# half-potato/nmf

Hardware: AMD Instinct MI355X
Metric: train rays/sec (microfacet_tensorf2, 4096-ray chunks, steady state) (higher is better)
Workload: dtype f32; 1 GPU; BASELINE configs[1] on scene S1 (solid cube, SURVEY 8d), TensoRF 128^3 (16+24 comps, f32 tables), env 512x1024, 800x800 camera, 4096 rays/GPU/step in 1 chunk(s) of 4096, fwd+bwd+all-reduce+Adam, steady state (all secondary rays re-traced); rays_per_gpu=4096, chunks_in_flight=1, grid=128, parallelism=dp1, ranks_seen=1, startup_steps=55, operator_graph_fallbacks=0

## Files before the change

### include/nmf_hip.h

```cpp
#ifndef NMF_HIP_H
#define NMF_HIP_H

#include <stdint.h>

#ifdef __cplusplus
extern "C" {
#endif

#define NMF_OK 0
#define NMF_EINVAL (-1)
#define NMF_ERANGE (-2)

#define NMF_DENSITY_C 16
#define NMF_APP_C 24
#define NMF_APP_DIM 24
#define NMF_MLP_IN 66
#define NMF_MLP_HID 64

#define NMF_ABI_VERSION 125
int nmf_version(void);
const char* nmf_last_error_string(void);

int nmf_event_create(void** event);
int nmf_event_create_timed(void** event);
// ... 199 lines not shown
                        const float* feat_noise, float anoise, float min_rough, int32_t row_inputs, float* V, float* N,
                        float* r1, float* f0, float* diffuse, float* feat, float* xyz, void* stream);
int nmf_bounce_prep_fwd_heads(const int32_t* bidx, int64_t Mb, const float* normals, const float* app, const float* head_W,
                              const float* head_b, float diffuse_mul, float diffuse_bias, float tint_bias, float f0_bias,
                              float rough_bias, const float* xyzt, const int32_t* ray_id, const float* rays, const float* conv,
                              const float* feat_noise, float anoise, float min_rough, int32_t row_inputs, float* heads_out,
                              float* V, float* N, float* r1, float* f0, float* diffuse, float* feat, float* xyz, void* stream);
int nmf_bounce_prep_bwd(const int32_t* inv, int64_t M, const int32_t* bidx, int64_t Mb, const float* normals,
                        const float* heads, const int32_t* ray_id, const float* rays, const float* conv,
                        float min_rough, int32_t detach_normals, int32_t row_inputs, const float* dN,
                        const float* dr1, const float* df0,
                        const float* ddiffuse, const int32_t row_strides[4], const float* dfeat, float* d_normals,
                        float* d_heads, float* d_app, void* stream);
int nmf_bounce_prep_heads_bwd(const int32_t* bidx, int64_t Mb, const float* normals, const float* heads, const int32_t* ray_id,
                              const float* rays, const float* conv, float min_rough, int32_t detach_normals, const float* dN,
                              const float* dr1, const float* df0, const float* ddiffuse, const int32_t row_strides[4],
                              const float* dfeat, const float* app, const float* head_W, const float* head_b, float diffuse_mul,
                              float diffuse_bias, float tint_bias, float f0_bias, float rough_bias, float* d_normals, float* d_app,
                              float* g_head_W, float* g_head_b, void* stream);
int nmf_ray_compose_fwd(const float* weight, const float* refl_rows, const int32_t* inv, const float* normals,
                        const float* rays, const int64_t* offsets, int64_t B, const float* bg, int32_t bg_per_ray,
                        int32_t tonemap, int32_t noclip, float* rgb_map, float* acc, float* rgb_lin, float* ori,
                        void* stream);
int nmf_ray_compose_bwd(const float* weight, const float* refl_rows, const int32_t* inv, const float* normals,
                        const float* rays, const int32_t* ray_id, int64_t M, const float* bg, int32_t bg_per_ray,
                        int32_t tonemap, int32_t noclip, const float* rgb_lin, const float* d_rgb_map,
                        const float* d_acc, const float* d_ori, float* d_weight, float* d_refl, float* d_normals,
                        void* stream);
int nmf_bg_adjoint(const float* acc, const float* d_rgb_map, int64_t B, float* d_bg, void* stream);

int nmf_retrace_scores(const float* brdf , const float* V_rows, const float* N_rows ,
                       const float* lpdf , const float* w_rows , const int32_t* cnt_rows,
                       const int32_t* row_of_ray, int64_t R, float* score, void* stream);
int nmf_argsort_f32(const float* keys, int64_t n, int32_t* order, void* workspace, int64_t workspace_bytes,
                    void* stream);
int64_t nmf_topk_select_workspace_bytes(int64_t n);
int nmf_topk_select(const float* keys, int64_t n, int64_t k, int32_t* idx_top, int32_t* idx_rest, void* workspace,
                    int64_t workspace_bytes, void* stream);
int64_t nmf_argsort_workspace_bytes(int64_t n);

int nmf_l1_mean_fwd(const float* const x[], const int64_t numel[], int32_t count, float* out, void* stream);
int nmf_l1_mean_bwd(const float* const x[], const int64_t numel[], int32_t count, const float* d_out,
                    float* const g[], int32_t accumulate, void* stream);
int nmf_sqerr_fwd(const float* pred, const float* gt, int64_t n, float* out, void* stream);
int nmf_sqerr_bwd(const float* pred, const float* gt, int64_t n, const float* d_out, float* d_pred, void* stream);
int nmf_loss_mix_fwd(const float* const x[], const int64_t numel[], const float w[], int32_t count, float scale,
                     float* out, void* stream);
int nmf_loss_mix_bwd(const int64_t numel[], const float w[], int32_t count, float scale, const float* d_out,
                     float* const g[], void* stream);
int64_t nmf_loss_head_workspace_bytes(int64_t n_rays);
int nmf_loss_head(const float* pred, const float* gt, int64_t n_rays, const float* d_out, float scale, float w_pred,
                  float w_a, float w_b, float* loss, float* d_pred, float* g_a, float* g_b, void* workspace,
                  int64_t workspace_bytes, void* stream);

typedef struct {
    void* param;
    const void* grad;
    void* exp_avg;
    void* exp_avg_sq;
    int64_t numel;
    double beta1, beta2, eps, weight_decay, step_size, bc2_sqrt;
    int32_t is_f64;
    int32_t reserved;
} nmf_adam_slot;
int nmf_adam_step(const nmf_adam_slot* slots, int32_t n_slots, const float* guard, void* stream);

typedef struct {
    const void* src;
    void* dst;
    int64_t numel;
    int32_t src_is_f64;
    int32_t dst_is_f64;
} nmf_copy_slot;
int nmf_multi_copy(const nmf_copy_slot* slots, int32_t n_slots, void* stream);

int nmf_ssim(const float* a, const float* b, int64_t n_img, int32_t H, int32_t W, int32_t C,
             const double* taps11, double c1, double c2,
             double* mean_out, float* map_out, void* workspace, int64_t workspace_bytes, void* stream);
int64_t nmf_ssim_workspace_bytes(int64_t n_img, int32_t H, int32_t W, int32_t C);
int nmf_normal_err(const float* pred, const float* gt, const float* acc, int64_t n_img, int64_t n_px,
                   double* mean_out, float* err_map, void* workspace, int64_t workspace_bytes, void* stream);
int64_t nmf_normal_err_workspace_bytes(int64_t n_img, int64_t n_px);

int nmf_material_maps(const float* app, const float* normals, const float* weight, const int64_t* offsets, int64_t B, int64_t M,
                      const float* rays, const float* head_W, const float* head_b, float diffuse_mul, float diffuse_bias,
                      float tint_bias, float f0_bias, float rough_bias, const float* conv, const int32_t* inv,
                      const int64_t* row_off, const int32_t* cnt, int64_t Mb, const float* incoming, const float* brdf_weight,
                      int64_t R, const float* acc, const float* bg, float* out, void* stream);

#define NMF_EDIT_ROW 32
#define NMF_EDIT_MAX 16
int nmf_heads_edit(float* heads, const float* xyz, int32_t xyz_stride, int64_t n, const float* edits, int32_t n_edits, void* stream);
int nmf_material_maps_edit(const float* app, const float* normals, const float* weight, const int64_t* offsets, int64_t B, int64_t M,
                           const float* rays, const float* head_W, const float* head_b, float diffuse_mul, float diffuse_bias,
                           float tint_bias, float f0_bias, float rough_bias, const float* conv, const int32_t* inv,
                           const int64_t* row_off, const int32_t* cnt, int64_t Mb, const float* incoming, const float* brdf_weight,
                           int64_t R, const float* acc, const float* bg, float* out, const float* xyz, int32_t xyz_stride,
                           const float* edits, int32_t n_edits, void* stream);

int nmf_mc_count(const float* vol, int32_t gx, int32_t gy, int32_t gz, float level, uint8_t* cases, int32_t* vcount,
                 int32_t* tcount, void* stream);
int nmf_mc_emit(const float* vol, int32_t gx, int32_t gy, int32_t gz, float level, const uint8_t* cases, const int32_t* vscan,
                const int32_t* tscan, int64_t n_verts, int64_t n_faces, float* verts, int32_t* faces, void* stream);
int64_t nmf_mc_workspace_bytes(int32_t gx, int32_t gy, int32_t gz);
int nmf_mc_case_triangles(int case_index, int8_t out[16]);

#define NMF_TV_PLANE 0
#define NMF_TV_LINE 1
#define NMF_TV_ENVMAP 2
int64_t nmf_tv_workspace_bytes(const int32_t* shape, const int32_t* kind, int32_t count);
int nmf_tv_fwd_bwd(const float* const x[], float* const g[], const int32_t* shape, const int64_t* x_stride, const int64_t* g_stride,
                   const int32_t* kind, const float w[], int32_t count, const float* scale_dev, float* value_out, void* workspace,
                   int64_t workspace_bytes, void* stream);

int nmf_env_resample(const float* src, int32_t kind, int32_t Hs, int32_t Ws, float r00, float r01, float r02, float r10, float r11,
                     float r12, float r20, float r21, float r22, float gain, int32_t supersample, float* dst, int32_t H, int32_t W,
                     void* stream);

int nmf_relight_frame(const float* rgb_lin, const float* acc, int64_t n_img, int64_t H, int64_t W, float* out, void* stream);
int64_t nmf_relight_ratio_workspace_bytes(int64_t n_img, int64_t H, int64_t W);
int nmf_relight_ratio(const float* pred, const float* gt, int64_t n_img, int64_t H, int64_t W, double* sum, int64_t* count,
                      void* workspace, int64_t workspace_bytes, void* stream);
int64_t nmf_relight_adjust_workspace_bytes(int64_t n_img, int64_t H, int64_t W);
int nmf_relight_adjust(const float* pred, const float* gt, float multi_r, float multi_g, float multi_b, int64_t n_img, int64_t H,
                       int64_t W, float* tp, float* tg, double* sqerr, void* workspace, int64_t workspace_bytes, void* stream);

int nmf_camera_rays(float r00, float r01, float r02, float r10, float r11, float r12, float r20, float r21, float r22, float tx,
                    float ty, float tz, float fx, float fy, float cx, float cy, int32_t H, int32_t W, float* rays, void* stream);
int nmf_frame_finish(const float* rgb, const float* depth, const float* normal, const float* acc, float near, float far,
                     const uint8_t* lut, int32_t H, int32_t W, uint8_t* out, void* stream);

int nmf_atlas_texels(const float* verts, const int32_t* faces, int64_t V, int64_t F, int32_t W, int32_t T, int64_t t0, int64_t n,
                     float* pos, int32_t* face_of, void* stream);
int nmf_atlas_store(const int32_t* face_of, const float* albedo, const float* f0, const float* roughness, const float* normal,
                    int64_t t0, int64_t n, int32_t W, uint8_t* albedo_tex, uint8_t* f0_tex, uint8_t* rough_tex, uint8_t* normal_tex,
                    void* stream);

#define NMF_MERGE_MAX_LISTS 8
typedef struct {
    const int64_t* offsets[NMF_MERGE_MAX_LISTS];
    const float* z[NMF_MERGE_MAX_LISTS];
    int64_t* dst[NMF_MERGE_MAX_LISTS];
    float scale[NMF_MERGE_MAX_LISTS];
    int64_t M[NMF_MERGE_MAX_LISTS];
} nmf_merge_lists;
int nmf_rays_place(const float* rays_in, const float* R, const float* c, float s, int32_t inverse, int64_t B, float* rays_out,
                   void* stream);
int nmf_merge_rank(int32_t K, const nmf_merge_lists* lists, int64_t B, int64_t* offsets_m, void* stream);
int nmf_merge_scatter(int64_t M_k, int64_t M_total, const int64_t* dst, const float* sigma, const float* dist, const float* z,
                      const float* normal, const int32_t* ray_id, const int32_t* inv, float sigma_ratio, float scale, const float* R,
                      int32_t part, int64_t row_base, float* sigma_m, float* dist_m, float* z_m, float* normal_m, int32_t* ray_id_m,
                      int32_t* part_m, int32_t* src_m, int32_t* inv_m, void* stream);

#ifdef __cplusplus
}
#endif
#endif
```

### nmf_amd/csrc/brdf.hip

```cpp
#include "common.hpp"

namespace {



template <int G>
__global__ void __launch_bounds__(256) k_segment_sum_wide(const float* __restrict__ vals, int64_t stride, int D,
                                                          const int64_t* __restrict__ offsets, int64_t n_seg,
                                                          float* __restrict__ out) {
    const int64_t s = (int64_t)blockIdx.x * 4 + (threadIdx.x >> 6);
    if (s >= n_seg) return;
    const int lane = lane_id();
    const int ch = lane & (G - 1), slot = lane / G;
    constexpr int SLOTS = 64 / G;
    const int64_t b = offsets[s], e = offsets[s + 1];
    float a = 0.f;
    if (ch < D) {
        float a1 = 0.f, a2 = 0.f, a3 = 0.f;
        int64_t r = b + slot;
        for (; r + 3 * SLOTS < e; r += 4 * SLOTS) {
            const float v0 = vals[r * stride + ch], v1 = vals[(r + SLOTS) * stride + ch];
            const float v2 = vals[(r + 2 * SLOTS) * stride + ch], v3 = vals[(r + 3 * SLOTS) * stride + ch];
            a += v0; a1 += v1; a2 += v2; a3 += v3;
        }
        for (; r < e; r += SLOTS) a += vals[r * stride + ch];
        a = (a + a1) + (a2 + a3);
    }
#pragma unroll
    for (int sh = 32; sh >= G; sh >>= 1) a += __shfl_down(a, sh, 64);
    if (lane < D) out[s * D + lane] = a;
}

}


extern "C" int nmf_segment_sum_wide(const float* vals, int64_t row_stride, int32_t D, const int64_t* offsets,
                                    int64_t n_seg, float* out, void* stream) {
    NMF_REQUIRE(n_seg >= 0, NMF_EINVAL, "nmf_segment_sum_wide: n_seg < 0");
    if (n_seg == 0) return NMF_OK;
    NMF_REQUIRE(vals && offsets && out && D > 0 && D <= 64 && row_stride >= D, NMF_EINVAL, "nmf_segment_sum_wide: args");
    const dim3 grid((unsigned)cdiv(n_seg, 4)), block(256);
    hipStream_t st = (hipStream_t)stream;
    if (D <= 8) NMF_LAUNCH(k_segment_sum_wide<8>, grid, block, 0, st, vals, row_stride, D, offsets, n_seg, out);
    else if (D <= 16) NMF_LAUNCH(k_segment_sum_wide<16>, grid, block, 0, st, vals, row_stride, D, offsets, n_seg, out);
    else if (D <= 32) NMF_LAUNCH(k_segment_sum_wide<32>, grid, block, 0, st, vals, row_stride, D, offsets, n_seg, out);
    else NMF_LAUNCH(k_segment_sum_wide<64>, grid, block, 0, st, vals, row_stride, D, offsets, n_seg, out);
    NMF_CHECK_LAUNCH("nmf_segment_sum_wide");
    return NMF_OK;
}
```

### nmf_amd/csrc/composite.hip

```cpp
#include "common.hpp"

namespace {

constexpr int WPR_MAX_RAYS = 16384;

template <int W, int D>
__device__ __forceinline__ double lane_below(double v) {
    if constexpr (W <= 16) {
        return dpp_f64<0x110 + D, 0xf, 0xf>(v);
    } else {
        return __shfl_up(v, D, W);
    }
}
template <int W>
__device__ __forceinline__ double group_incl_prod(double v, int lane) {
    { const double t = lane_below<W, 1>(v); if (lane >= 1) v *= t; }
    if constexpr (W > 2) { const double t = lane_below<W, 2>(v); if (lane >= 2) v *= t; }
    if constexpr (W > 4) { const double t = lane_below<W, 4>(v); if (lane >= 4) v *= t; }
    if constexpr (W > 8) { const double t = lane_below<W, 8>(v); if (lane >= 8) v *= t; }
    if constexpr (W > 16) { const double t = __shfl_up(v, 16, W); if (lane >= 16) v *= t; }
    if constexpr (W > 32) { const double t = __shfl_up(v, 32, W); if (lane >= 32) v *= t; }
    return v;
}
template <int W>
__device__ __forceinline__ double group_incl_sum(double v, int lane) {
    { const double t = lane_below<W, 1>(v); if (lane >= 1) v += t; }
    if constexpr (W > 2) { const double t = lane_below<W, 2>(v); if (lane >= 2) v += t; }
    if constexpr (W > 4) { const double t = lane_below<W, 4>(v); if (lane >= 4) v += t; }
    if constexpr (W > 8) { const double t = lane_below<W, 8>(v); if (lane >= 8) v += t; }
    if constexpr (W > 16) { const double t = __shfl_up(v, 16, W); if (lane >= 16) v += t; }
    if constexpr (W > 32) { const double t = __shfl_up(v, 32, W); if (lane >= 32) v += t; }
    return v;
}

template <int W>
__global__ void __launch_bounds__(256) k_composite_fwd_wave(const float* __restrict__ sigma,
                                                            const float* __restrict__ dist,
                                                            const int64_t* __restrict__ offsets, int64_t b, float scale,
                                                            float* __restrict__ weight, float* __restrict__ acc) {
    const int64_t r = ((int64_t)blockIdx.x * 256 + threadIdx.x) / W;
    const int lane = threadIdx.x & (W - 1);
    const bool ray_ok = r < b;
    const int64_t s = ray_ok ? offsets[r] : 0, e = ray_ok ? offsets[r + 1] : 0;
    double carry = 1.0;
    float a_sum = 0.f;
    float sg_n = 0.f, ds_n = 0.f;
    if (s + lane < e) { sg_n = sigma[s + lane]; ds_n = dist[s + lane]; }
    for (int64_t k0 = s; k0 < e; k0 += W) {
        const int64_t k = k0 + lane;
        const bool in = k < e;
        const float sg = sg_n, ds = ds_n;
        if (k + W < e) { sg_n = sigma[k + W]; ds_n = dist[k + W]; }
        float alpha = 0.f;
        if (in) alpha = 1.0f - expf(-fmul(sg, fmul(ds, scale)));
        const float f = in ? fadd(fsub(1.0f, alpha), 1e-10f) : 1.0f;
        const double incl = group_incl_prod<W>((double)f, lane);
        const double below = lane_below<W, 1>(incl);
        const double T = carry * (lane >= 1 ? below : 1.0);
        const float w = fmul(alpha, (float)T);
        if (in) weight[k] = w;
        a_sum += in ? w : 0.f;
        carry *= __shfl(incl, W - 1, W);
    }
    if (acc) {
#pragma unroll
        for (int d = W / 2; d > 0; d >>= 1) a_sum += __shfl_down(a_sum, d, W);
        if (lane == 0 && ray_ok) acc[r] = a_sum;
    }
}

template <int W>
__global__ void __launch_bounds__(256) k_composite_bwd_wave(const float* __restrict__ sigma,
                                                            const float* __restrict__ dist,
                                                            const float* __restrict__ weight,
                                                            const int64_t* __restrict__ offsets, int64_t b, float scale,
                                                            const float* __restrict__ d_weight,
                                                            float* __restrict__ d_sigma, int one_chunk_path) {
    const int64_t r = ((int64_t)blockIdx.x * 256 + threadIdx.x) / W;
    const int lane = threadIdx.x & (W - 1);
    const bool ray_ok = r < b;
    const int64_t s = ray_ok ? offsets[r] : 0, e = ray_ok ? offsets[r + 1] : 0;
    if (one_chunk_path && e - s <= W) {
        const int n = (int)(e - s);
        const bool in = lane < n;
        const int64_t k = e - 1 - lane;
        float dw = 0.f, d = 0.f, ex = 1.f, f = 1.0f;
        double v = 0.0;
        if (in) {
            dw = d_weight[k];
            v = (double)dw * (double)weight[k];
            d = fmul(dist[k], scale);
            ex = expf(-fmul(sigma[k], d));
            f = fadd(fsub(1.0f, 1.0f - ex), 1e-10f);
        }
        const double incl = group_incl_sum<W>(v, lane);
        const float A = in ? (-(float)(0.0 + incl - v) / f) * (d * ex) : 0.f;
        const int src = in ? n - 1 - lane : lane;
        const float d2 = __shfl(d, src, W), ex2 = __shfl(ex, src, W), dw2 = __shfl(dw, src, W), A2 = __shfl(A, src, W);
        const float f2 = in ? __shfl(f, src, W) : 1.0f;
        const double incl2 = group_incl_prod<W>((double)f2, lane);
        const double below = lane_below<W, 1>(incl2);
        const double T = 1.0 * (lane >= 1 ? below : 1.0);
        if (in) d_sigma[s + lane] = A2 + dw2 * (float)T * (d2 * ex2);
        return;
    }
    double carry = 0.0;
    float p_dw = 0.f, p_w = 0.f, p_di = 0.f, p_sg = 0.f;
    if (e - 1 - lane >= s) { const int64_t q = e - 1 - lane; p_dw = d_weight[q]; p_w = weight[q]; p_di = dist[q]; p_sg = sigma[q]; }
    for (int64_t k1 = e; k1 > s; k1 -= W) {
        const int64_t k = k1 - 1 - lane;
        const bool in = k >= s;
        const float c_dw = p_dw, c_w = p_w, c_di = p_di, c_sg = p_sg;
        if (k - W >= s) { const int64_t q = k - W; p_dw = d_weight[q]; p_w = weight[q]; p_di = dist[q]; p_sg = sigma[q]; }
        const double v = in ? (double)c_dw * (double)c_w : 0.0;
        const double incl = group_incl_sum<W>(v, lane);
        if (in) {
            const float d = fmul(c_di, scale);
            const float ex = expf(-fmul(c_sg, d));
            const float f = fadd(fsub(1.0f, 1.0f - ex), 1e-10f);
            d_sigma[k] = (-(float)(carry + incl - v) / f) * (d * ex);
        }
        carry += __shfl(incl, W - 1, W);
    }
    double cp = 1.0;
    float q_di = 0.f, q_sg = 0.f, q_dw = 0.f, q_ds = 0.f;
    if (s + lane < e) { const int64_t q = s + lane; q_di = dist[q]; q_sg = sigma[q]; q_dw = d_weight[q]; q_ds = d_sigma[q]; }
    for (int64_t k0 = s; k0 < e; k0 += W) {
        const int64_t k = k0 + lane;
        const bool in = k < e;
        const float c_di = q_di, c_sg = q_sg, c_dw = q_dw, c_ds = q_ds;
        if (k + W < e) { const int64_t q = k + W; q_di = dist[q]; q_sg = sigma[q]; q_dw = d_weight[q]; q_ds = d_sigma[q]; }
        float d = 0.f, ex = 1.f;
        if (in) { d = fmul(c_di, scale); ex = expf(-fmul(c_sg, d)); }
        const float f = in ? fadd(fsub(1.0f, 1.0f - ex), 1e-10f) : 1.0f;
        const double incl = group_incl_prod<W>((double)f, lane);
        const double below = lane_below<W, 1>(incl);
        const double T = cp * (lane >= 1 ? below : 1.0);
        if (in) d_sigma[k] = c_ds + c_dw * (float)T * (d * ex);
        cp *= __shfl(incl, W - 1, W);
    }
}

template <int D>
__global__ void __launch_bounds__(256) k_segment_sum(const float* __restrict__ vals, const float* __restrict__ scale,
                                                     const int64_t* __restrict__ offsets, int64_t n_seg,
                                                     float* __restrict__ out) {
    const int64_t r = (int64_t)blockIdx.x * blockDim.x + threadIdx.x;
    if (r >= n_seg) return;
    const int64_t s = offsets[r], e = offsets[r + 1];
    float a[D];
#pragma unroll
    for (int d = 0; d < D; ++d) a[d] = 0.f;
    for (int64_t k = s; k < e; ++k) {
        const float sc = scale ? scale[k] : 1.f;
#pragma unroll
        for (int d = 0; d < D; ++d) a[d] = fadd(a[d], fmul(sc, vals[k * D + d]));
    }
#pragma unroll
    for (int d = 0; d < D; ++d) out[r * D + d] = a[d];
}

template <int D, int W>
__global__ void __launch_bounds__(256) k_segment_sum_group(const float* __restrict__ vals, const float* __restrict__ scale,
                                                           const int64_t* __restrict__ offsets, int64_t n_seg,
                                                           float* __restrict__ out) {
    const int64_t r = ((int64_t)blockIdx.x * 256 + threadIdx.x) / W;
    const int lane = threadIdx.x & (W - 1);
    const bool ok = r < n_seg;
    const int64_t s = ok ? offsets[r] : 0, e = ok ? offsets[r + 1] : 0;
    float a[D];
#pragma unroll
    for (int d = 0; d < D; ++d) a[d] = 0.f;
    int64_t k = s + lane;
    for (; k + 3 * W < e; k += 4 * W) {
        float sc[4], v[4][D];
#pragma unroll
        for (int q = 0; q < 4; ++q) {
            sc[q] = scale ? scale[k + q * W] : 1.f;
#pragma unroll
            for (int d = 0; d < D; ++d) v[q][d] = vals[(k + q * W) * D + d];
        }
#pragma unroll
        for (int q = 0; q < 4; ++q)
#pragma unroll
            for (int d = 0; d < D; ++d) a[d] += sc[q] * v[q][d];
    }
    for (; k < e; k += W) {
        const float sc = scale ? scale[k] : 1.f;
#pragma unroll
        for (int d = 0; d < D; ++d) a[d] += sc * vals[k * D + d];
    }
#pragma unroll
    for (int sh = W / 2; sh > 0; sh >>= 1) {
#pragma unroll
        for (int d = 0; d < D; ++d) a[d] += __shfl_down(a[d], sh, W);
    }
    if (ok && lane == 0) {
#pragma unroll
        for (int d = 0; d < D; ++d) out[r * D + d] = a[d];
    }
}

}

static int group_width(int dflt) { return dflt; }

extern "C" int nmf_composite_fwd(const float* sigma, const float* dist, const int64_t* offsets, int64_t b,
                                 float distance_scale, float* weight, float* acc, void* stream) {
    NMF_REQUIRE(b >= 0, NMF_EINVAL, "nmf_composite_fwd: b < 0");
    if (b == 0) return NMF_OK;
    NMF_REQUIRE(sigma && dist && offsets && weight, NMF_EINVAL, "nmf_composite_fwd: null");
    if (b <= WPR_MAX_RAYS)
        NMF_LAUNCH(k_composite_fwd_wave<64>, dim3((unsigned)cdiv(b, 4)), dim3(256), 0, (hipStream_t)stream, sigma,
                           dist, offsets, b, distance_scale, weight, acc);
    else if (group_width(8) == 16)
        NMF_LAUNCH(k_composite_fwd_wave<16>, dim3((unsigned)cdiv(b, 16)), dim3(256), 0, (hipStream_t)stream, sigma,
                           dist, offsets, b, distance_scale, weight, acc);
    else
        NMF_LAUNCH(k_composite_fwd_wave<8>, dim3((unsigned)cdiv(b, 32)), dim3(256), 0, (hipStream_t)stream, sigma,
                           dist, offsets, b, distance_scale, weight, acc);
    NMF_CHECK_LAUNCH("nmf_composite_fwd");
    return NMF_OK;
}

extern "C" int nmf_composite_bwd(const float* sigma, const float* dist, const float* weight, const int64_t* offsets,
                                 int64_t b, float distance_scale, const float* d_weight, float* d_sigma,
                                 void* stream) {
    NMF_REQUIRE(b >= 0, NMF_EINVAL, "nmf_composite_bwd: b < 0");
    if (b == 0) return NMF_OK;
    NMF_REQUIRE(sigma && dist && weight && offsets && d_weight && d_sigma, NMF_EINVAL, "nmf_composite_bwd: null");
    static const int one_chunk = !(getenv("NMF_COMPOSITE_ONE_CHUNK") && atoi(getenv("NMF_COMPOSITE_ONE_CHUNK")) == 0);
    if (b <= WPR_MAX_RAYS)
        NMF_LAUNCH(k_composite_bwd_wave<64>, dim3((unsigned)cdiv(b, 4)), dim3(256), 0, (hipStream_t)stream, sigma,
                           dist, weight, offsets, b, distance_scale, d_weight, d_sigma, one_chunk);
    else if (group_width(16) == 16)
        NMF_LAUNCH(k_composite_bwd_wave<16>, dim3((unsigned)cdiv(b, 16)), dim3(256), 0, (hipStream_t)stream, sigma,
                           dist, weight, offsets, b, distance_scale, d_weight, d_sigma, one_chunk);
    else
        NMF_LAUNCH(k_composite_bwd_wave<8>, dim3((unsigned)cdiv(b, 32)), dim3(256), 0, (hipStream_t)stream, sigma,
                           dist, weight, offsets, b, distance_scale, d_weight, d_sigma, one_chunk);
    NMF_CHECK_LAUNCH("nmf_composite_bwd");
    return NMF_OK;
}

extern "C" int nmf_segment_sum(const float* vals, const float* scale, const int64_t* offsets, int64_t n_seg,
                               int32_t D, int32_t lanes, float* out, void* stream) {
    NMF_REQUIRE(n_seg >= 0, NMF_EINVAL, "nmf_segment_sum: n_seg < 0");
    if (n_seg == 0) return NMF_OK;
    NMF_REQUIRE(vals && offsets && out, NMF_EINVAL, "nmf_segment_sum: null");
    NMF_REQUIRE(lanes == 1 || lanes == 8, NMF_ERANGE, "nmf_segment_sum: lanes must be 1 (index order) or 8");
    hipStream_t st = (hipStream_t)stream;
    if (lanes == 8) {
        dim3 grid((unsigned)cdiv(n_seg, 32)), block(256);
        switch (D) {
            case 1: NMF_LAUNCH((k_segment_sum_group<1, 8>), grid, block, 0, st, vals, scale, offsets, n_seg, out); break;
            case 2: NMF_LAUNCH((k_segment_sum_group<2, 8>), grid, block, 0, st, vals, scale, offsets, n_seg, out); break;
            case 3: NMF_LAUNCH((k_segment_sum_group<3, 8>), grid, block, 0, st, vals, scale, offsets, n_seg, out); break;
            case 4: NMF_LAUNCH((k_segment_sum_group<4, 8>), grid, block, 0, st, vals, scale, offsets, n_seg, out); break;
            default: return nmf_fail(NMF_ERANGE, "nmf_segment_sum: D must be 1..4");
        }
        NMF_CHECK_LAUNCH("nmf_segment_sum");
        return NMF_OK;
    }
    dim3 grid((unsigned)cdiv(n_seg, 256)), block(256);
    switch (D) {
        case 1: NMF_LAUNCH(k_segment_sum<1>, grid, block, 0, st, vals, scale, offsets, n_seg, out); break;
        case 2: NMF_LAUNCH(k_segment_sum<2>, grid, block, 0, st, vals, scale, offsets, n_seg, out); break;
        case 3: NMF_LAUNCH(k_segment_sum<3>, grid, block, 0, st, vals, scale, offsets, n_seg, out); break;
        case 4: NMF_LAUNCH(k_segment_sum<4>, grid, block, 0, st, vals, scale, offsets, n_seg, out); break;
        default: return nmf_fail(NMF_ERANGE, "nmf_segment_sum: D must be 1..4");
    }
    NMF_CHECK_LAUNCH("nmf_segment_sum");
    return NMF_OK;
}
```

### nmf_amd/csrc/heads.hip

```cpp
#include "heads_eval.hpp"
#include "rows_bwd.hpp"

namespace {

using nmf_heads::F;
using nmf_heads::O;
using nmf_heads::HeadP;
using nmf_heads::sigm;

__device__ __forceinline__ void load_feat(const float* __restrict__ feat, int64_t m, float (&f)[F]) {
    const float4* q = reinterpret_cast<const float4*>(feat + m * F);
#pragma unroll
    for (int i = 0; i < F / 4; ++i) {
        const float4 v = q[i];
        f[4 * i] = v.x; f[4 * i + 1] = v.y; f[4 * i + 2] = v.z; f[4 * i + 3] = v.w;
    }
}

__global__ void __launch_bounds__(256) k_heads_fwd(const float* __restrict__ feat, int64_t M, const float* __restrict__ W,
                                                   const float* __restrict__ b, HeadP hp, float* __restrict__ out) {
    const int64_t m = (int64_t)blockIdx.x * blockDim.x + threadIdx.x;
    if (m >= M) return;
    float f[F], v[O];
    load_feat(feat, m, f);
// ... 17 lines not shown
    __shared__ float s_W[O * F];
    __shared__ float s_b[O];
    for (int i = t; i < O * F; i += 256) s_W[i] = W[i];
    if (t < O) s_b[t] = b[t];
    __syncthreads();
    const int64_t n_it = (M + 255) / 256;
    for (int64_t it = blockIdx.x; it < n_it; it += gridDim.x) {
        const int64_t m = it * 256 + t;
        float f[F], da[O];
        if (m < M) {
            load_feat(feat, m, f);
            float gq[O];
            float4 addv[F / 4];
            if (rin.bidx) nmf_rows::prep_bwd_row(rin, m, gq, addv);
#pragma unroll
            for (int j = 0; j < O; ++j) {
                float a = s_b[j];
#pragma unroll
                for (int k = 0; k < F; ++k) a += s_W[j * F + k] * f[k];
                const float g = rin.bidx ? gq[j] : d_out[m * O + j];
                float d;
                if (j < 3) {
                    const float s = sigm(hp.diffuse_mul * a + hp.diffuse_bias);
                    d = g * s * (1.f - s) * hp.diffuse_mul;
                } else if (j < 9) {
                    const float s = sigm(a + (j < 6 ? hp.tint_bias : hp.f0_bias));
                    d = g * s * (1.f - s);
                } else {
                    const float s = sigm(a + hp.rough_bias);
                    const float r = 0.5f * s;
                    d = (r >= 1e-2f && r <= 1.f) ? g * 0.5f * s * (1.f - s) : 0.f;
                }
                da[j] = d;
            }
            float df[F];
#pragma unroll
            for (int k = 0; k < F; ++k) df[k] = 0.f;
#pragma unroll
            for (int j = 0; j < O; ++j)
#pragma unroll
                for (int k = 0; k < F; ++k) df[k] += da[j] * s_W[j * F + k];
            float4* q = reinterpret_cast<float4*>(d_feat + m * F);
            if (rin.bidx) {
#pragma unroll
                for (int i = 0; i < F / 4; ++i) {
                    df[4 * i] = addv[i].x + df[4 * i]; df[4 * i + 1] = addv[i].y + df[4 * i + 1];
                    df[4 * i + 2] = addv[i].z + df[4 * i + 2]; df[4 * i + 3] = addv[i].w + df[4 * i + 3];
                }
            } else if (d_feat_add) {
                const float4* qa = reinterpret_cast<const float4*>(d_feat_add + m * F);
#pragma unroll
                for (int i = 0; i < F / 4; ++i) {
                    const float4 a = qa[i];
                    df[4 * i] = a.x + df[4 * i]; df[4 * i + 1] = a.y + df[4 * i + 1];
                    df[4 * i + 2] = a.z + df[4 * i + 2]; df[4 * i + 3] = a.w + df[4 * i + 3];
                }
            }
#pragma unroll
            for (int i = 0; i < F / 4; ++i) q[i] = make_float4(df[4 * i], df[4 * i + 1], df[4 * i + 2], df[4 * i + 3]);
        } else {
#pragma unroll
            for (int k = 0; k < F; ++k) f[k] = 0.f;
#pragma unroll
            for (int j = 0; j < O; ++j) da[j] = 0.f;
        }
        __syncthreads();
#pragma unroll
        for (int j = 0; j < O; ++j) s_da[t * (O + 1) + j] = da[j];
#pragma unroll
        for (int k = 0; k < F; ++k) s_f[t * (F + 1) + k] = f[k];
        __syncthreads();
#pragma unroll 4
        for (int r0 = 64 * wv; r0 < 64 * wv + 64; r0 += 4) {
            const int row = r0 + kg;
            const float a = ci < O ? s_da[row * (O + 1) + ci] : 0.f;
            const float b0 = s_f[row * (F + 1) + ci];
            const float b1 = ci < F - 16 ? s_f[row * (F + 1) + 16 + ci] : (ci == F - 16 ? 1.f : 0.f);
            g0 = __builtin_amdgcn_mfma_f32_16x16x4f32(a, b0, g0, 0, 0, 0);
            g1 = __builtin_amdgcn_mfma_f32_16x16x4f32(a, b1, g1, 0, 0, 0);
        }
    }
    __syncthreads();
    float* red = s_f;
#pragma unroll
    for (int r = 0; r < 4; ++r) {
        red[wv * 512 + r * 64 + lane] = g0[r];
        red[wv * 512 + 256 + r * 64 + lane] = g1[r];
    }
    __syncthreads();
#pragma unroll
    for (int e = t; e < 512; e += 256) {
        const float v = (red[e] + red[512 + e]) + (red[1024 + e] + red[1536 + e]);
        const int blk = e >> 8, r = (e >> 6) & 3, ln = e & 63;
        const int oi = 4 * (ln >> 4) + r, c = ln & 15;
        if (oi < O) {
            if (blk == 0) atomicAdd(gW + oi * F + c, v);
            else if (c < F - 16) atomicAdd(gW + oi * F + 16 + c, v);
            else if (c == F - 16) atomicAdd(gb + oi, v);
        }
    }
}

}

extern "C" int nmf_heads_fwd(const float* feat, int64_t M, const float* W, const float* b, float diffuse_mul,
                             float diffuse_bias, float tint_bias, float f0_bias, float rough_bias, float* out,
                             void* stream) {
    NMF_REQUIRE(M >= 0, NMF_EINVAL, "nmf_heads_fwd: M < 0");
    if (M == 0) return NMF_OK;
    NMF_REQUIRE(feat && W && b && out, NMF_EINVAL, "nmf_heads_fwd: null");
    HeadP hp{diffuse_mul, diffuse_bias, tint_bias, f0_bias, rough_bias};
    NMF_LAUNCH(k_heads_fwd, dim3((unsigned)cdiv(M, 256)), dim3(256), 0, (hipStream_t)stream, feat, M, W, b, hp, out);
    NMF_CHECK_LAUNCH("nmf_heads_fwd");
    return NMF_OK;
}

extern "C" int nmf_heads_bwd(const float* feat, int64_t M, const float* W, const float* b, float diffuse_mul,
                             float diffuse_bias, float tint_bias, float f0_bias, float rough_bias, const float* d_out,
                             const float* d_feat_add, float* d_feat, float* gW, float* gb, void* stream) {
    NMF_REQUIRE(M >= 0, NMF_EINVAL, "nmf_heads_bwd: M < 0");
    if (M == 0) return NMF_OK;
    NMF_REQUIRE(feat && W && b && d_out && d_feat && gW && gb, NMF_EINVAL, "nmf_heads_bwd: null");
    HeadP hp{diffuse_mul, diffuse_bias, tint_bias, f0_bias, rough_bias};
    const int64_t n_it = cdiv(M, 256);
    const unsigned grid = (unsigned)(n_it < 1024 ? n_it : 1024);
    NMF_LAUNCH(k_heads_bwd, dim3(grid), dim3(256), 0, (hipStream_t)stream, feat, M, W, b, hp, d_out, d_feat_add, d_feat, gW, gb,
                       nmf_rows::RowsBwdIn{});
    NMF_CHECK_LAUNCH("nmf_heads_bwd");
    return NMF_OK;
}

extern "C" int nmf_bounce_prep_heads_bwd(const int32_t* bidx, int64_t Mb, const float* normals, const float* heads,
                                         const int32_t* ray_id, const float* rays, const float* conv, float min_rough,
                                         int32_t detach_normals, const float* dN, const float* dr1, const float* df0,
                                         const float* ddiffuse, const int32_t row_strides[4], const float* dfeat, const float* app,
                                         const float* head_W, const float* head_b, float diffuse_mul, float diffuse_bias,
                                         float tint_bias, float f0_bias, float rough_bias, float* d_normals, float* d_app,
                                         float* g_head_W, float* g_head_b, void* stream) {
    NMF_REQUIRE(Mb >= 0, NMF_EINVAL, "nmf_bounce_prep_heads_bwd: Mb < 0");
    if (Mb == 0) return NMF_OK;
    NMF_REQUIRE(bidx && normals && heads && ray_id && rays && conv && app && head_W && head_b && d_normals && d_app && g_head_W &&
                    g_head_b, NMF_EINVAL, "nmf_bounce_prep_heads_bwd: null");
    HeadP hp{diffuse_mul, diffuse_bias, tint_bias, f0_bias, rough_bias};
    nmf_rows::RowsBwdIn rin{bidx, normals, heads, ray_id, rays, nmf_rows::Conv{conv}, min_rough, (int)detach_normals, dN, dr1, df0, ddiffuse,
                            row_strides ? row_strides[0] : 3, row_strides ? row_strides[1] : 1, row_strides ? row_strides[2] : 3,
                            row_strides ? row_strides[3] : 3, dfeat, d_normals};
    const int64_t n_it = cdiv(Mb, 256);
    const unsigned grid = (unsigned)(n_it < 1024 ? n_it : 1024);
    NMF_LAUNCH(k_heads_bwd, dim3(grid), dim3(256), 0, (hipStream_t)stream, app, Mb, head_W, head_b, hp, nullptr, nullptr, d_app,
                       g_head_W, g_head_b, rin);
    NMF_CHECK_LAUNCH("nmf_bounce_prep_heads_bwd");
    return NMF_OK;
}
```

### nmf_amd/csrc/host_ext.cpp

```cpp
#include <torch/extension.h>

#include <algorithm>
#include <chrono>
#include <cstring>
#include <functional>
#include <map>
#include <memory>
#include <string>
#include <tuple>
#include <vector>

#include "nmf_hip.h"

namespace py = pybind11;
using at::Tensor;
using OT = c10::optional<Tensor>;

namespace {

PyObject* g_error_class = nullptr;

[[noreturn]] void fail(const std::string& msg) {
    if (g_error_class) {
        PyErr_SetString(g_error_class, msg.c_str());
// ... 769 lines not shown
    if (!ok || x.stride(0) < width) {
        x = x.contiguous();
        keep.push_back(x);
    }
    return {static_cast<const float*>(x.data_ptr()), (int)(x.size(0) > 1 ? x.stride(0) : width)};
}

std::tuple<Tensor, Tensor, Tensor> vm_query_rows(int64_t p_addr, const Tensor& xyzt, const std::vector<Tensor>& dpk,
                                                 const std::vector<Tensor>& dlk, int64_t stream) {
    TimedScope _ts(__func__, stream);
    const auto* p = reinterpret_cast<const nmf_vm_params*>(p_addr);
    const int64_t M = xyzt.size(0);
    if (dpk.size() != 3 || dlk.size() != 3) fail("vm_query_rows: three planes / lines expected");
    const bool bf16 = dpk[0].scalar_type() == at::kBFloat16;
    const void *a[3], *b[3];
    for (int i = 0; i < 3; ++i) {
        if (dpk[i].scalar_type() != dpk[0].scalar_type() || dlk[i].scalar_type() != dpk[0].scalar_type())
            fail("vm_query_rows: mixed table dtypes");
        a[i] = vptr(dpk[i]);
        b[i] = vptr(dlk[i]);
    }
    Tensor sf = fe(xyzt, {M}), gr = fe(xyzt, {M, 3}), nr = fe(xyzt, {M, 3});
    check(nmf_vm_query_rows(p, f32(xyzt), M, a, b, bf16 ? 1 : 0, out(sf), nullptr, out(gr), out(nr), st(stream)),
          "nmf_vm_query_rows");
    return {sf, gr, nr};
}

std::tuple<Tensor, Tensor> vm_query_sigma(int64_t p_addr, const Tensor& xyzt, const std::vector<Tensor>& planes,
                                          const std::vector<Tensor>& lines, int64_t stream) {
    TimedScope _ts(__func__, stream);
    const auto* p = reinterpret_cast<const nmf_vm_params*>(p_addr);
    const int64_t M = xyzt.size(0);
    if (planes.size() != 3 || lines.size() != 3) fail("vm_query_sigma: three planes / lines expected");
    const bool bf16 = planes[0].scalar_type() == at::kBFloat16;
    const void *a[3], *b[3];
    for (int i = 0; i < 3; ++i) {
        if (planes[i].scalar_type() != planes[0].scalar_type() || lines[i].scalar_type() != planes[0].scalar_type())
            fail("vm_query_sigma: mixed table dtypes");
        if (planes[i].size(-1) != 16 || lines[i].size(-1) != 16 || !planes[i].is_contiguous() || !lines[i].is_contiguous())
            fail("vm_query_sigma: density factors [G,G,16] / [G,16] (channel-last views) expected");
        a[i] = vptr(planes[i]);
        b[i] = vptr(lines[i]);
    }
    Tensor sf = fe(xyzt, {M}), sg = fe(xyzt, {M});
    check(nmf_vm_query_sigma(p, f32(xyzt), M, a, b, bf16 ? 1 : 0, out(sf), out(sg), st(stream)), "nmf_vm_query_sigma");
    return {sf, sg};
}

Tensor sqerr_fwd(const Tensor& pred, const Tensor& gt, int64_t stream) {
    TimedScope _ts(__func__, stream);
    Tensor o = at::zeros({}, pred.options().dtype(at::kFloat));
    if (pred.numel()) check(nmf_sqerr_fwd(f32(pred), f32(gt), pred.numel(), out(o), st(stream)), "nmf_sqerr_fwd");
    return o;
}

Tensor sqerr_bwd(const Tensor& pred, const Tensor& gt, const Tensor& d_out, int64_t stream) {
    TimedScope _ts(__func__, stream);
    Tensor d = at::empty_like(pred);
    if (pred.numel()) check(nmf_sqerr_bwd(f32(pred), f32(gt), pred.numel(), f32(d_out), out(d), st(stream)), "nmf_sqerr_bwd");
    return d;
}

std::tuple<Tensor, Tensor, Tensor, Tensor, Tensor> shade_mix_bwd_view(const Tensor& V, const Tensor& f0, const Tensor& diff,
                                                                      const Tensor& cnt, const Tensor& row_of_ray,
                                                                      const Tensor& L, const Tensor& inc, const Tensor& brdf,
                                                                      const Tensor& d_rows, int64_t stream) {
    TimedScope _ts(__func__, stream);
    const int64_t R = row_of_ray.size(0);
    Tensor d_inc = fe(V, {R, 3}), d_brdf = fe(V, {R, 3}), dL = fe(V, {R, 3}), d_fd = fe(V, {R, 6}), dV = fe(V, {R, 3});
    check(nmf_shade_mix_bwd_view(f32(V), f32(f0), f32(diff), i32(cnt), i32(row_of_ray), R, f32(L), f32(inc), f32(brdf),
                                 f32(d_rows), out(d_inc), out(d_brdf), out(dL), out(d_fd), out(dV), st(stream)),
          "nmf_shade_mix_bwd_view");
    return {d_inc, d_brdf, dL, d_fd, dV};
}

Tensor ggx_rays_bwd_view(const Tensor& V, const Tensor& N, const Tensor& r, const Tensor& off, const Tensor& sobol,
                         const Tensor& row_of_ray, const Tensor& j_of_ray, const OT& dL, const OT& d_rays,
                         int64_t stream) {
    TimedScope _ts(__func__, stream);
    const int64_t R = row_of_ray.size(0);
    Tensor d = fe(V, {R, 7});
    check(nmf_ggx_rays_bwd_view(f32(V), f32(N), f32(r), f32(off), f32(sobol), i32(row_of_ray), i32(j_of_ray), R,
                                static_cast<const float*>(vptr(dL)), static_cast<const float*>(vptr(d_rays)), out(d),
                                st(stream)),
          "nmf_ggx_rays_bwd_view");
    return d;
}

void view_adjoint_to_rays(const Tensor& ray_id, const Tensor& bidx, const Tensor& dv_a, const OT& dv_b, Tensor d_rays,
                          int64_t stream) {
    TimedScope _ts(__func__, stream);
    std::vector<Tensor> keep;
    const auto a = rows_of(dv_a, 3, keep), b = rows_of(dv_b, 3, keep);
    check(nmf_view_adjoint_to_rays(i32(ray_id), i32(bidx), a.first, a.second, b.first, b.second, bidx.size(0),
                                   ptr<float>(d_rays, at::kFloat), st(stream)),
          "nmf_view_adjoint_to_rays");
}

Tensor select_total(const Tensor& weights, const Tensor& u, double extra, Tensor ws, int64_t stream) {
    TimedScope _ts(__func__, stream);
    Tensor total = at::empty({}, weights.options().dtype(at::kFloat));
    check(nmf_select_total(f32(weights), f32(u), weights.size(0), extra, ptr<double>(ws, at::kDouble), out(total),
                           st(stream)),
          "nmf_select_total");
    return total;
}

std::tuple<Tensor, Tensor, Tensor> bounce_prep_bwd(const OT& inv, const Tensor& normals, const Tensor& heads, const Tensor& ray_id,
                                                   const Tensor& rays, const Tensor& conv, double min_rough, bool detach_n,
                                                   const OT& dN, const OT& dr1, const OT& df0, const OT& ddiff, const OT& dfeat,
                                                   const OT& bidx, int64_t row_inputs, int64_t stream) {
    TimedScope _ts(__func__, stream);
    const int64_t M = inv.has_value() ? inv->size(0) : ray_id.size(0);
    const int64_t Mb = bidx.has_value() ? bidx->size(0) : 0;
    const int64_t n_out = row_inputs ? Mb : M;
    Tensor d_normals = fe(normals, {row_inputs == 2 ? Mb : M, 3}), d_heads = fe(normals, {n_out, 11});
    Tensor d_app = fe(normals, {n_out, 24});
    if (M) {
        std::vector<Tensor> keep;
        const auto a = rows_of(dN, 3, keep), b = rows_of(dr1, 1, keep), c = rows_of(df0, 3, keep), d = rows_of(ddiff, 3, keep);
        const int32_t strides[4] = {a.second, b.second, c.second, d.second};
        check(nmf_bounce_prep_bwd(static_cast<const int32_t*>(vptr(inv)), M, static_cast<const int32_t*>(vptr(bidx)), Mb,
                                  f32(normals), heads.size(0) ? f32(heads) : nullptr, i32(ray_id), f32(rays), f32(conv),
                                  (float)min_rough, detach_n ? 1 : 0, (int32_t)row_inputs, a.first, b.first, c.first, d.first,
                                  strides, static_cast<const float*>(vptr(dfeat)), out(d_normals), out(d_heads), out(d_app),
                                  st(stream)),
              "nmf_bounce_prep_bwd");
    }
    return {d_normals, d_heads, d_app};
}

std::tuple<Tensor, Tensor> bounce_prep_heads_bwd(const Tensor& bidx, const Tensor& normals, const Tensor& heads, const Tensor& ray_id,
                                                 const Tensor& rays, const Tensor& conv, double min_rough, bool detach_n, const OT& dN,
                                                 const OT& dr1, const OT& df0, const OT& ddiff, const OT& dfeat, const Tensor& app,
                                                 const Tensor& W, const Tensor& b, const std::vector<double>& hp, const Tensor& gW,
                                                 const Tensor& gb, int64_t stream) {
    TimedScope _ts("heads_bwd", stream);
    if (hp.size() != 5) fail("bounce_prep_heads_bwd: hp = (diffuse_mul, diffuse_bias, tint_bias, f0_bias, rough_bias)");
    const int64_t Mb = bidx.size(0);
    Tensor d_normals = fe(normals, {Mb, 3}), d_app = fe(normals, {Mb, 24});
    if (Mb) {
        std::vector<Tensor> keep;
        const auto a = rows_of(dN, 3, keep), b2 = rows_of(dr1, 1, keep), c = rows_of(df0, 3, keep), d = rows_of(ddiff, 3, keep);
        const int32_t strides[4] = {a.second, b2.second, c.second, d.second};
        OT df;
        if (dfeat.has_value()) df = dfeat->contiguous();
        check(nmf_bounce_prep_heads_bwd(i32(bidx), Mb, f32(normals), f32(heads), i32(ray_id), f32(rays), f32(conv), (float)min_rough,
                                        detach_n ? 1 : 0, a.first, b2.first, c.first, d.first, strides, of32(df), f32(app), f32(W),
                                        f32(b), (float)hp[0], (float)hp[1], (float)hp[2], (float)hp[3], (float)hp[4], out(d_normals),
                                        out(d_app), static_cast<float*>(vptr(gW)), static_cast<float*>(vptr(gb)), st(stream)),
              "nmf_bounce_prep_heads_bwd");
    }
    return {d_normals, d_app};
}

void adam_step(int64_t slots_addr, int64_t n, const OT& guard, int64_t stream) {
    TimedScope _ts(__func__, stream);
    check(nmf_adam_step(reinterpret_cast<const nmf_adam_slot*>(slots_addr), (int32_t)n, of32(guard), st(stream)),
          "nmf_adam_step");
}
void multi_copy(int64_t slots_addr, int64_t n, int64_t stream) {
    TimedScope _ts(__func__, stream);
    check(nmf_multi_copy(reinterpret_cast<const nmf_copy_slot*>(slots_addr), (int32_t)n, st(stream)), "nmf_multi_copy");
}

std::vector<Tensor> loss_mix_bwd(const std::vector<std::vector<int64_t>>& shapes, const std::vector<double>& weights,
                                 double scale, const Tensor& d_out, int64_t stream) {
    TimedScope _ts(__func__, stream);
    const size_t n = shapes.size();
    if (weights.size() != n || n > 16) fail("loss_mix_bwd: shapes / weights");
    std::vector<Tensor> grads;
    int64_t numel[16];
    float w[16];
    float* g[16];
    for (size_t i = 0; i < n; ++i) {
        grads.push_back(at::empty(shapes[i], d_out.options().dtype(at::kFloat)));
        numel[i] = grads[i].numel();
        w[i] = (float)weights[i];
        g[i] = out(grads[i]);
    }
    check(nmf_loss_mix_bwd(numel, w, (int32_t)n, (float)scale, f32(d_out), g, st(stream)), "nmf_loss_mix_bwd");
    return grads;
}

void l1_mean_bwd_into(const std::vector<Tensor>& tensors, const Tensor& d_out, std::vector<Tensor> grads, bool accumulate,
                      int64_t stream) {
    TimedScope _ts(__func__, stream);
    const size_t n = tensors.size();
    if (grads.size() != n || n > 32) fail("l1_mean_bwd: tensors / gradients");
    const float* x[32];
    float* g[32];
    int64_t numel[32];
    for (size_t i = 0; i < n; ++i) {
        if (grads[i].numel() != tensors[i].numel()) fail("l1_mean_bwd: gradient / tensor size mismatch");
        x[i] = dense_f32(tensors[i]);
        g[i] = const_cast<float*>(dense_f32(grads[i]));
        numel[i] = tensors[i].numel();
    }
    check(nmf_l1_mean_bwd(x, numel, (int32_t)n, f32(d_out), g, accumulate ? 1 : 0, st(stream)), "nmf_l1_mean_bwd");
}

void sat_build_bwd_into(Tensor d_sat, const Tensor& bg, const Tensor& act, const OT& d_pole, double brightness, double mul,
                        const OT& sc, Tensor d_bg, int64_t stream) {
    TimedScope _ts(__func__, stream);
    const int64_t H = bg.size(-2), W = bg.size(-1);
    check(nmf_sat_build_bwd(ptr<float>(d_sat, at::kFloat), f32(bg), f32(act), (int32_t)H, (int32_t)W, (float)brightness,
                            (float)mul, static_cast<const float*>(vptr(sc)), static_cast<const float*>(vptr(d_pole)),
                            ptr<float>(d_bg, at::kFloat), st(stream)),
          "nmf_sat_build_bwd");
}

void sat_build_into(const Tensor& bg, double brightness, double mul, const OT& sc, Tensor act, Tensor sat, const OT& pole,
                    const OT& sat_i4, int64_t stream) {
    TimedScope _ts(__func__, stream);
    const int64_t H = bg.size(-2), W = bg.size(-1);
    check(nmf_sat_build(f32(bg), (int32_t)H, (int32_t)W, (float)brightness, (float)mul, static_cast<const float*>(vptr(sc)),
                        ptr<float>(act, at::kFloat), ptr<float>(sat, at::kFloat), static_cast<float*>(vptr(pole)),
                        static_cast<float*>(vptr(sat_i4)), st(stream)),
          "nmf_sat_build");
}

void sh_project_into(const Tensor& vals, const Tensor& wq, const Tensor& sh_A, Tensor coeffs, Tensor conv, int64_t stream) {
    TimedScope _ts(__func__, stream);
    check(nmf_sh_project(f32(vals), f32(wq), wq.size(0), (int32_t)wq.size(1), f32(sh_A), ptr<float>(coeffs, at::kFloat),
                         ptr<float>(conv, at::kFloat), st(stream)),
          "nmf_sh_project");
}

void vm_pack_density_into(int64_t p_addr, const std::vector<Tensor>& planes, const std::vector<Tensor>& lines,
                          const std::vector<Tensor>& dpk, const std::vector<Tensor>& dlk, int64_t stream) {
    TimedScope _ts(__func__, stream);
    const auto* p = reinterpret_cast<const nmf_vm_params*>(p_addr);
    P3 a = three(planes), b = three(lines), c = three(dpk), d = three(dlk);
    float *oc[3], *od[3];
    for (int i = 0; i < 3; ++i) { oc[i] = const_cast<float*>(c.p[i]); od[i] = const_cast<float*>(d.p[i]); }
    check(nmf_vm_pack_density(p, a.p, b.p, oc, od, st(stream)), "nmf_vm_pack_density");
}

#include "step_core.inc"

}

namespace {

template <class F>
void drain_timer(CallTimer*& timer, F fn) {
    std::unique_ptr<CallTimer> t(timer);
    timer = nullptr;
    if (!t) return;
    for (auto& r : t->recs) {
        check(nmf_event_synchronize(r.b), "nmf_event_synchronize");
        fn(r, t->recs[0]);
    }
}
float ms_between(void* a, void* b) {
    float ms = 0.f;
    check(nmf_event_elapsed_ms(a, b, &ms), "nmf_event_elapsed_ms");
    return ms;
}
template <class F>
py::dict timer_sums(CallTimer*& timer, F keys) {
    std::map<std::string, std::pair<double, int64_t>> acc;
    drain_timer(timer, [&](const CallTimer::Rec& r, const CallTimer::Rec&) {
        const float ms = ms_between(r.a, r.b);
        for (const std::string& k : keys(r)) {
            acc[k].first += ms;
            acc[k].second += 1;
        }
    });
    py::dict out;
    for (auto& kv : acc) out[py::str(kv.first)] = py::make_tuple(kv.second.first, kv.second.second);
    return out;
}

PyObject* g_unsupported_class = nullptr;

}

PYBIND11_MODULE(_nmf_host, m) {
    m.doc() = "host-side fast path of nmf_amd.hip (same C ABI underneath)";
    m.def("set_error_class", [](py::object cls) {
        g_error_class = cls.ptr();
        Py_XINCREF(g_error_class);
    });
    m.def("set_unsupported_class", [](py::object cls) {
        g_unsupported_class = cls.ptr();
        Py_XINCREF(g_unsupported_class);
    });
    m.def("unsupported_class", []() { return g_unsupported_class ? py::reinterpret_borrow<py::object>(g_unsupported_class) : py::object(py::none()); });
    py::register_local_exception_translator([](std::exception_ptr p) {
        try {
            if (p) std::rethrow_exception(p);
        } catch (const UnsupportedChunk& e) {
            PyErr_SetString(g_unsupported_class ? g_unsupported_class : PyExc_RuntimeError, e.what());
        }
    });
    m.def("abi_version", []() { return (int)NMF_ABI_VERSION; });
    m.def("call_timing_begin", [](const std::string& only) {
        if (!g_call_timer) g_call_timer = new CallTimer();
        g_call_timer->next = 0;
        g_call_timer->recs.clear();
        g_call_filter = only;
    }, py::arg("only") = "");
    m.def("call_timing_end", []() {
        return timer_sums(g_call_timer, [](const CallTimer::Rec& r) { return std::vector<std::string>{r.name}; });
    });
    m.def("kernel_timing_begin", [](const std::string& only, bool by_stream) {
        g_kernel_by_stream = by_stream;
        if (!g_kernel_timer) g_kernel_timer = new CallTimer();
        g_kernel_timer->next = 0;
        g_kernel_timer->recs.clear();
        g_kernel_filter = only;
        g_probe_open = nullptr;
        check(nmf_set_launch_probe(&launch_probe), "nmf_set_launch_probe");
    }, py::arg("only") = "", py::arg("by_stream") = false);
    m.def("kernel_timing_end", []() {
        check(nmf_set_launch_probe(nullptr), "nmf_set_launch_probe");
        return timer_sums(g_kernel_timer, [](const CallTimer::Rec& r) {
            const std::string sid = "@" + std::to_string(reinterpret_cast<int64_t>(r.stream));
            std::vector<std::string> keys = {kernel_name(r.name), sid};
            if (g_kernel_by_stream) keys.push_back(kernel_name(r.name) + sid);
            return keys;
        });
    });
    m.def("readback_wait_us", [](bool reset) { const double w = SizeReadback::waited_us(); if (reset) SizeReadback::waited_us() = 0.0; return w; });
    m.def("readback_wait_by_slot_us", [](bool reset) {
        std::vector<double> v(SizeReadback::waited_by_slot(), SizeReadback::waited_by_slot() + 4);
        if (reset) for (int i = 0; i < 4; ++i) SizeReadback::waited_by_slot()[i] = 0.0;
        return v;
    });
    m.def("set_call_delay", [](const std::string& name, double us) { g_delay_name = name; g_delay_us = us; });
    m.def("call_timing_timeline", []() {
        py::list out;
        drain_timer(g_call_timer, [&](const CallTimer::Rec& r, const CallTimer::Rec& first) {
            out.append(py::make_tuple(std::string(r.name), reinterpret_cast<int64_t>(r.stream), 1e3 * ms_between(first.a, r.a),
                                      1e3 * ms_between(first.a, r.b), r.host_us - first.host_us));
        });
        return out;
    });
    m.def("march_count", &march_count);
    m.def("march_scan", &march_scan, py::arg("counts"), py::arg("max_samples"), py::arg("stream"), py::arg("pub") = 0, py::arg("pub_seq") = 0);
    m.def("march_fill", &march_fill);
    using OV = c10::optional<std::vector<Tensor>>;
    m.def("vm_query_fwd", [](int64_t p_addr, const Tensor& xyzt, const OV& dpk, const OV& dlk, const OV& apl, const OV& ali, const OT& basis,
                             bool want_density, bool want_normal, bool want_app, bool want_coef, int64_t stream, int64_t live) {
        const std::vector<Tensor> none;
        return vm_query_fwd(p_addr, xyzt, dpk ? *dpk : none, dlk ? *dlk : none, apl ? *apl : none, ali ? *ali : none, basis,
                            want_density, want_normal, want_app, want_coef, stream, live);
    }, py::arg("p_addr"), py::arg("xyzt"), py::arg("dpk"), py::arg("dlk"), py::arg("apl"), py::arg("ali"), py::arg("basis"),
       py::arg("want_density"), py::arg("want_normal"), py::arg("want_app"), py::arg("want_coef"), py::arg("stream"), py::arg("live") = 0);
    m.def("composite_fwd", &composite_fwd);
    m.def("segment_sum", &segment_sum);
    m.def("sat_lookup_fwd", &sat_lookup_fwd);
    m.def("select_bounces", &select_bounces);
    m.def("expand_segments", &expand_segments);
    m.def("brdf_mlp_fwd", &brdf_mlp_fwd, py::arg("w"), py::arg("half_vec"), py::arg("diff_vec"), py::arg("feat_src"), py::arg("rough_src"),
          py::arg("src_idx"), py::arg("out_bias"), py::arg("with_mask"), py::arg("max_workgroups"), py::arg("stream"),
          py::arg("image") = py::none());
    m.def("brdf_mlp_pack", &brdf_mlp_pack);
    m.def("bounce_prep_heads_bwd", &bounce_prep_heads_bwd);
    m.def("bounce_prep_fwd_heads", &bounce_prep_fwd_heads);
    m.def("brdf_mlp_bwd_sets", &brdf_mlp_bwd_sets, py::arg("w"), py::arg("sets"), py::arg("grads"), py::arg("max_workgroups"), py::arg("stream"),
          py::arg("image") = py::none());
    m.def("heads_fwd", &heads_fwd);
    m.def("material_maps", &material_maps, py::arg("app"), py::arg("normals"), py::arg("w"), py::arg("offsets"), py::arg("rays"), py::arg("W"),
          py::arg("b"), py::arg("hp"), py::arg("conv"), py::arg("inv"), py::arg("row_off"), py::arg("cnt"), py::arg("incoming"),
          py::arg("brdf_weight"), py::arg("acc"), py::arg("bg"), py::arg("stream"), py::arg("xyz") = py::none(), py::arg("edits") = py::none());
    m.def("heads_edit", &heads_edit);
    m.def("ggx_rays_fwd", &ggx_rays_fwd);
    m.def("shade_mix_fwd", &shade_mix_fwd);
    m.def("bounce_index", &bounce_index, py::arg("counts"), py::arg("xyzt"), py::arg("stream"), py::arg("pub") = 0, py::arg("pub_seq") = 0,
          py::arg("live") = 0);
    m.def("bounce_index_select", [](const Tensor& w, const Tensor& u, int64_t mode, double mul, double add, double sum_w, const OT& sum_w_dev,
                                    const OT& xyzt, int64_t stream) {
        return bounce_index_select(w, u, mode, mul, add, sum_w, sum_w_dev, xyzt, stream);
    });
    m.def("bounce_prep_fwd", &bounce_prep_fwd);
    m.def("ray_compose_fwd", &ray_compose_fwd);
    m.def("composite_bwd", &composite_bwd);
    m.def("segment_sum_wide", &segment_sum_wide);
    m.def("sat_lookup_bwd", &sat_lookup_bwd);
    m.def("brdf_mlp_bwd", &brdf_mlp_bwd, py::arg("w"), py::arg("half_vec"), py::arg("diff_vec"), py::arg("feat_src"), py::arg("rough_src"),
          py::arg("src_idx"), py::arg("fwd_out"), py::arg("act_mask"), py::arg("d_out"), py::arg("grads"), py::arg("max_workgroups"),
          py::arg("stream"), py::arg("image") = py::none());
    m.def("heads_bwd", &heads_bwd);
    m.def("ggx_rays_bwd", &ggx_rays_bwd);
    m.def("shade_mix_bwd", &shade_mix_bwd);
    m.def("ray_compose_bwd", &ray_compose_bwd);
    m.def("vm_query_bwd_segments", &vm_query_bwd_segments);
    m.def("vm_unpack_density_grad", &vm_unpack_density_grad);
    m.def("adam_step", &adam_step);
    m.def("multi_copy", &multi_copy);
    m.def("loss_mix_bwd", &loss_mix_bwd);
    m.def("l1_mean_bwd_into", &l1_mean_bwd_into);
    m.def("sat_build_bwd_into", &sat_build_bwd_into);
    m.def("sat_build_into", &sat_build_into);
    m.def("sh_project_into", &sh_project_into);
    m.def("vm_pack_density_into", &vm_pack_density_into);
    m.def("vm_query_rows", &vm_query_rows);
    m.def("vm_query_sigma", &vm_query_sigma);
    m.def("sat_lookup_bwd_dirs", &sat_lookup_bwd_dirs);
    m.def("sat_lookup_bwd_table", &sat_lookup_bwd_table);
    m.def("loss_head", &loss_head);
    m.def("bg_adjoint", &bg_adjoint);
    m.def("sqerr_fwd", &sqerr_fwd);
    m.def("sqerr_bwd", &sqerr_bwd);
    m.def("shade_mix_bwd_view", &shade_mix_bwd_view);
    m.def("ggx_rays_bwd_view", &ggx_rays_bwd_view);
    m.def("view_adjoint_to_rays", &view_adjoint_to_rays);
    m.def("select_total", &select_total);
    m.def("bounce_prep_bwd", &bounce_prep_bwd);
    py::class_<StepCore>(m, "StepCore")
        .def(py::init<>())
        .def("chunk", &StepCore::chunk)
        .def("train_forward", &StepCore::train_forward)
        .def("train_backward", &StepCore::train_backward)
        .def("has_pending", &StepCore::has_pending)
        .def("render", &StepCore::render, py::arg("rays"), py::arg("focal"), py::arg("noise"), py::arg("want_maps"),
             py::arg("want_materials") = false, py::arg("want_linear") = false)
        .def("set_material_edits", &StepCore::set_material_edits)
        .def("n_material_edits", &StepCore::n_material_edits)
        .def("begin_step", &StepCore::begin_step)
        .def("join_env_table_backward", &StepCore::join_env_table_backward)
        .def("env_was_used", &StepCore::env_was_used)
        .def("env_table_backward_queued", &StepCore::env_table_backward_queued)
#define RW(name) .def_readwrite(#name, &StepCore::name)
        RW(env_keep_sat) RW(env_split) RW(early_cb) RW(comm_stream) RW(peer_streams) RW(main_stream) RW(side_streams) RW(set_stream) RW(main_stream_obj) RW(side_stream_objs) RW(overlap) RW(sparse_normals)
        RW(mlp_side_min_rays) RW(mlp_side_min_env_rays) RW(mlp_side_wgs_env) RW(walk_side_min_samples) RW(mlp_side_wgs)
        RW(env_binned_from) RW(vm_p) RW(dpk) RW(dlk) RW(dpl) RW(dli) RW(f_dpk) RW(f_dlk) RW(f_apl) RW(f_ali) RW(apl) RW(ali) RW(basis) RW(head_p) RW(head_W) RW(head_b) RW(mlp_ws) RW(mlp_image)
        RW(mlp_bias) RW(sobol) RW(env_table) RW(env_pole) RW(env_sc) RW(env_act) RW(env_bg) RW(sh_conv) RW(march_p0) RW(march_p1)
        RW(max_samples) RW(alpha_bits) RW(alpha_coarse) RW(scale) RW(anoise) RW(min_rough) RW(rays_per_ray) RW(test_rays_per_ray)
        RW(detach_n) RW(max_brdf_rays) RW(max_retrace_rays) RW(white) RW(one) RW(select_ws) RW(g_dpk) RW(g_dlk) RW(g_apl) RW(g_ali)
        RW(g_mlp) RW(g_basis) RW(g_hW) RW(g_hb) RW(d_sat) RW(d_pole) RW(d_mip) RW(d_bg_out) RW(used_env) RW(sampler) RW(wait_tables) RW(wait_env)
#undef RW
        ;
}
```

### nmf_amd/csrc/rows_bwd.hpp

```cpp
#pragma once
#include "common.hpp"

namespace nmf_rows {

constexpr int HEADS = 11;
constexpr int FEAT = NMF_APP_DIM;

struct Conv {
    const float* c;
};

__device__ __forceinline__ void sh9(float x, float y, float z, float (&Y)[9]) {
    const float C0 = 0.28209479177387814f, C1 = 0.4886025119029199f;
    const float C20 = 1.0925484305920792f, C22 = 0.31539156525252005f, C24 = 0.5462742152960396f;
    Y[0] = C0;
    Y[1] = C1 * y;
    Y[2] = C1 * z;
    Y[3] = C1 * x;
    Y[4] = C20 * (x * y);
    Y[5] = C20 * (y * z);
    Y[6] = C22 * (3.f * (z * z) - 1.f);
    Y[7] = C20 * (x * z);
    Y[8] = C24 * (x * x - y * y);
}

__device__ __forceinline__ float sgn(float v) { return v > 0.f ? 1.f : (v < 0.f ? -1.f : 0.f); }


static __device__ __noinline__ void irradiance_E(float nx, float ny, float nz, Conv conv, float* __restrict__ E3) {
    float Y[9];
    sh9(nx, ny, nz, Y);
#pragma unroll
    for (int c = 0; c < 3; ++c) {
        float E = 0.f;
#pragma unroll
        for (int k = 0; k < 9; ++k) E += conv.c[k * 3 + c] * Y[k];
        E3[c] = E;
    }
}


struct RowsBwdIn {
    const int32_t* bidx;
    const float* normals;
    const float* heads;
    const int32_t* ray_id;
    const float* rays;
    Conv conv;
    float min_rough;
    int detach_n;
    const float *dN, *dr1, *df0, *ddiff;
    int sN, sr, sf, sd;
    const float* dfeat;
    float* d_normals;
};
__device__ __forceinline__ void prep_bwd_row(const RowsBwdIn& q, int64_t t, float (&gh)[HEADS], float4 (&gf)[FEAT / 4]) {
    const bool want_n = !q.detach_n && q.dN;
    const int64_t m = q.bidx[t];
    const float nx = q.normals[t * 3], ny = q.normals[t * 3 + 1], nz = q.normals[t * 3 + 2];
    float dn[3] = {0.f, 0.f, 0.f}, dd[3] = {0.f, 0.f, 0.f}, d0[3] = {0.f, 0.f, 0.f}, dr = 0.f;
    if (want_n) { dn[0] = q.dN[t * q.sN]; dn[1] = q.dN[t * q.sN + 1]; dn[2] = q.dN[t * q.sN + 2]; }
    if (q.ddiff) { dd[0] = q.ddiff[t * q.sd]; dd[1] = q.ddiff[t * q.sd + 1]; dd[2] = q.ddiff[t * q.sd + 2]; }
    if (q.df0) { d0[0] = q.df0[t * q.sf]; d0[1] = q.df0[t * q.sf + 1]; d0[2] = q.df0[t * q.sf + 2]; }
    if (q.dr1) dr = q.dr1[t * q.sr];
    const float h9 = q.heads[t * HEADS + 9];
#pragma unroll
    for (int i = 0; i < FEAT / 4; ++i)
        gf[i] = q.dfeat ? reinterpret_cast<const float4*>(q.dfeat + t * FEAT)[i] : make_float4(0.f, 0.f, 0.f, 0.f);
    float gn[3] = {0.f, 0.f, 0.f};
    if (want_n) {
        const float* d = q.rays + (int64_t)q.ray_id[m] * 6 + 3;
        const float s = sgn(-(d[0] * nx + d[1] * ny + d[2] * nz));
        gn[0] = dn[0] * s; gn[1] = dn[1] * s; gn[2] = dn[2] * s;
    }
    q.d_normals[t * 3] = gn[0]; q.d_normals[t * 3 + 1] = gn[1]; q.d_normals[t * 3 + 2] = gn[2];
#pragma unroll
    for (int j = 0; j < HEADS; ++j) gh[j] = 0.f;
    float E3[3];
    irradiance_E(nx, ny, nz, q.conv, E3);
#pragma unroll
    for (int c = 0; c < 3; ++c) {
        gh[c] = q.ddiff ? dd[c] * E3[c] : 0.f;
        gh[6 + c] = d0[c];
    }
    gh[9] = (q.dr1 && h9 >= q.min_rough) ? dr : 0.f;
}

}
```

### nmf_amd/csrc/shade.hip

```cpp
#include "common.hpp"
#include "heads_eval.hpp"
#include "rows_bwd.hpp"

namespace {

constexpr int IDX_CHUNK = 1024;
constexpr int FLAG_SHIFT = 40;

__device__ __forceinline__ int64_t wave_scan_i64(int64_t v, int lane) {
#pragma unroll
    for (int d = 1; d < 64; d <<= 1) {
        int64_t t = __shfl_up(v, d, 64);
        if (lane >= d) v += t;
    }
    return v;
}

__device__ __forceinline__ int64_t block_scan_i64(int64_t v, int64_t* ws , int64_t* total) {
    const int tid = threadIdx.x, lane = tid & 63, wid = tid >> 6;
    int64_t incl = wave_scan_i64(v, lane);
    if (lane == 63) ws[wid] = incl;
    __syncthreads();
    if (tid == 0) {
        int64_t run = 0;
// ... 224 lines not shown
        if (t >= Mb) return;
        nmf_rows::RowsBwdIn rin{bidx, normals, heads, ray_id, rays, conv, min_rough, detach_n, dN, dr1, df0, ddiff, sN, sr, sf, sd, dfeat,
                                d_normals};
        float gh[HEADS];
        float4 gf[FEAT / 4];
        nmf_rows::prep_bwd_row(rin, t, gh, gf);
        float4* o4 = reinterpret_cast<float4*>(d_app + t * FEAT);
#pragma unroll
        for (int i = 0; i < FEAT / 4; ++i) o4[i] = gf[i];
#pragma unroll
        for (int j = 0; j < HEADS; ++j) d_heads[t * HEADS + j] = gh[j];
        return;
    }
    if (row_inputs == 2) {
        if (t < Mb) {
            float gn[3] = {0.f, 0.f, 0.f};
            if (!detach_n && dN) {
                const float nx = normals[t * 3], ny = normals[t * 3 + 1], nz = normals[t * 3 + 2];
                const float* d = rays + (int64_t)ray_id[bidx[t]] * 6 + 3;
                const float s = sgn(-(d[0] * nx + d[1] * ny + d[2] * nz));
                gn[0] = dN[t * sN] * s; gn[1] = dN[t * sN + 1] * s; gn[2] = dN[t * sN + 2] * s;
            }
            d_normals[t * 3] = gn[0]; d_normals[t * 3 + 1] = gn[1]; d_normals[t * 3 + 2] = gn[2];
        }
    } else if (t < M) {
        const int64_t row = inv[t];
        float gn[3] = {0.f, 0.f, 0.f};
        if (row >= 0 && !detach_n && dN) {
            const float nx = normals[t * 3], ny = normals[t * 3 + 1], nz = normals[t * 3 + 2];
            const float* d = rays + (int64_t)ray_id[t] * 6 + 3;
            const float s = sgn(-(d[0] * nx + d[1] * ny + d[2] * nz));
            gn[0] = dN[row * sN] * s; gn[1] = dN[row * sN + 1] * s; gn[2] = dN[row * sN + 2] * s;
        }
        d_normals[t * 3] = gn[0]; d_normals[t * 3 + 1] = gn[1]; d_normals[t * 3 + 2] = gn[2];
    }
    const int64_t n_out = row_inputs ? Mb : M;
    if (t >= n_out) return;
    const int64_t row = row_inputs ? t : inv[t];
    const int64_t m = row_inputs ? (int64_t)bidx[t] : t;
    float gh[HEADS];
#pragma unroll
    for (int j = 0; j < HEADS; ++j) gh[j] = 0.f;
    float4* o4 = reinterpret_cast<float4*>(d_app + t * FEAT);
    if (row >= 0) {
        const int64_t in = row_inputs == 2 ? t : m;
        const float nx = normals[in * 3], ny = normals[in * 3 + 1], nz = normals[in * 3 + 2];
        const float* h = heads + t * HEADS;
        float E3[3];
        irradiance_E(nx, ny, nz, conv, E3);
#pragma unroll
        for (int c = 0; c < 3; ++c) {
            gh[c] = ddiff ? ddiff[row * sd + c] * E3[c] : 0.f;
            gh[6 + c] = df0 ? df0[row * sf + c] : 0.f;
        }
        gh[9] = (dr1 && h[9] >= min_rough) ? dr1[row * sr] : 0.f;
        const float4* g4 = dfeat ? reinterpret_cast<const float4*>(dfeat + row * FEAT) : nullptr;
#pragma unroll
        for (int i = 0; i < FEAT / 4; ++i) o4[i] = g4 ? g4[i] : make_float4(0.f, 0.f, 0.f, 0.f);
    } else {
#pragma unroll
        for (int i = 0; i < FEAT / 4; ++i) o4[i] = make_float4(0.f, 0.f, 0.f, 0.f);
    }
#pragma unroll
    for (int j = 0; j < HEADS; ++j) d_heads[t * HEADS + j] = gh[j];
}

constexpr float SRGB_LIMIT = 0.0031308f;

__device__ __forceinline__ float srgb(float x, int noclip) {
    float o = x > SRGB_LIMIT ? 1.055f * powf(fmaxf(x, SRGB_LIMIT), 1.0f / 2.4f) - 0.055f : 12.92f * x;
    return noclip ? o : fminf(fmaxf(o, 0.f), 1.f);
}

__device__ __forceinline__ float srgb_grad(float x, int noclip) {
    float o, g;
    if (x > SRGB_LIMIT) {
        const float p = powf(x, 1.0f / 2.4f);
        o = 1.055f * p - 0.055f;
        g = 1.055f * (1.0f / 2.4f) * p / x;
    } else {
        o = 12.92f * x;
        g = 12.92f;
    }
    if (!noclip && (o < 0.f || o > 1.f)) g = 0.f;
    return g;
}

template <int W>
__global__ void __launch_bounds__(256) k_ray_compose_fwd_wave(
    const float* __restrict__ weight, const float* __restrict__ refl_rows, const int32_t* __restrict__ inv,
    const float* __restrict__ normals, const float* __restrict__ rays, const int64_t* __restrict__ offsets, int64_t B,
    const float* __restrict__ bg, int bg_per_ray, int tonemap, int noclip, float* __restrict__ rgb_map,
    float* __restrict__ acc_out, float* __restrict__ rgb_lin, float* __restrict__ ori_out) {
    const int64_t r = ((int64_t)blockIdx.x * 256 + threadIdx.x) / W;
    const int lane = threadIdx.x & (W - 1);
    const bool ok = r < B;
    const int64_t s = ok ? offsets[r] : 0, e = ok ? offsets[r + 1] : 0;
    const int64_t rq = ok ? r : 0;
    const float dx = rays[rq * 6 + 3], dy = rays[rq * 6 + 4], dz = rays[rq * 6 + 5];
    float v[5] = {0.f, 0.f, 0.f, 0.f, 0.f};
    const bool rows = inv && refl_rows;
    for (int64_t k = s + lane; k < e; k += 2 * W) {
        const int64_t k1 = k + W;
        const bool two = k1 < e;
        const int64_t kb = two ? k1 : k;
        const float w0 = weight[k], w1 = two ? weight[kb] : 0.f;
        int64_t row0 = -1, row1 = -1;
        if (rows) { row0 = inv[k]; row1 = inv[kb]; }
        float n0[3] = {0.f, 0.f, 0.f}, n1[3] = {0.f, 0.f, 0.f};
        if (ori_out) {
#pragma unroll
            for (int c = 0; c < 3; ++c) { n0[c] = normals[k * 3 + c]; n1[c] = normals[kb * 3 + c]; }
        }
        float c0[3] = {0.f, 0.f, 0.f}, c1[3] = {0.f, 0.f, 0.f};
        if (rows) {
            const int64_t q0 = row0 >= 0 ? row0 : 0, q1 = row1 >= 0 ? row1 : 0;
#pragma unroll
            for (int c = 0; c < 3; ++c) { c0[c] = refl_rows[q0 * 3 + c]; c1[c] = refl_rows[q1 * 3 + c]; }
        }
        v[0] += w0;
        if (row0 >= 0) { v[1] += w0 * c0[0]; v[2] += w0 * c0[1]; v[3] += w0 * c0[2]; }
        if (ori_out) {
            const float ndv = fminf(-(dx * n0[0] + dy * n0[1] + dz * n0[2]), 0.f);
            v[4] += w0 * (ndv * ndv);
        }
        if (two) {
            v[0] += w1;
            if (row1 >= 0) { v[1] += w1 * c1[0]; v[2] += w1 * c1[1]; v[3] += w1 * c1[2]; }
            if (ori_out) {
                const float ndv = fminf(-(dx * n1[0] + dy * n1[1] + dz * n1[2]), 0.f);
                v[4] += w1 * (ndv * ndv);
            }
        }
    }
#pragma unroll
    for (int q = 0; q < 5; ++q)
        for (int d = W / 2; d > 0; d >>= 1) v[q] += __shfl_down(v[q], d, W);
    if (lane != 0 || !ok) return;
    rgb_lin[r * 3] = v[1]; rgb_lin[r * 3 + 1] = v[2]; rgb_lin[r * 3 + 2] = v[3];
    acc_out[r] = v[0];
    if (ori_out) ori_out[r] = v[4];
    const float* b = bg + (bg_per_ray ? r * 3 : 0);
    const float t = 1.f - v[0];
    rgb_map[r * 3] = (tonemap ? srgb(v[1], noclip) : v[1]) + t * b[0];
    rgb_map[r * 3 + 1] = (tonemap ? srgb(v[2], noclip) : v[2]) + t * b[1];
    rgb_map[r * 3 + 2] = (tonemap ? srgb(v[3], noclip) : v[3]) + t * b[2];
}

__global__ void __launch_bounds__(256) k_ray_compose_bwd(
    const float* __restrict__ weight, const float* __restrict__ refl_rows, const int32_t* __restrict__ inv,
    const float* __restrict__ normals, const float* __restrict__ rays, const int32_t* __restrict__ ray_id, int64_t M,
    const float* __restrict__ bg, int bg_per_ray, int tonemap, int noclip, const float* __restrict__ rgb_lin,
    const float* __restrict__ d_rgb_map, const float* __restrict__ d_acc, const float* __restrict__ d_ori,
    float* __restrict__ d_weight, float* __restrict__ d_refl, float* __restrict__ d_normals) {
    const int64_t m = (int64_t)blockIdx.x * blockDim.x + threadIdx.x;
    if (m >= M) return;
    const int64_t r = ray_id[m];
    const float w = weight[m];
    float g[3] = {0.f, 0.f, 0.f};
    float ga = d_acc ? d_acc[r] : 0.f;
    if (d_rgb_map) {
        const float* b = bg + (bg_per_ray ? r * 3 : 0);
#pragma unroll
        for (int c = 0; c < 3; ++c) {
            const float dm = d_rgb_map[r * 3 + c];
            g[c] = tonemap ? dm * srgb_grad(rgb_lin[r * 3 + c], noclip) : dm;
            ga -= dm * b[c];
        }
    }
    float dw = ga;
    const int64_t row = (inv && refl_rows) ? inv[m] : -1;
    if (row >= 0) {
        dw += g[0] * refl_rows[row * 3] + g[1] * refl_rows[row * 3 + 1] + g[2] * refl_rows[row * 3 + 2];
        d_refl[row * 3] = w * g[0]; d_refl[row * 3 + 1] = w * g[1]; d_refl[row * 3 + 2] = w * g[2];
    }
    float gn[3] = {0.f, 0.f, 0.f};
    if (d_ori) {
        const float dx = rays[r * 6 + 3], dy = rays[r * 6 + 4], dz = rays[r * 6 + 5];
        const float ndv = -(dx * normals[m * 3] + dy * normals[m * 3 + 1] + dz * normals[m * 3 + 2]);
        if (ndv < 0.f) {
            const float go = d_ori[r];
            dw += go * ndv * ndv;
            const float k = go * w * 2.f * ndv;
            gn[0] = -k * dx; gn[1] = -k * dy; gn[2] = -k * dz;
        }
    }
    d_weight[m] = dw;
    if (d_normals) {
        d_normals[m * 3] = gn[0]; d_normals[m * 3 + 1] = gn[1]; d_normals[m * 3 + 2] = gn[2];
    }
}

__global__ void __launch_bounds__(256) k_bg_adjoint(const float* __restrict__ acc, const float* __restrict__ d_rgb, int64_t n,
                                                    float* __restrict__ d_bg) {
    const int64_t k = (int64_t)blockIdx.x * 256 + threadIdx.x;
    if (k < n) d_bg[k] = (1.f - acc[k / 3]) * d_rgb[k];
}

}

extern "C" int64_t nmf_bounce_index_workspace_bytes(int64_t M) { return (cdiv(M > 0 ? M : 1, IDX_CHUNK) + 1) * 8; }

static int bounce_index_impl(const int32_t* counts, SelectArgs sel, int64_t M, const int64_t* M_live, int32_t* bidx, int64_t* row_off,
                             int32_t* cnt_rows, int32_t* inv, int64_t* totals, const float* xyzt, float* xyzt_rows, void* workspace,
                             int64_t workspace_bytes, void* publish_mapped_dev, int64_t publish_seq, void* stream);
extern "C" int nmf_bounce_index(const int32_t* counts, int64_t M, const int64_t* M_live, int32_t* bidx, int64_t* row_off,
                                int32_t* cnt_rows, int32_t* inv, int64_t* totals, const float* xyzt, float* xyzt_rows,
                                void* workspace, int64_t workspace_bytes, void* publish_mapped_dev, int64_t publish_seq,
                                void* stream) {
    NMF_REQUIRE(counts || M == 0, NMF_EINVAL, "nmf_bounce_index: null");
    return bounce_index_impl(counts, SelectArgs{nullptr, nullptr, 0, 0.f, 0.f, 0.f, nullptr}, M, M_live, bidx, row_off, cnt_rows, inv, totals,
                             xyzt, xyzt_rows, workspace, workspace_bytes, publish_mapped_dev, publish_seq, stream);
}
extern "C" int nmf_bounce_index_select(const float* weights, const float* u, int32_t mode, float mul, float add, float sum_w,
                                       const float* sum_w_dev, int64_t M, const int64_t* M_live, int32_t* bidx, int64_t* row_off,
                                       int32_t* cnt_rows, int32_t* inv, int64_t* totals, const float* xyzt, float* xyzt_rows,
                                       void* workspace, int64_t workspace_bytes, void* publish_mapped_dev, int64_t publish_seq,
                                       void* stream) {
    NMF_REQUIRE((weights && u) || M == 0, NMF_EINVAL, "nmf_bounce_index_select: null");
    NMF_REQUIRE(mode == 0 || mode == 1, NMF_EINVAL, "nmf_bounce_index_select: mode");
    NMF_REQUIRE(M <= (int64_t)IDX_CHUNK * IDX_CHUNK, NMF_ERANGE, "nmf_bounce_index_select: more than 2^20 samples (use nmf_select_bounces + nmf_bounce_index)");
    return bounce_index_impl(nullptr, SelectArgs{weights, u, (int)mode, mul, add, sum_w, sum_w_dev}, M, M_live, bidx, row_off, cnt_rows, inv,
                             totals, xyzt, xyzt_rows, workspace, workspace_bytes, publish_mapped_dev, publish_seq, stream);
}
static int bounce_index_impl(const int32_t* counts, SelectArgs sel, int64_t M, const int64_t* M_live, int32_t* bidx, int64_t* row_off,
                             int32_t* cnt_rows, int32_t* inv, int64_t* totals, const float* xyzt, float* xyzt_rows, void* workspace,
                             int64_t workspace_bytes, void* publish_mapped_dev, int64_t publish_seq, void* stream) {
    int64_t* pub = static_cast<int64_t*>(publish_mapped_dev);
    NMF_REQUIRE(M >= 0, NMF_EINVAL, "nmf_bounce_index: M < 0");
    NMF_REQUIRE(totals && row_off, NMF_EINVAL, "nmf_bounce_index: null");
    hipStream_t st = (hipStream_t)stream;
    if (M == 0) {
        hipError_t e = hipMemsetAsync(totals, 0, 16, st);
        if (e == hipSuccess) e = hipMemsetAsync(row_off, 0, 8, st);
        if (e != hipSuccess) return nmf_fail((int)e, "nmf_bounce_index: memset");
        if (pub) return nmf_publish_i64x2(totals, pub, publish_seq, stream);
        return NMF_OK;
    }
    NMF_REQUIRE((counts || sel.w) && bidx && cnt_rows && inv && workspace, NMF_EINVAL, "nmf_bounce_index: null");
    NMF_REQUIRE(!xyzt_rows || xyzt, NMF_EINVAL, "nmf_bounce_index: xyzt_rows needs xyzt");
    const float4* x4 = reinterpret_cast<const float4*>(xyzt);
    float4* r4 = reinterpret_cast<float4*>(xyzt_rows);
    const int64_t n_chunks = cdiv(M, IDX_CHUNK);
    NMF_REQUIRE(workspace_bytes >= nmf_bounce_index_workspace_bytes(M), NMF_EINVAL, "nmf_bounce_index: workspace too small");
    NMF_REQUIRE(n_chunks <= (1 << 22), NMF_ERANGE, "nmf_bounce_index: M too large");
    int64_t* chunk = static_cast<int64_t*>(workspace);
    NMF_REQUIRE(!M_live || n_chunks <= IDX_CHUNK, NMF_ERANGE, "nmf_bounce_index: bound too large for a device-side count (M_live)");
    NMF_LAUNCH(k_idx_partial, dim3((unsigned)n_chunks), dim3(IDX_CHUNK), 0, st, counts, M, chunk, M_live, sel);
    if (n_chunks <= IDX_CHUNK) {
        NMF_LAUNCH(k_idx_final_fused, dim3((unsigned)n_chunks), dim3(IDX_CHUNK), 0, st, counts, M, chunk,
                           (int)n_chunks, totals, bidx, row_off, cnt_rows, inv, x4, r4, pub, publish_seq, M_live, sel);
    } else {
        NMF_LAUNCH(k_idx_top, dim3(1), dim3(IDX_CHUNK), 0, st, chunk, (int)n_chunks, totals);
        NMF_LAUNCH(k_idx_final, dim3((unsigned)n_chunks), dim3(IDX_CHUNK), 0, st, counts, M, chunk, totals, bidx,
                           row_off, cnt_rows, inv, x4, r4);
    }
    NMF_CHECK_LAUNCH("nmf_bounce_index");
    if (pub && n_chunks > IDX_CHUNK) return nmf_publish_i64x2(totals, pub, publish_seq, stream);
    return NMF_OK;
}

static Conv load_conv(const float* conv) {
    Conv c;
    c.c = conv;
    return c;
}

extern "C" int nmf_bounce_prep_fwd(const int32_t* bidx, int64_t Mb, const float* normals, const float* app,
                                   const float* heads, const float* xyzt, const int32_t* ray_id, const float* rays,
                                   const float* conv, const float* feat_noise, float anoise, float min_rough,
                                   int32_t row_inputs, float* V, float* N, float* r1, float* f0, float* diffuse,
                                   float* feat, float* xyz, void* stream) {
    NMF_REQUIRE(Mb >= 0, NMF_EINVAL, "nmf_bounce_prep_fwd: Mb < 0");
    if (Mb == 0) return NMF_OK;
    NMF_REQUIRE(bidx && normals && app && heads && xyzt && ray_id && rays && conv && V && N && r1 && f0 &&
                    diffuse && feat && xyz, NMF_EINVAL, "nmf_bounce_prep_fwd: null");
    NMF_LAUNCH(k_bounce_prep_fwd, dim3((unsigned)cdiv(Mb, 256)), dim3(256), 0, (hipStream_t)stream, bidx, Mb,
                       normals, app, heads, reinterpret_cast<const float4*>(xyzt), ray_id, rays, load_conv(conv),
                       feat_noise, anoise, min_rough, (int)row_inputs, V, N, r1, f0, diffuse, feat, xyz,
                       HeadsIn{nullptr, nullptr, nmf_heads::HeadP{0.f, 0.f, 0.f, 0.f, 0.f}, nullptr});
    NMF_CHECK_LAUNCH("nmf_bounce_prep_fwd");
    return NMF_OK;
}

extern "C" int nmf_bounce_prep_fwd_heads(const int32_t* bidx, int64_t Mb, const float* normals, const float* app, const float* head_W,
                                         const float* head_b, float diffuse_mul, float diffuse_bias, float tint_bias, float f0_bias,
                                         float rough_bias, const float* xyzt, const int32_t* ray_id, const float* rays,
                                         const float* conv, const float* feat_noise, float anoise, float min_rough,
                                         int32_t row_inputs, float* heads_out, float* V, float* N, float* r1, float* f0,
                                         float* diffuse, float* feat, float* xyz, void* stream) {
    NMF_REQUIRE(Mb >= 0, NMF_EINVAL, "nmf_bounce_prep_fwd_heads: Mb < 0");
    if (Mb == 0) return NMF_OK;
    NMF_REQUIRE(row_inputs == 1 || row_inputs == 2, NMF_EINVAL, "nmf_bounce_prep_fwd_heads: app must be given per bounce row");
    NMF_REQUIRE(bidx && normals && app && head_W && head_b && heads_out && xyzt && ray_id && rays && conv && V && N && r1 && f0 &&
                    diffuse && feat && xyz, NMF_EINVAL, "nmf_bounce_prep_fwd_heads: null");
    NMF_LAUNCH(k_bounce_prep_fwd, dim3((unsigned)cdiv(Mb, 256)), dim3(256), 0, (hipStream_t)stream, bidx, Mb,
                       normals, app, heads_out, reinterpret_cast<const float4*>(xyzt), ray_id, rays, load_conv(conv),
                       feat_noise, anoise, min_rough, (int)row_inputs, V, N, r1, f0, diffuse, feat, xyz,
                       HeadsIn{head_W, head_b, nmf_heads::HeadP{diffuse_mul, diffuse_bias, tint_bias, f0_bias, rough_bias}, heads_out});
    NMF_CHECK_LAUNCH("nmf_bounce_prep_fwd_heads");
    return NMF_OK;
}

extern "C" int nmf_bounce_prep_bwd(const int32_t* inv, int64_t M, const int32_t* bidx, int64_t Mb, const float* normals,
                                   const float* heads, const int32_t* ray_id, const float* rays, const float* conv,
                                   float min_rough, int32_t detach_normals, int32_t row_inputs, const float* dN,
                                   const float* dr1, const float* df0,
                                   const float* ddiffuse, const int32_t row_strides[4], const float* dfeat,
                                   float* d_normals, float* d_heads, float* d_app, void* stream) {
    const int sN = row_strides ? row_strides[0] : 3, sr = row_strides ? row_strides[1] : 1;
    const int sf = row_strides ? row_strides[2] : 3, sd = row_strides ? row_strides[3] : 3;
    NMF_REQUIRE(M >= 0, NMF_EINVAL, "nmf_bounce_prep_bwd: M < 0");
    if (M == 0) return NMF_OK;
    NMF_REQUIRE((inv || row_inputs == 2) && normals && ray_id && rays && conv && d_normals, NMF_EINVAL,
                "nmf_bounce_prep_bwd: null");
    NMF_REQUIRE(Mb >= 0 && Mb <= M, NMF_EINVAL, "nmf_bounce_prep_bwd: Mb outside [0, M]");
    NMF_REQUIRE((row_inputs ? Mb == 0 : false) || (heads && d_heads && d_app), NMF_EINVAL, "nmf_bounce_prep_bwd: null");
    NMF_REQUIRE(!row_inputs || Mb == 0 || bidx, NMF_EINVAL, "nmf_bounce_prep_bwd: row_inputs needs bidx");
    const int64_t n_threads = row_inputs == 2 ? (Mb > 0 ? Mb : 1) : M;
    NMF_LAUNCH(k_bounce_prep_bwd, dim3((unsigned)cdiv(n_threads, 256)), dim3(256), 0, (hipStream_t)stream, inv, M, bidx,
                       Mb, normals, heads, ray_id, rays, load_conv(conv), min_rough, (int)detach_normals, (int)row_inputs,
                       dN, dr1, df0, ddiffuse, sN, sr, sf, sd, dfeat, d_normals, d_heads, d_app);
    NMF_CHECK_LAUNCH("nmf_bounce_prep_bwd");
    return NMF_OK;
}

extern "C" int nmf_ray_compose_fwd(const float* weight, const float* refl_rows, const int32_t* inv, const float* normals,
                                   const float* rays, const int64_t* offsets, int64_t B, const float* bg,
                                   int32_t bg_per_ray, int32_t tonemap, int32_t noclip, float* rgb_map, float* acc,
                                   float* rgb_lin, float* ori, void* stream) {
    NMF_REQUIRE(B >= 0, NMF_EINVAL, "nmf_ray_compose_fwd: B < 0");
    if (B == 0) return NMF_OK;
    NMF_REQUIRE(rays && offsets && bg && rgb_map && acc && rgb_lin, NMF_EINVAL, "nmf_ray_compose_fwd: null");
    NMF_REQUIRE(!ori || normals || !weight, NMF_EINVAL, "nmf_ray_compose_fwd: ori needs normals");
    if (B <= 16384)
        NMF_LAUNCH(k_ray_compose_fwd_wave<64>, dim3((unsigned)cdiv(B, 4)), dim3(256), 0, (hipStream_t)stream, weight,
                           refl_rows, inv, normals, rays, offsets, B, bg, (int)bg_per_ray, (int)tonemap, (int)noclip,
                           rgb_map, acc, rgb_lin, ori);
    else
        NMF_LAUNCH(k_ray_compose_fwd_wave<8>, dim3((unsigned)cdiv(B, 32)), dim3(256), 0, (hipStream_t)stream, weight,
                           refl_rows, inv, normals, rays, offsets, B, bg, (int)bg_per_ray, (int)tonemap, (int)noclip,
                           rgb_map, acc, rgb_lin, ori);
    NMF_CHECK_LAUNCH("nmf_ray_compose_fwd");
    return NMF_OK;
}

extern "C" int nmf_ray_compose_bwd(const float* weight, const float* refl_rows, const int32_t* inv, const float* normals,
                                   const float* rays, const int32_t* ray_id, int64_t M, const float* bg,
                                   int32_t bg_per_ray, int32_t tonemap, int32_t noclip, const float* rgb_lin,
                                   const float* d_rgb_map, const float* d_acc, const float* d_ori, float* d_weight,
                                   float* d_refl, float* d_normals, void* stream) {
    NMF_REQUIRE(M >= 0, NMF_EINVAL, "nmf_ray_compose_bwd: M < 0");
    if (M == 0) return NMF_OK;
    NMF_REQUIRE(weight && rays && ray_id && bg && rgb_lin && d_weight, NMF_EINVAL, "nmf_ray_compose_bwd: null");
    NMF_REQUIRE(!(inv && refl_rows) || d_refl, NMF_EINVAL, "nmf_ray_compose_bwd: d_refl missing");
    NMF_REQUIRE(!d_ori || normals, NMF_EINVAL, "nmf_ray_compose_bwd: d_ori needs normals");
    NMF_LAUNCH(k_ray_compose_bwd, dim3((unsigned)cdiv(M, 256)), dim3(256), 0, (hipStream_t)stream, weight,
                       refl_rows, inv, normals, rays, ray_id, M, bg, (int)bg_per_ray, (int)tonemap, (int)noclip, rgb_lin,
                       d_rgb_map, d_acc, d_ori, d_weight, d_refl, d_normals);
    NMF_CHECK_LAUNCH("nmf_ray_compose_bwd");
    return NMF_OK;
}

extern "C" int nmf_bg_adjoint(const float* acc, const float* d_rgb_map, int64_t B, float* d_bg, void* stream) {
    NMF_REQUIRE(B >= 0, NMF_EINVAL, "nmf_bg_adjoint: B < 0");
    if (B == 0) return NMF_OK;
    NMF_REQUIRE(acc && d_rgb_map && d_bg, NMF_EINVAL, "nmf_bg_adjoint: null");
    NMF_LAUNCH(k_bg_adjoint, dim3((unsigned)cdiv(3 * B, 256)), dim3(256), 0, (hipStream_t)stream, acc, d_rgb_map, 3 * B,
                       d_bg);
    NMF_CHECK_LAUNCH("nmf_bg_adjoint");
    return NMF_OK;
}
```

### nmf_amd/csrc/step_core.inc

```

struct UnsupportedChunk : std::runtime_error { using std::runtime_error::runtime_error; };

struct RuntimeEvent {
    void* ev = nullptr;
    RuntimeEvent() {}
    void* get() {
        if (!ev) check(nmf_event_create(&ev), "nmf_event_create");
        return ev;
    }
    ~RuntimeEvent() { if (ev) nmf_event_destroy(ev); }
    RuntimeEvent(const RuntimeEvent&) = delete;
    RuntimeEvent& operator=(const RuntimeEvent&) = delete;
};

struct SizeReadback {
    void* host = nullptr;
    void* dev = nullptr;
    int64_t seq = 0;
    ~SizeReadback() { if (host) nmf_host_free_mapped(host); }
    std::pair<int64_t, int64_t> arm() {
        if (!host) check(nmf_host_alloc_mapped(&host, &dev, 64), "nmf_host_alloc_mapped");
        ++seq;
        return {reinterpret_cast<int64_t>(dev), seq};
    }
    static double& waited_us() { static double w = 0.0; return w; }
    static double* waited_by_slot() { static double w[4] = {0, 0, 0, 0}; return w; }
    static int& slot() { static int s = 0; return s; }
    std::pair<int64_t, int64_t> get() {
        struct Acc {
            std::chrono::steady_clock::time_point t0 = std::chrono::steady_clock::now();
            ~Acc() {
                const double us = std::chrono::duration<double, std::micro>(std::chrono::steady_clock::now() - t0).count();
                waited_us() += us;
                waited_by_slot()[slot() & 3] += us;
                ++slot();
            }
        } acc;
        py::gil_scoped_release nogil;
        check(nmf_wait_seq(host, seq, 30.0), "nmf_wait_seq");
        const int64_t* p = static_cast<const int64_t*>(host);
        return {p[0], p[1]};
    }
};

struct CoreSamples {
    Tensor xyzt, ray_id, step_id, dist, offsets, whole_valid, rays, valid;
    OT jitter, z;
    int64_t M = 0, b = 0, N = 0;
    int64_t live = 0;
    SizeReadback* live_rb = nullptr;
};

struct CoreLevel {
    int lvl = 0;
    CoreSamples S;
    int64_t B = 0, M = 0, R = 0, Mb = 0;
    std::vector<int64_t> n_samples;
    Tensor offsets, sf, sg, w, conv, bidx, row_off, cnt32, inv, row_of_ray, j_of_ray, off, xyz_rows, app, heads;
    Tensor V, N, r1, f0, diff, feat, L, hl, dl, lpdf, mip, brays, incoming, bg, refl, rgb_map, acc, rgb_lin;
    OT gr, nr, brdf, brdf_mask, idx_re, idx_no, brays_re, mip_re, brays_no, mip_no, sf_rows, gr_rows, ori, rough;
    std::unique_ptr<CoreLevel> child;
    bool sparse_n = false, per_ray_bg = false;
};

class StepCore {
  public:
    int64_t main_stream = 0;
    std::vector<int64_t> side_streams;
    py::object set_stream, main_stream_obj;
    std::vector<py::object> side_stream_objs;
    bool overlap = true, sparse_normals = true;
    int64_t mlp_side_min_rays = 100000, mlp_side_min_env_rays = 200000, mlp_side_wgs_env = 256, walk_side_min_samples = 200000,
            mlp_side_wgs = 256, env_binned_from = 30000;
    int64_t vm_p = 0;
    std::vector<Tensor> dpk, dlk, apl, ali;
    std::vector<Tensor> f_dpk, f_dlk, f_apl, f_ali;
    std::vector<Tensor> dpl, dli;
    Tensor basis;
    std::vector<double> head_p;
    Tensor head_W, head_b;
    std::vector<Tensor> mlp_ws;
    Tensor mlp_image;
    double mlp_bias = 0.0;
    Tensor sobol;
    Tensor env_table, env_pole, env_sc, env_act, env_bg, sh_conv;
    int64_t march_p0 = 0, march_p1 = 0, max_samples = -1;
    OT alpha_bits, alpha_coarse;
    double scale = 25.0, anoise = 0.25, min_rough = 0.0, rays_per_ray = 128.0, test_rays_per_ray = 128.0;
    bool detach_n = false;
    std::vector<int64_t> max_brdf_rays, max_retrace_rays;
    Tensor white, one, select_ws;
    std::vector<Tensor> g_dpk, g_dlk, g_apl, g_ali, g_mlp;
    Tensor g_basis, g_hW, g_hb, d_sat, d_pole, d_mip;
    OT d_bg_out;
    int64_t wait_tables = 0, wait_env = 0;
    bool used_env = false, early_env_done = false;
    bool env_split = true;
    int64_t env_split_min_lookups = 16384;
    bool env_keep_sat = false;
    py::object early_cb = py::none();
    int64_t comm_stream = 0;
    std::vector<int64_t> peer_streams;
    py::dict train_forward(const Tensor& rays, double focal, py::object noise) {
        if (n_edits_ > 0) throw py::value_error("material edits are set: they are an evaluation feature and never enter a gradient "
                                                "(set_material_edits(None) before training)");
        pending_.reset();
        begin(noise);
        auto t = fwd(0, rays, focal, OT(), noise, true);
        py::dict out;
        out["kept"] = t->B;
        if (t->M == 0) {
            out["n_samples"] = std::vector<int64_t>{0};
            keep_.clear();
            return out;
        }
        out["n_samples"] = t->n_samples;
        {
            std::vector<int64_t> nr, nb;
            for (CoreLevel* l = t.get(); l; l = l->child.get()) { nr.push_back(l->R); nb.push_back(l->Mb); }
            out["n_rays"] = nr;
            out["n_rows"] = nb;
        }
        out["rgb_map"] = t->rgb_map;
        out["acc"] = t->acc;
        out["ori"] = *t->ori;
        out["whole_valid"] = t->S.whole_valid;
        pending_ = std::move(t);
        pending_keep_ = std::move(keep_);
        keep_.clear();
        return out;
    }
    bool has_pending() const { return (bool)pending_; }
    void train_backward(const Tensor& d_rgb, const OT& d_acc, const OT& d_ori, bool last) {
        if (!pending_) throw std::runtime_error("train_backward without a pending train_forward (the chunk was superseded by another forward)");
        std::unique_ptr<CoreLevel> t = std::move(pending_);
        keep_ = std::move(pending_keep_);
        pending_keep_.clear();
        dens_segs_.clear();
        app_segs_.clear();
        walk_forks_.clear();
        walk_clean_i_ = 0;
        last_chunk_ = last;
        bwd(*t, d_rgb.contiguous(), d_acc, d_ori);
        const bool early = last && comm_stream && !early_cb.is_none();
        if (early) {
            void* ev = next_ev();
            check(nmf_event_record(ev, st(main_stream)), "nmf_event_record");
            check(nmf_stream_wait_event(st(comm_stream), ev), "nmf_stream_wait_event");
            if (early_env_done && early_env_side_) {
                void* ev2 = next_ev();
                check(nmf_event_record(ev2, st(early_env_side_)), "nmf_event_record");
                check(nmf_stream_wait_event(st(comm_stream), ev2), "nmf_stream_wait_event");
            }
            for (int64_t ps : peer_streams)
                if (ps != main_stream) side_waits_for(comm_stream, ps);
        }
        flush_walks();
        if (early) early_cb();
    }

    py::dict chunk(const Tensor& rays, const Tensor& gt, double focal, py::object noise, double inv_lbatch,
                   const std::vector<double>& wts, bool want_total, bool last, py::object l1_fn) {
        py::dict out = train_forward(rays, focal, noise);
        if (!pending_) {
            out["loss"] = py::none();
            return out;
        }
        CoreLevel* t = pending_.get();
        const int64_t b = t->rgb_map.size(0);
        Tensor gt_b = gt.narrow(0, 0, b).contiguous();
        Tensor loss, d_rgb, d_acc, d_ori;
        if (wts.size() == 4 && t->rgb_map.is_contiguous() && b == t->B) {
            if (!loss_ws_.defined() || loss_ws_.numel() < nmf_loss_head_workspace_bytes(b) || loss_ws_.device() != rays.device())
                loss_ws_ = at::zeros({std::max<int64_t>(2 * nmf_loss_head_workspace_bytes(b), 4096)}, rays.options().dtype(at::kByte));
            std::tie(loss, d_rgb, d_ori, d_acc) =
                loss_head(t->rgb_map, gt_b, one, inv_lbatch, wts[0], wts[2], wts[3], loss_ws_, main_stream);
        } else {
            loss = sqerr_fwd(t->rgb_map, gt_b, main_stream);
            std::vector<std::vector<int64_t>> shapes = {{}, {}, {t->B}, {t->B}};
            std::vector<Tensor> dl = loss_mix_bwd(shapes, wts, inv_lbatch, one, main_stream);
            d_rgb = sqerr_bwd(t->rgb_map, gt_b, dl[0], main_stream);
            d_ori = dl[2]; d_acc = dl[3];
        }
        out["total"] = py::none();
        if (want_total) out["total"] = l1_fn(loss, *t->ori, t->acc);
        train_backward(d_rgb, d_acc, d_ori, last);
        out["loss"] = loss;
        return out;
    }

    py::object render(const Tensor& rays, double focal, py::object noise, bool want_maps, bool want_materials = false,
                      bool want_linear = false) {
        begin(noise);
        eval_z_ = want_maps;
        std::unique_ptr<CoreLevel> t;
        try {
            t = fwd(0, rays, focal, OT(), noise, false);
        } catch (...) {
            eval_z_ = false;
            throw;
        }
        eval_z_ = false;
        if (t->M == 0) return py::none();
        py::dict out;
        out["rgb_map"] = t->rgb_map;
        out["acc"] = t->acc;
        out["kept"] = t->B;
        out["n_samples"] = t->n_samples;
        if (want_materials) out["materials"] = material_maps_(*t);
        if (want_linear) out["rgb_lin"] = t->rgb_lin;
        if (want_maps) {
            if (!t->S.z.has_value() || !t->nr.has_value()) throw UnsupportedChunk("evaluation maps need the sampler's z values and dense normals");
            out["depth"] = segment_sum(t->S.z->view({t->M, 1}), OT(t->w), t->offsets, t->B, 1, main_stream).view({t->B});
            Tensor wn = segment_sum(*t->nr, OT(t->w), t->offsets, t->B, 1, main_stream);
            Tensor a = t->acc.unsqueeze(1);
            out["world_normal"] = a * wn + (1.0 - a);
        }
        return out;
    }

    void set_material_edits(const OT& table) {
        if (!table.has_value() || !table->defined() || table->numel() == 0) {
            edits_ = Tensor();
            n_edits_ = 0;
            return;
        }
        if (table->dim() != 2 || table->size(1) != NMF_EDIT_ROW || table->scalar_type() != at::kFloat)
            throw py::value_error("set_material_edits: the table is fp32 [K,32]");
        if (table->size(0) > NMF_EDIT_MAX) throw py::value_error("set_material_edits: at most 16 edits");
        edits_ = table->detach().to(at::kCPU).contiguous().clone();
        n_edits_ = edits_.size(0);
    }
    int64_t n_material_edits() const { return n_edits_; }

  private:
    Tensor edits_;
    int64_t n_edits_ = 0;
    Tensor material_maps_(CoreLevel& t) {
        if (!t.nr.has_value() || t.sparse_n || t.lvl != 0)
            throw UnsupportedChunk("material maps need the dense normals of level 0");
        if (!t.brdf.has_value() || !t.incoming.defined() || t.incoming.size(0) != t.R || !t.conv.defined() || !head_W.defined())
            throw UnsupportedChunk("material maps need the bounce rows' incoming radiance and BRDF weights");
        const int64_t M = t.M, B = t.B;
        Tensor xyzt = t.S.xyzt.narrow(0, 0, M).contiguous();
        Tensor app = *std::get<4>(vm_query_fwd(vm_p, xyzt, fw(f_dpk, dpk), fw(f_dlk, dlk), fw(f_apl, apl), fw(f_ali, ali), basis, false,
                                               false, true, false, main_stream));
        Tensor rays = t.S.rays.narrow(0, 0, B).contiguous();
        Tensor nr = t.nr->contiguous(), w = t.w.contiguous(), inv = t.inv.narrow(0, 0, M).contiguous();
        Tensor incoming = t.incoming.contiguous(), brdf = t.brdf->contiguous(), conv = t.conv.contiguous();
        Tensor maps = material_maps(app, nr, w, t.offsets.contiguous(), rays, head_W, head_b, head_p, conv, inv, t.row_off.contiguous(),
                                    t.cnt32.contiguous(), incoming, brdf, t.acc.contiguous(), t.bg.contiguous(), main_stream, OT(xyzt),
// ... 310 lines not shown
            t->sf = t->sf.narrow(0, 0, Ml); t->sg = t->sg.narrow(0, 0, Ml); t->w = t->w.narrow(0, 0, Ml);
            if (t->gr.has_value()) t->gr = t->gr->narrow(0, 0, Ml);
            if (t->nr.has_value()) t->nr = t->nr->narrow(0, 0, Ml);
            t->inv = t->inv.narrow(0, 0, Ml);
        }
        if (R == 0) {
            env_ready();
            throw UnsupportedChunk("no bounce rows");
        }
        t->R = R; t->Mb = Mb;
        t->bidx = t->bidx.narrow(0, 0, Mb); t->row_off = t->row_off.narrow(0, 0, Mb + 1); t->cnt32 = t->cnt32.narrow(0, 0, Mb);
        std::tie(t->row_of_ray, t->j_of_ray) = expand_segments(t->row_off, Mb, R, main_stream);
        t->off = uniform(noise, {Mb, 1, 2}).reshape({Mb, 2}).contiguous();
        t->xyz_rows = xyz_rows.narrow(0, 0, Mb);
        OT feat_noise;
        {
            py::object fn = noise.attr("rows")(deferred, t->bidx);
            if (!fn.is_none()) feat_noise = fn.cast<Tensor>();
        }
        if (sparse_n) {
            Tensor sfr, grr, nrr;
            std::tie(sfr, grr, nrr) = vm_query_rows(vm_p, t->xyz_rows, fw(f_dpk, dpk), fw(f_dlk, dlk), main_stream);
            t->sf_rows = sfr; t->gr_rows = grr; t->nr = nrr;
        }
        t->app = *std::get<4>(vm_query_fwd(vm_p, t->xyz_rows, fw(f_dpk, dpk), fw(f_dlk, dlk), fw(f_apl, apl), fw(f_ali, ali), basis, false,
                                           false, true, false, main_stream));
        Tensor xyz;
        env_ready();
        if (!is_train && n_edits_ > 0) {
            t->heads = heads_fwd(t->app, head_W, head_b, head_p, main_stream);
            heads_edit(t->heads, t->xyz_rows, edits_, main_stream);
            std::tie(t->V, t->N, t->r1, t->f0, t->diff, t->feat, xyz) =
                bounce_prep_fwd(t->bidx, *t->nr, t->app, t->heads, S.xyzt, S.ray_id, S.rays, t->conv, feat_noise, anoise, -1e30,
                                sparse_n ? 2 : 1, main_stream);
        } else {
            std::tie(t->heads, t->V, t->N, t->r1, t->f0, t->diff, t->feat, xyz) =
                bounce_prep_fwd_heads(t->bidx, *t->nr, t->app, head_W, head_b, head_p, S.xyzt, S.ray_id, S.rays, t->conv, feat_noise,
                                      anoise, is_train ? min_rough : -1e30, sparse_n ? 2 : 1, main_stream);
        }
        std::tie(t->L, t->hl, t->dl, t->lpdf, t->mip, t->brays) =
            ggx_rays_fwd(t->V, t->N, t->r1, xyz, t->off, t->cnt32, sobol, t->row_of_ray, t->j_of_ray, main_stream);
        const bool has_retrace = lvl < (int)max_retrace_rays.size();
        const bool sorts = !pins_.is_none() && pins_.attr("sorts")(lvl).cast<bool>();
        const int64_t num_retrace = has_retrace ? std::min<int64_t>(R, max_retrace_rays[lvl]) : 0;
        const bool full_retrace = has_retrace && num_retrace >= R && !sorts;
        auto mlp = [&]() {
            Tensor o, mk;
            std::tie(o, mk) = brdf_mlp_fwd(mlp_ws, t->hl, t->dl, t->feat, t->r1, t->row_of_ray, mlp_bias, is_train, 0, main_stream, mlp_img());
            t->brdf = o;
            if (is_train) t->brdf_mask = mk;
        };
        if (!full_retrace) mlp();
        if (has_retrace) {
            if (full_retrace) {
                skip(noise, "rand", {R});
                t->child = fwd(lvl + 1, t->brays, focal, t->mip, noise, is_train, mlp);
                if (t->child->M == 0) throw UnsupportedChunk("no secondary sample");
                t->n_samples.insert(t->n_samples.end(), t->child->n_samples.begin(), t->child->n_samples.end());
                t->incoming = t->child->rgb_map;
            } else {
                Tensor w_rows = at::index_select(t->w, 0, t->bidx);
                Tensor cc = retrace_scores_(*t->brdf, t->V, t->N, t->lpdf, w_rows, t->cnt32, t->row_of_ray);
                cc = cc / cc.sum() * (double)num_retrace;
                cc = cc + uniform(noise, {R});
                const int64_t cut = std::max<int64_t>(R - num_retrace, 0);
                if (pins_.is_none()) {
                    Tensor top, rest;
                    std::tie(top, rest) = topk_select_(cc.contiguous(), R - cut);
                    t->idx_re = top.to(at::kLong);
                    t->idx_no = rest.to(at::kLong);
                } else {
                    Tensor order = argsort_(cc.contiguous()).to(at::kLong);
                    trace_put("retrace_order_own" + std::to_string(lvl), order);
                    py::dict ro = pins_.attr("retrace_order").cast<py::dict>();
                    if (ro.contains(py::int_(lvl))) order = ro[py::int_(lvl)].cast<Tensor>().to(order.device());
                    t->idx_re = order.narrow(0, cut, R - cut);
                    t->idx_no = order.narrow(0, 0, cut);
                    trace_put("retrace_score" + std::to_string(lvl), cc);
                    trace_put("retrace_order" + std::to_string(lvl), order);
                    trace_put("retrace_idx" + std::to_string(lvl), *t->idx_re);
                }
                t->incoming = at::empty({R, 3}, rays.options().dtype(at::kFloat));
                if (t->idx_re->size(0) > 0) {
                    t->brays_re = at::index_select(t->brays, 0, *t->idx_re);
                    t->mip_re = at::index_select(t->mip, 0, *t->idx_re);
                    t->child = fwd(lvl + 1, *t->brays_re, focal, t->mip_re, noise, is_train);
                    if (t->child->M == 0) throw UnsupportedChunk("no secondary sample");
                    t->n_samples.insert(t->n_samples.end(), t->child->n_samples.begin(), t->child->n_samples.end());
                    t->incoming.index_copy_(0, *t->idx_re, t->child->rgb_map);
                }
                if (t->idx_no->size(0) > 0) {
                    t->brays_no = at::index_select(t->brays, 0, *t->idx_no);
                    t->mip_no = at::index_select(t->mip, 0, *t->idx_no);
                    skip(noise, "rand", {t->idx_no->size(0)});
                    skip(noise, "rand", {t->idx_no->size(0)});
                    t->incoming.index_copy_(0, *t->idx_no, env_fwd(*t->brays_no, *t->mip_no));
                }
            }
        } else {
            skip(noise, "rand", {R});
            skip(noise, "rand", {R});
            t->incoming = env_fwd(t->brays, t->mip);
        }
        if (per_ray_bg) {
            skip(noise, "rand", {B});
            skip(noise, "rand", {B});
        }
        Tensor contrib = shade_mix_fwd(t->V, t->f0, t->diff, t->cnt32, t->row_of_ray, t->L, t->incoming, *t->brdf, main_stream);
        t->refl = segment_sum(contrib, OT(), t->row_off, Mb, 8, main_stream);
        std::tie(t->rgb_map, t->acc, t->rgb_lin, t->ori) =
            ray_compose_fwd(t->w, t->refl, t->inv, lvl == 0 ? t->nr : OT(), S.rays, t->offsets, B, t->bg, per_ray_bg, lvl == 0, false,
                            lvl == 0, main_stream);
        if (!trace_.is_none()) {
            const std::string s = std::to_string(lvl);
            trace_put("rgb_map" + s, t->rgb_map); trace_put("acc_map" + s, t->acc); trace_put("whole_valid" + s, S.whole_valid);
            trace_put("incoming" + s, t->incoming);
            if (t->ori.has_value()) trace_put("ori" + s, *t->ori);
        }
        return t;
    }

    Tensor retrace_scores_(const Tensor& brdf, const Tensor& V, const Tensor& N, const Tensor& lpdf, const Tensor& w_rows,
                           const Tensor& cnt, const Tensor& row_of_ray) {
        const int64_t R = row_of_ray.size(0);
        Tensor o = fe(V, {R});
        check(nmf_retrace_scores(f32(brdf), f32(V), f32(N), f32(lpdf), f32(w_rows), i32(cnt), i32(row_of_ray), R, out(o), st(main_stream)),
              "nmf_retrace_scores");
        return o;
    }
    std::pair<Tensor, Tensor> topk_select_(const Tensor& keys, int64_t k) {
        const int64_t n = keys.size(0);
        Tensor top = ie(keys, {k}, at::kInt), rest = ie(keys, {n - k}, at::kInt);
        const int64_t nbytes = nmf_topk_select_workspace_bytes(n);
        Tensor ws = ie(keys, {(nbytes + 7) / 8}, at::kLong);
        check(nmf_topk_select(f32(keys), n, k, k ? static_cast<int32_t*>(top.data_ptr()) : nullptr,
                              n - k ? static_cast<int32_t*>(rest.data_ptr()) : nullptr, ws.data_ptr(), nbytes, st(main_stream)),
              "nmf_topk_select");
        return {top, rest};
    }
    Tensor argsort_(const Tensor& keys) {
        const int64_t n = keys.size(0);
        Tensor idx = ie(keys, {n}, at::kInt);
        const int64_t nbytes = nmf_argsort_workspace_bytes(n);
        Tensor ws = ie(keys, {(nbytes + 7) / 8}, at::kLong);
        check(nmf_argsort_f32(f32(keys), n, static_cast<int32_t*>(idx.data_ptr()), ws.data_ptr(), nbytes, st(main_stream)),
              "nmf_argsort_f32");
        return idx;
    }

    Tensor bwd(CoreLevel& t, const Tensor& d_rgb, const OT& d_acc, const OT& d_ori) {
        CoreSamples& S = t.S;
        const int lvl = t.lvl;
        const bool view = lvl > 0;
        Tensor d_w;
        OT d_refl, d_nrm;
        std::tie(d_w, d_refl, d_nrm) =
            ray_compose_bwd(t.w, t.refl, t.inv, d_ori.has_value() ? t.nr : OT(), S.rays, S.ray_id, t.bg, t.per_ray_bg, lvl == 0, false,
                            t.rgb_lin, d_rgb, d_acc, d_ori, d_ori.has_value(), main_stream);
        Tensor d_sigma = composite_bwd(t.sg, S.dist, t.w, t.offsets, t.B, scale, d_w, main_stream);
        bool early_walk = false;
        if (t.sparse_n && t.M >= walk_side_min_samples) {
            const int64_t ws = fork(4);
            if (ws) {
                std::vector<Seg> segs = {Seg(S.xyzt, t.sf, OT(), d_sigma, OT(), OT(), OT())};
                walk_segments(segs, OT(), ws);
                end_side();
                walk_forks_.push_back(ws);
                keep_.push_back(d_sigma);
                keep_.push_back(d_w);
                early_walk = true;
            }
        }
        Tensor d_rays;
        int64_t env_side = 0;
        if (t.per_ray_bg) {
            Tensor d_bg = bg_adjoint(t.acc, d_rgb, main_stream);
            Tensor env_rows = t.B == S.rays.size(0) ? S.rays : S.rays.narrow(0, 0, t.B);
            env_side = t.B >= mlp_side_min_rays ? fork(2 + (lvl > 0 ? 1 : 0)) : 0;
            d_rays = env_bwd(env_rows, *t.rough, d_bg, env_side ? env_side : main_stream);
            if (env_side) end_side();
            keep_.push_back(d_bg);
        }
        Tensor d_inc, d_brdf, dL, d_fd, dV, dV_rows;
        if (view) {
            std::tie(d_inc, d_brdf, dL, d_fd, dV) =
                shade_mix_bwd_view(t.V, t.f0, t.diff, t.cnt32, t.row_of_ray, t.L, t.incoming, *t.brdf, *d_refl, main_stream);
            dV_rows = segment_sum(dV, OT(), t.row_off, t.Mb, 8, main_stream);
        } else {
            std::tie(d_inc, d_brdf, dL, d_fd) =
                shade_mix_bwd(t.V, t.f0, t.diff, t.cnt32, t.row_of_ray, t.L, t.incoming, *t.brdf, *d_refl, main_stream);
        }
        Tensor rows6 = segment_sum_wide(d_fd, 6, t.row_off, t.Mb, main_stream);
        const int64_t n_re = t.idx_re.has_value() ? t.idx_re->size(0) : (t.child ? t.R : 0);
        const int64_t n_env = t.R - n_re;
        const bool below = t.child && t.child->B >= mlp_side_min_rays;
        Tensor d_feat;
        bool have_feat = false;
        const int64_t mlp_side = (below || n_env >= mlp_side_min_env_rays) ? fork(lvl > 0 ? 1 : 0) : 0;
        if (mlp_side) {
            d_feat = brdf_mlp_bwd(mlp_ws, t.hl, t.dl, t.feat, t.r1, t.row_of_ray, *t.brdf, *t.brdf_mask, d_brdf, g_mlp,
                                   below ? mlp_side_wgs : mlp_side_wgs_env, mlp_side, mlp_img());
            end_side();
            have_feat = true;
            keep_.push_back(d_brdf);
        }
        Tensor d_brays;
        if (!t.idx_re.has_value() && t.child) {
            d_brays = bwd(*t.child, d_inc, OT(), OT());
        } else if (!t.idx_re.has_value()) {
            d_brays = env_bwd(t.brays, t.mip, d_inc, main_stream);
        } else {
            d_brays = at::empty_like(t.brays);
            if (t.idx_re->size(0) > 0)
                d_brays.index_copy_(0, *t.idx_re, bwd(*t.child, at::index_select(d_inc, 0, *t.idx_re), OT(), OT()));
            if (t.idx_no->size(0) > 0)
                d_brays.index_copy_(0, *t.idx_no, env_bwd(*t.brays_no, *t.mip_no, at::index_select(d_inc, 0, *t.idx_no), main_stream));
        }
        if (lvl == 0 && last_chunk_ && used_env && d_bg_out.has_value()) {
            const int64_t ss = fork(5);
            if (ss) {
                for (int64_t es : env_streams_)
                    if (es != ss) side_waits_for(ss, es);
                for (int64_t ps : peer_streams)
                    if (ps != main_stream) side_waits_for(ss, ps);
                Tensor ds = env_keep_sat ? d_sat.clone() : d_sat;
                sat_build_bwd_into(ds, env_bg, env_act, d_pole, 0.0, 1.0, env_sc, *d_bg_out, ss);
                if (env_keep_sat) keep_.push_back(ds);
                end_side();
                early_env_side_ = ss;
                early_env_done = true;
            }
        }
        if (mlp_side) join(mlp_side, {d_feat});
        if (!have_feat)
            d_feat = brdf_mlp_bwd(mlp_ws, t.hl, t.dl, t.feat, t.r1, t.row_of_ray, *t.brdf, *t.brdf_mask, d_brdf, g_mlp, 0, main_stream, mlp_img());
        Tensor dN, dr1, dV_ggx;
        if (view) {
            Tensor d_nrv = ggx_rays_bwd_view(t.V, t.N, t.r1, t.off, sobol, t.row_of_ray, t.j_of_ray, dL, d_brays, main_stream);
            Tensor rows7 = segment_sum_wide(d_nrv, 7, t.row_off, t.Mb, main_stream);
            dN = rows7.slice(1, 0, 3); dr1 = rows7.select(1, 3); dV_ggx = rows7.slice(1, 4, 7);
        } else {
            Tensor d_nr = ggx_rays_bwd(t.V, t.N, t.r1, t.off, sobol, t.row_of_ray, t.j_of_ray, dL, d_brays, main_stream);
            Tensor rows4 = segment_sum(d_nr, OT(), t.row_off, t.Mb, 8, main_stream);
            dN = rows4.slice(1, 0, 3); dr1 = rows4.select(1, 3);
        }
        Tensor d_normals, d_heads, d_app;
        if (t.sparse_n) {
            std::tie(d_normals, d_app) =
                bounce_prep_heads_bwd(t.bidx, *t.nr, t.heads, S.ray_id, S.rays, t.conv, min_rough, detach_n, dN, dr1, rows6.slice(1, 0, 3),
                                      rows6.slice(1, 3, 6), d_feat, t.app, head_W, head_b, head_p, g_hW, g_hb, main_stream);
        } else {
            std::tie(d_normals, d_heads, d_app) =
                bounce_prep_bwd(OT(t.inv), *t.nr, t.heads, S.ray_id, S.rays, t.conv, min_rough, detach_n, dN, dr1,
                                rows6.slice(1, 0, 3), rows6.slice(1, 3, 6), d_feat, t.bidx, 1, main_stream);
            d_app = heads_bwd(t.app, head_W, head_b, head_p, d_heads, g_hW, g_hb, OT(d_app), main_stream);
        }
        app_segs_.push_back(Seg(t.xyz_rows, OT(), OT(), OT(), OT(), OT(), d_app));
        OT d_normal;
        if (detach_n) d_normal = d_nrm;
        else if (d_nrm.has_value()) d_normal = d_normals.add_(*d_nrm);
        else d_normal = d_normals;
        if (t.sparse_n) {
            if (!early_walk) dens_segs_.push_back(Seg(S.xyzt, t.sf, OT(), d_sigma, OT(), OT(), OT()));
            if (d_normal.has_value())
                dens_segs_.push_back(Seg(t.xyz_rows, *t.sf_rows, *t.gr_rows, zero_like(*t.sf_rows), OT(), *d_normal, OT()));
        } else {
            dens_segs_.push_back(Seg(S.xyzt, t.sf, t.gr, d_sigma, OT(), d_normal, OT()));
        }
        if (env_side) join(env_side, {d_rays});
        if (view) {
            if (!d_rays.defined()) d_rays = at::zeros_like(S.rays);
            view_adjoint_to_rays(S.ray_id, t.bidx, dV_rows, dV_ggx, d_rays, main_stream);
        }
        return d_rays;
    }

    int64_t early_env_side_ = 0;
    Tensor zeros_, loss_ws_;
    Tensor zero_like(const Tensor& x) {
        const int64_t n = x.numel();
        if (!zeros_.defined() || zeros_.numel() < n || zeros_.device() != x.device())
            zeros_ = at::zeros({std::max<int64_t>(2 * n, 1 << 16)}, x.options().dtype(at::kFloat));
        return zeros_.narrow(0, 0, n).view(x.sizes());
    }

  public:
    void join_env_table_backward() {
        if (early_env_done && early_env_side_) join(early_env_side_);
        early_env_done = false;
        early_env_side_ = 0;
    }

  private:
    static std::vector<bool> seg_key(const Seg& s) {
        return {std::get<3>(s).has_value(), std::get<4>(s).has_value(), std::get<5>(s).has_value(), std::get<6>(s).has_value()};
    }
    void walk(std::vector<Seg>& all, const OT& gb, int64_t stream) {
        std::vector<std::vector<bool>> keys;
        for (auto& s : all) {
            auto k = seg_key(s);
            if (std::find(keys.begin(), keys.end(), k) == keys.end()) keys.push_back(k);
        }
        for (auto& k : keys) {
            std::vector<Seg> segs;
            for (auto& s : all)
                if (seg_key(s) == k) segs.push_back(s);
            for (size_t i = 0; i < segs.size(); i += NMF_VM_MAX_SEGMENTS) {
                std::vector<Seg> part(segs.begin() + i, segs.begin() + std::min(segs.size(), i + (size_t)NMF_VM_MAX_SEGMENTS));
                walk_segments(part, gb, stream);
            }
        }
    }
    void flush_walks() {
        walk(dens_segs_, OT(), main_stream);
        walk(app_segs_, g_basis, main_stream);
        for (int64_t s : walk_forks_) join(s);
        walk_forks_.clear();
        dens_segs_.clear();
        app_segs_.clear();
        keep_.clear();
    }
};
```

### nmf_amd/hip.py

```python
import ctypes as C
import importlib.util
import os

import numpy as np
import torch

_HERE = os.path.dirname(os.path.abspath(__file__))
LIB_PATH = os.environ.get("NMF_HIP_LIB") or os.path.join(_HERE, "lib", "libnmf_hip.so")
HOST_EXT_PATH = os.path.join(_HERE, "lib", "_nmf_host.so")
_BUILD_HINT = "build it with `python -c 'import __graft_entry__ as g; g.build()'` (or nmf_amd/csrc/build.sh)"


class NmfHipError(RuntimeError):
    pass


def _load():
    if not os.path.exists(LIB_PATH):
        raise NmfHipError(f"{LIB_PATH} not found: {_BUILD_HINT}.  nmf_amd has no CPU fallback.")
    return C.CDLL(LIB_PATH)


def _load_host():
    if not os.path.exists(HOST_EXT_PATH):
        raise NmfHipError(f"{HOST_EXT_PATH} not found: {_BUILD_HINT}.  nmf_amd has no CPU fallback.")
    spec = importlib.util.spec_from_file_location("_nmf_host", HOST_EXT_PATH)
    mod = importlib.util.module_from_spec(spec)
    try:
        spec.loader.exec_module(mod)
    except ImportError as e:
        raise NmfHipError(f"{HOST_EXT_PATH} does not load ({e}): {_BUILD_HINT}") from e
    if mod.abi_version() != _lib.nmf_version():
        raise NmfHipError(f"{HOST_EXT_PATH} was built against ABI version {mod.abi_version()}, {LIB_PATH} is version "
                          f"{_lib.nmf_version()}: {_BUILD_HINT}")
    mod.set_error_class(NmfHipError)
    return mod


_lib = _load()
HOST_EXT = _load_host()


class MarchParams(C.Structure):
    _fields_ = [("aabb_min", C.c_float * 3), ("aabb_max", C.c_float * 3), ("alpha_inv", C.c_float * 3),
                ("stepsize", C.c_float), ("half_step", C.c_float), ("near_t", C.c_float), ("far_t", C.c_float),
                ("focal", C.c_float), ("n_steps", C.c_int32), ("grid", C.c_int32 * 3), ("is_train", C.c_int32),
                ("seed", C.c_uint64), ("offset", C.c_uint64), ("occ_min", C.c_float * 3), ("occ_max", C.c_float * 3)]


class VmParams(C.Structure):
    _fields_ = [("aabb_min", C.c_float * 3), ("inv_size", C.c_float * 3), ("density_shift", C.c_float),
                ("grid", C.c_int32), ("stencil", C.c_float * 5), ("stencil_off", C.c_float * 5)]


class AdamSlot(C.Structure):
    _fields_ = [("param", C.c_void_p), ("grad", C.c_void_p), ("exp_avg", C.c_void_p), ("exp_avg_sq", C.c_void_p),
                ("numel", C.c_int64), ("beta1", C.c_double), ("beta2", C.c_double), ("eps", C.c_double),
                ("weight_decay", C.c_double), ("step_size", C.c_double), ("bc2_sqrt", C.c_double),
                ("is_f64", C.c_int32), ("reserved", C.c_int32)]


class CopySlot(C.Structure):
    _fields_ = [("src", C.c_void_p), ("dst", C.c_void_p), ("numel", C.c_int64), ("src_is_f64", C.c_int32),
                ("dst_is_f64", C.c_int32)]


EXPORTS = [
    "nmf_version", "nmf_last_error_string", "nmf_event_create", "nmf_event_create_timed", "nmf_event_elapsed_ms", "nmf_event_destroy", "nmf_event_record", "nmf_event_synchronize",
    "nmf_stream_wait_event", "nmf_host_alloc_mapped", "nmf_host_free_mapped", "nmf_publish_i64x2", "nmf_wait_seq", "nmf_set_launch_probe", "nmf_alpha_pack", "nmf_march_count", "nmf_march_scan", "nmf_march_scan_workspace_bytes",
    "nmf_march_fill", "nmf_march_dense", "nmf_vm_pack_density", "nmf_vm_query_fwd", "nmf_vm_query_rows", "nmf_vm_query_sigma", "nmf_sat_lookup_bwd_dirs",
    "nmf_vm_unpack_density_grad", "nmf_vm_bwd_workspace_bytes", "nmf_composite_fwd", "nmf_composite_bwd", "nmf_segment_sum",
    "nmf_sat_build", "nmf_sat_build_bwd", "nmf_sat_lookup_fwd", "nmf_sat_lookup_bwd", "nmf_sat_lookup_bwd_binned",
    "nmf_sat_lookup_bwd_workspace_bytes",
    "nmf_select_bounces", "nmf_select_total", "nmf_view_adjoint_to_rays", "nmf_expand_segments", "nmf_segment_sum_wide",
    "nmf_brdf_mlp_fwd", "nmf_brdf_mlp_image_bytes", "nmf_brdf_mlp_pack",
    "nmf_brdf_mlp_bwd_segments", "nmf_brdf_mlp_bwd_segments_workspace_bytes", "nmf_heads_fwd", "nmf_heads_bwd", "nmf_ggx_rays_fwd", "nmf_ggx_rays_bwd", "nmf_ggx_rays_bwd_view", "nmf_ggx_prob", "nmf_shade_mix_fwd", "nmf_shade_mix_bwd", "nmf_shade_mix_bwd_view",
    "nmf_adam_step", "nmf_bounce_index", "nmf_bounce_index_workspace_bytes", "nmf_bounce_prep_fwd", "nmf_bounce_prep_bwd",
    "nmf_ray_compose_fwd", "nmf_ray_compose_bwd", "nmf_l1_mean_fwd", "nmf_l1_mean_bwd", "nmf_sqerr_fwd", "nmf_sqerr_bwd",
    "nmf_loss_mix_fwd", "nmf_loss_mix_bwd", "nmf_loss_head", "nmf_loss_head_workspace_bytes", "nmf_bg_adjoint", "nmf_vm_query_bwd_segments", "nmf_vm_bwd_clean_bytes", "nmf_sh_project",
    "nmf_retrace_scores", "nmf_argsort_f32", "nmf_argsort_workspace_bytes", "nmf_topk_select", "nmf_topk_select_workspace_bytes", "nmf_alpha_coarse", "nmf_alpha_coarse_words", "nmf_bounce_index_select", "nmf_bounce_prep_fwd_heads", "nmf_bounce_prep_heads_bwd", "nmf_multi_copy",
    "nmf_ssim", "nmf_ssim_workspace_bytes", "nmf_normal_err", "nmf_normal_err_workspace_bytes",
    "nmf_material_maps", "nmf_material_maps_edit", "nmf_heads_edit",
    "nmf_mc_count", "nmf_mc_emit", "nmf_mc_workspace_bytes", "nmf_mc_case_triangles",
    "nmf_tv_fwd_bwd", "nmf_tv_workspace_bytes",
    "nmf_env_resample",
    "nmf_relight_frame", "nmf_relight_ratio", "nmf_relight_ratio_workspace_bytes", "nmf_relight_adjust",
    "nmf_relight_adjust_workspace_bytes",
    "nmf_camera_rays", "nmf_frame_finish",
    "nmf_atlas_texels", "nmf_atlas_store",
    "nmf_rays_place", "nmf_merge_rank", "nmf_merge_scatter",
]
for _n in EXPORTS:
    if not hasattr(_lib, _n):
        raise NmfHipError(f"libnmf_hip.so does not export {_n}")


def _declare_from_header():
    import re
    hdr = os.path.join(os.path.dirname(_HERE), "include", "nmf_hip.h")
    if not os.path.exists(hdr):
        raise NmfHipError(f"{hdr} is missing: the C-ABI prototypes of libnmf_hip.so are read from it (keep include/ next "
                          "to the nmf_amd package)")
    text = re.sub(r"/\*.*?\*/", " ", open(hdr).read(), flags=re.S)
    text = re.sub(r"//[^\n]*", " ", text)
    scal = {"int64_t": C.c_int64, "int32_t": C.c_int32, "int": C.c_int32, "uint64_t": C.c_uint64, "uint32_t": C.c_uint32,
            "float": C.c_float, "double": C.c_double}
    for ret, name, args in re.findall(r"\b(int64_t|int|const char\s*\*)\s+(nmf_\w+)\s*\(([^;{}]*?)\)\s*;", text):
        fn = getattr(_lib, name, None)
        if fn is None:
            continue
        fn.restype = C.c_int64 if ret == "int64_t" else (C.c_char_p if "char" in ret else C.c_int)
        types = []
        args = re.sub(r"\(\s*\*\s*(\w+)\s*\)\s*\([^)]*\)", r"*\1", args)
        for a in [x.strip() for x in args.split(",")]:
            if a in ("void", ""):
                continue
            if "*" in a or "[" in a:
                types.append(C.c_void_p)
            else:
                tok = [t for t in a.replace("const", " ").split() if t in scal]
                if not tok:
                    raise NmfHipError(f"cannot derive the ctypes type of '{a}' in {name}")
                types.append(scal[tok[0]])
        fn.argtypes = types


_declare_from_header()


def version():
    return _lib.nmf_version()


def _check(code, what):
    if code != 0:
        raise NmfHipError(f"{what} failed: {_lib.nmf_last_error_string().decode()} [{code}]")


def _stream():
    return torch._C._cuda_getCurrentRawStream(torch._C._cuda_getDevice())


def _p(t, dtype=None):
    if t is None:
        return None
    if dtype is not None and t.dtype != dtype:
        raise NmfHipError(f"expected {dtype}, got {t.dtype}")
    if not t.is_cuda:
        raise NmfHipError("nmf_amd operators need device tensors (no CPU path)")
    if not t.is_contiguous():
        raise NmfHipError("tensor must be contiguous")
    return t.data_ptr() or None


def channels_last_ptr_ok(t):
    _, Cn, H, W = t.shape
    return t.stride(1) == 1 and t.stride(3) == Cn and t.stride(2) == W * Cn


_host_mirror = {}


def host(t):
    if not isinstance(t, torch.Tensor):
        return np.asarray(t)
    if not t.is_cuda:
        return t.detach().numpy()
    key = (t.data_ptr(), t._version, tuple(t.shape), t.dtype)
    v = _host_mirror.get(id(t))
    if v is None or v[0] != key:
        if len(_host_mirror) > 256:
            _host_mirror.clear()
        v = (key, t.detach().cpu().numpy(), t)
        _host_mirror[id(t)] = v
    return v[1]


class Readback:
    _ring = {}

    def __init__(self):
        self.pin = torch.empty(4, dtype=torch.int64).pin_memory()
        self.ev = torch.cuda.Event()
        self.n = 0

    @classmethod
    def of(cls, dev):
        r = cls._ring.setdefault(str(dev), [[cls() for _ in range(4)], 0])
        r[1] = (r[1] + 1) & 3
        return r[0][r[1]]

    def start(self, t):
        self.n = t.numel()
        self.pin[: self.n].copy_(t, non_blocking=True)
        self.ev.record()
        return self

    def get(self):
        self.ev.synchronize()
        return self.pin[: self.n].tolist()


def march_params(aabb, alpha_inv, stepsize, near, far, focal, n_steps, grid, is_train, seed=0, offset=0, occ_box=None):
    p = MarchParams()
    if occ_box is not None:
        p.occ_min[:] = [float(v) for v in occ_box[0]]
        p.occ_max[:] = [float(v) for v in occ_box[1]]
    else:
        p.occ_min[:] = [1.0, 1.0, 1.0]
        p.occ_max[:] = [-1.0, -1.0, -1.0]
    a = host(aabb).astype(np.float32)
    p.aabb_min[:] = a[0].tolist()
    p.aabb_max[:] = a[1].tolist()
    p.alpha_inv[:] = np.asarray(alpha_inv, dtype=np.float32).tolist() if alpha_inv is not None else [0, 0, 0]
    st = np.float32(stepsize)
    p.stepsize = float(st)
    p.half_step = float(np.float32(st / np.float32(2)))
    p.near_t = float(np.float32(near))
    p.far_t = float(np.float32(far))
    p.focal = float(np.float32(focal))
    p.n_steps = int(n_steps)
    p.grid[:] = [int(g) for g in grid] if grid is not None else [0, 0, 0]
    p.is_train = 1 if is_train else 0
    p.seed = int(seed)
    p.offset = int(offset)
    return p


def alpha_pack(volume):
    n = volume.numel()
    bits = torch.zeros((n + 31) // 32, dtype=torch.int32, device=volume.device)
    _check(_lib.nmf_alpha_pack(_p(volume.contiguous(), torch.float32), C.c_int64(n), _p(bits), _stream()), "nmf_alpha_pack")
    return bits


def alpha_coarse(bits, grid):
    g = (C.c_int32 * 3)(*[int(v) for v in grid])
    words = _lib.nmf_alpha_coarse_words(g)
    coarse = torch.zeros(max(words, 1), dtype=torch.int32, device=bits.device)
    _check(_lib.nmf_alpha_coarse(_p(bits, torch.int32), g, _p(coarse), _stream()), "nmf_alpha_coarse")
    return coarse


# ... 235 lines not shown
    r = HOST_EXT.brdf_mlp_fwd(list(weights or ()), half_vec, diff_vec, feat_src, rough_src, src_idx, out_bias, bool(with_mask),
                              int(max_workgroups), _stream(), image)
    return r if with_mask else r[0]


def brdf_mlp_bwd(weights, half_vec, diff_vec, feat_src, rough_src, src_idx, fwd_out, act_mask, d_out, grads, max_workgroups=0,
                 image=None):
    return HOST_EXT.brdf_mlp_bwd(list(weights or ()), half_vec, diff_vec, feat_src, rough_src, src_idx, fwd_out, act_mask, d_out,
                                 list(grads), int(max_workgroups), _stream(), image)


def brdf_mlp_bwd_segments(weights, sets, grads, max_workgroups=0, image=None):
    return HOST_EXT.brdf_mlp_bwd_sets(list(weights or ()), list(sets), list(grads), int(max_workgroups), _stream(), image)


def heads_fwd(feat, W, b, hp):
    return HOST_EXT.heads_fwd(feat, W, b, list(hp), _stream())


def heads_bwd(feat, W, b, hp, d_out, gW, gb, add_into=None):
    return HOST_EXT.heads_bwd(feat, W, b, list(hp), d_out, gW, gb, add_into, _stream())


def ggx_rays_fwd(V, N, r, x, off, cnt, sobol, row_of_ray, j_of_ray):
    return HOST_EXT.ggx_rays_fwd(V, N, r, x, off, cnt, sobol, row_of_ray, j_of_ray, _stream())


def ggx_prob(dir_in, dir_out, half, rough):
    R = dir_in.shape[0]
    out = torch.empty((R,), dtype=torch.float32, device=dir_in.device)
    _check(_lib.nmf_ggx_prob(_p(dir_in, torch.float32), _p(dir_out, torch.float32), _p(half, torch.float32),
                             _p(rough, torch.float32), C.c_int64(R), _p(out), _stream()), "nmf_ggx_prob")
    return out


def ggx_rays_bwd(V, N, r, off, sobol, row_of_ray, j_of_ray, dL, d_rays=None):
    return HOST_EXT.ggx_rays_bwd(V, N, r, off, sobol, row_of_ray, j_of_ray, dL, d_rays, _stream())


def ggx_rays_bwd_view(V, N, r, off, sobol, row_of_ray, j_of_ray, dL, d_rays=None):
    return HOST_EXT.ggx_rays_bwd_view(V, N, r, off, sobol, row_of_ray, j_of_ray, dL, d_rays, _stream())


def shade_mix_bwd_view(V, f0, diff, cnt, row_of_ray, L, inc, brdf, d_rows):
    return HOST_EXT.shade_mix_bwd_view(V, f0, diff, cnt, row_of_ray, L, inc, brdf, d_rows, _stream())


def shade_mix_fwd(V, f0, diff, cnt, row_of_ray, L, inc, brdf):
    return HOST_EXT.shade_mix_fwd(V, f0, diff, cnt, row_of_ray, L, inc, brdf, _stream())


def shade_mix_bwd(V, f0, diff, cnt, row_of_ray, L, inc, brdf, d_rows):
    return HOST_EXT.shade_mix_bwd(V, f0, diff, cnt, row_of_ray, L, inc, brdf, d_rows, _stream())


def adam_step(slots, n, guard=None):
    return HOST_EXT.adam_step(C.addressof(slots), int(n), guard, _stream())


def bounce_index(counts, xyzt=None):
    return HOST_EXT.bounce_index(counts, xyzt, _stream())


def bounce_prep_fwd_heads(bidx, normals, app, head_W, head_b, hp, xyzt, ray_id, rays, conv, feat_noise, anoise, min_rough, row_inputs=1):
    return HOST_EXT.bounce_prep_fwd_heads(bidx, normals, app, head_W, head_b, list(hp), xyzt, ray_id, rays, conv, feat_noise, anoise,
                                          min_rough, int(row_inputs), _stream())


def bounce_index_select(weights, u, mode, mul, add=0.0, sum_w=1.0, xyzt=None):
    dev_sum = sum_w if isinstance(sum_w, torch.Tensor) else None
    return HOST_EXT.bounce_index_select(weights, u, mode, mul, add, 1.0 if dev_sum is not None else sum_w, dev_sum, xyzt, _stream())


def bounce_prep_fwd(bidx, normals, app, heads, xyzt, ray_id, rays, conv, feat_noise, anoise, min_rough, row_inputs=False):
    return HOST_EXT.bounce_prep_fwd(bidx, normals, app, heads, xyzt, ray_id, rays, conv, feat_noise, anoise, min_rough,
                                    int(row_inputs), _stream())


def bounce_prep_bwd(inv, normals, heads, ray_id, rays, conv, min_rough, detach_n, dN, dr1, df0, ddiff, dfeat,
                    bidx=None, row_inputs=False):
    return HOST_EXT.bounce_prep_bwd(inv, normals, heads, ray_id, rays, conv, float(min_rough), bool(detach_n), dN, dr1, df0, ddiff,
                                    dfeat, bidx, int(row_inputs), _stream())


def ray_compose_fwd(weight, refl_rows, inv, normals, rays, offsets, B, bg, bg_per_ray, tonemap, noclip, want_ori):
    return HOST_EXT.ray_compose_fwd(weight, refl_rows, inv, normals, rays, offsets, B, bg, bool(bg_per_ray), bool(tonemap),
                                    bool(noclip), bool(want_ori), _stream())


def ray_compose_bwd(weight, refl_rows, inv, normals, rays, ray_id, bg, bg_per_ray, tonemap, noclip, rgb_lin, d_rgb_map,
                    d_acc, d_ori, want_d_normals):
    return HOST_EXT.ray_compose_bwd(weight, refl_rows, inv, normals, rays, ray_id, bg, bool(bg_per_ray), bool(tonemap),
                                    bool(noclip), rgb_lin, d_rgb_map, d_acc, d_ori, bool(want_d_normals), _stream())


def _dense_f32(t):
    if t.dtype != torch.float32 or not t.is_cuda:
        raise NmfHipError("expected a float32 device tensor")
    if not (t.is_contiguous() or t.is_contiguous(memory_format=torch.channels_last)):
        raise NmfHipError("tensor storage must be dense")
    return t.data_ptr()


def l1_mean_fwd(tensors):
    n = len(tensors)
    out = torch.zeros((), dtype=torch.float32, device=tensors[0].device)
    ptrs = (C.c_void_p * n)(*[_dense_f32(t) for t in tensors])
    numel = (C.c_int64 * n)(*[t.numel() for t in tensors])
    _check(_lib.nmf_l1_mean_fwd(ptrs, numel, C.c_int32(n), _p(out), _stream()), "nmf_l1_mean_fwd")
    return out


def l1_mean_bwd(tensors, d_out, out=None):
    if out is None:
        grads = [torch.empty_like(t, memory_format=torch.preserve_format) for t in tensors]
        HOST_EXT.l1_mean_bwd_into(list(tensors), d_out, grads, False, _stream())
        return grads
    HOST_EXT.l1_mean_bwd_into(list(tensors), d_out, list(out), True, _stream())
    return out


def loss_mix_fwd(tensors, weights, scale):
    n = len(tensors)
    out = torch.zeros((), dtype=torch.float32, device=tensors[0].device)
    ptrs = (C.c_void_p * n)(*[_dense_f32(t) for t in tensors])
    numel = (C.c_int64 * n)(*[t.numel() for t in tensors])
    w = (C.c_float * n)(*[float(v) for v in weights])
    _check(_lib.nmf_loss_mix_fwd(ptrs, numel, w, C.c_int32(n), C.c_float(scale), _p(out), _stream()), "nmf_loss_mix_fwd")
    return out


def loss_mix_bwd(shapes, weights, scale, d_out):
    return HOST_EXT.loss_mix_bwd([list(s_) for s_ in shapes], [float(v) for v in weights], float(scale), d_out, _stream())


_loss_ws = {}


def loss_head_workspace(device, n_rays):
    key = (device, _stream())
    need = int(_lib.nmf_loss_head_workspace_bytes(C.c_int64(n_rays)))
    ws = _loss_ws.get(key)
    if ws is None or ws.numel() < need:
        ws = _loss_ws[key] = torch.zeros(max(2 * need, 4096), dtype=torch.uint8, device=device)
    return ws


def loss_head(pred, gt, d_out, scale, w_pred, w_a, w_b):
    return HOST_EXT.loss_head(pred, gt, d_out, scale, w_pred, w_a, w_b, loss_head_workspace(pred.device, pred.shape[0]), _stream())


def bg_adjoint(acc, d_rgb):
    return HOST_EXT.bg_adjoint(acc, d_rgb, _stream())


def sqerr_fwd(pred, gt):
    return HOST_EXT.sqerr_fwd(pred, gt, _stream())


def sqerr_bwd(pred, gt, d_out):
    return HOST_EXT.sqerr_bwd(pred, gt, d_out, _stream())


TV_KINDS = {"plane": 0, "line": 1, "env": 2}
_tv_ws = {}
_tv_scale = {}


def tv_kind(t):
    return "line" if t.shape[-1] == 1 else "plane"


def _tv_launch(tensors, kinds, weights, scale, grads, want_value):
    n = len(tensors)
    if not (n == len(kinds) == len(weights)) or (grads is not None and len(grads) != n):
        raise NmfHipError("tv: tensors / kinds / weights / grads differ in length")
    dev = tensors[0].device
    shape, xs, gs = (C.c_int32 * (3 * n))(), (C.c_int64 * (3 * n))(), (C.c_int64 * (3 * n))()
    for i, t in enumerate(tensors):
        g = grads[i] if grads is not None else None
        for u in (t, g):
            if u is None:
                continue
            if u.dtype != torch.float32 or not u.is_cuda or u.device != dev:
                raise NmfHipError("tv: expected float32 tensors on one device")
            if u.dim() not in (3, 4) or (u.dim() == 4 and u.shape[0] != 1) or (u is g and u.shape[-3:] != t.shape[-3:]):
                raise NmfHipError("tv: tensors are [1,C,H,W] (or [C,H,W]) and a gradient has its tensor's shape")
        shape[3 * i:3 * i + 3] = list(t.shape[-3:])
        xs[3 * i:3 * i + 3] = list(t.stride()[-3:])
        if g is not None:
            gs[3 * i:3 * i + 3] = list(g.stride()[-3:])
    kind = (C.c_int32 * n)(*[TV_KINDS[k] if isinstance(k, str) else int(k) for k in kinds])
    w = (C.c_float * n)(*[float(v) for v in weights])
    if not isinstance(scale, torch.Tensor):
        key = (dev, float(scale))
        if key not in _tv_scale:
            if len(_tv_scale) > 64:
                _tv_scale.clear()
            _tv_scale[key] = torch.full((), float(scale), dtype=torch.float32, device=dev)
        scale = _tv_scale[key]
    if scale.numel() != 1:
        raise NmfHipError("tv: the scale is a single device value")
    value, ws, ws_bytes = None, None, 0
    if want_value:
        need = int(_lib.nmf_tv_workspace_bytes(shape, kind, C.c_int32(n)))
        _check(min(need, 0), "nmf_tv_workspace_bytes")
        wkey = (dev, _stream())
        ws = _tv_ws.get(wkey)
        if ws is None or ws.numel() < need:
            ws = _tv_ws[wkey] = torch.zeros(max(2 * need, 4096), dtype=torch.uint8, device=dev)
        ws_bytes = ws.numel()
        value = torch.empty((), dtype=torch.float32, device=dev)
    ptrs = (C.c_void_p * n)(*[t.data_ptr() for t in tensors])
    gptrs = (C.c_void_p * n)(*[g.data_ptr() for g in grads]) if grads is not None else None
    _check(_lib.nmf_tv_fwd_bwd(ptrs, gptrs, shape, xs, gs if grads is not None else None, kind, w, C.c_int32(n),
                               _p(scale.reshape(()), torch.float32), _p(value), None if ws is None else C.c_void_p(ws.data_ptr()),
                               C.c_int64(ws_bytes), _stream()), "nmf_tv_fwd_bwd")
    return value


def tv_value_grad(tensors, kinds, weights, scale, grads=None, value=True):
    tensors = [t.detach() for t in tensors]
    if grads is None:
        grads = [torch.zeros_like(t, memory_format=torch.preserve_format) for t in tensors]
    return _tv_launch(tensors, kinds, weights, scale, list(grads), bool(value)), grads


def tv_value(tensors, kinds, weights, scale):
    return _tv_launch([t.detach() for t in tensors], kinds, weights, scale, None, True)


def retrace_scores(brdf, V_rows, N_rows, lpdf, w_rows, cnt_rows, row_of_ray):
    R = row_of_ray.shape[0]
    score = torch.empty(R, dtype=torch.float32, device=brdf.device)
    if R:
        _check(_lib.nmf_retrace_scores(_p(brdf, torch.float32), _p(V_rows, torch.float32), _p(N_rows, torch.float32),
                                       _p(lpdf, torch.float32), _p(w_rows, torch.float32), _p(cnt_rows, torch.int32),
                                       _p(row_of_ray, torch.int32), C.c_int64(R), _p(score), _stream()),
               "nmf_retrace_scores")
    return score


def argsort_f32(keys):
    n = keys.shape[0]
    order = torch.empty(n, dtype=torch.int32, device=keys.device)
    if n:
        nbytes = _lib.nmf_argsort_workspace_bytes(C.c_int64(n))
        ws = torch.empty(nbytes, dtype=torch.uint8, device=keys.device)
        _check(_lib.nmf_argsort_f32(_p(keys, torch.float32), C.c_int64(n), _p(order), _p(ws), C.c_int64(nbytes),
                                    _stream()), "nmf_argsort_f32")
    return order


def topk_select(keys, k):
    n = keys.shape[0]
    k = int(k)
    top = torch.empty(k, dtype=torch.int32, device=keys.device)
    rest = torch.empty(n - k, dtype=torch.int32, device=keys.device)
    if n:
        nbytes = _lib.nmf_topk_select_workspace_bytes(C.c_int64(n))
        ws = torch.empty(nbytes, dtype=torch.uint8, device=keys.device)
        _check(_lib.nmf_topk_select(_p(keys, torch.float32), C.c_int64(n), C.c_int64(k), _p(top) if k else None,
                                    _p(rest) if n - k else None, _p(ws), C.c_int64(nbytes), _stream()), "nmf_topk_select")
    return top, rest


def multi_copy(slots, n):
    return HOST_EXT.multi_copy(C.addressof(slots), int(n), _stream())


def ssim_taps(filter_size=11, filter_sigma=1.5):
    hw = filter_size // 2
    shift = (2 * hw - filter_size + 1) / 2
    f_i = ((np.arange(filter_size) - hw + shift) / filter_sigma) ** 2
    filt = np.exp(-0.5 * f_i)
    return filt / np.sum(filt)


def _batched(t, tail):
    t = t.reshape(-1, *t.shape[-tail:]) if t.dim() > tail else t.unsqueeze(0)
    return t.contiguous()


def ssim(a, b, max_val=1.0, k1=0.01, k2=0.03, return_map=False, filter_sigma=1.5):
    if a.shape != b.shape or a.dim() not in (3, 4):
        raise NmfHipError(f"ssim: images must have equal shapes [H,W,3] or [n,H,W,3], got {tuple(a.shape)} / {tuple(b.shape)}")
    A, B = _batched(a, 3), _batched(b, 3)
    n, H, W, Cn = A.shape
    taps = (C.c_double * 11)(*ssim_taps(11, filter_sigma))
    mean = torch.empty(n, dtype=torch.float64, device=A.device)
    smap = torch.empty((n, max(H - 10, 0), max(W - 10, 0), Cn), dtype=torch.float32, device=A.device) if return_map else None
    nbytes = int(_lib.nmf_ssim_workspace_bytes(C.c_int64(n), C.c_int32(H), C.c_int32(W), C.c_int32(Cn)))
    ws = torch.empty(max(nbytes, 8), dtype=torch.uint8, device=A.device)
    _check(_lib.nmf_ssim(_p(A, torch.float32), _p(B, torch.float32), C.c_int64(n), C.c_int32(H), C.c_int32(W), C.c_int32(Cn),
                         C.addressof(taps), C.c_double((k1 * max_val) ** 2), C.c_double((k2 * max_val) ** 2), _p(mean),
                         _p(smap), _p(ws), C.c_int64(ws.numel()), _stream()), "nmf_ssim")
    return (mean, smap) if return_map else mean


def normal_err(pred, gt, acc, return_map=False):
    if pred.shape != gt.shape or pred.dim() not in (2, 3) or pred.shape[-1] != 3 or pred.shape[:-1] != acc.shape:
        raise NmfHipError(f"normal_err: shapes {tuple(pred.shape)} / {tuple(gt.shape)} / {tuple(acc.shape)}")
    n = pred.shape[0] if pred.dim() == 3 else 1
    P, G, Acc = pred.reshape(n, -1, 3).contiguous(), gt.reshape(n, -1, 3).contiguous(), acc.reshape(n, -1).contiguous()
    n_px = P.shape[1]
    out = torch.empty(n, dtype=torch.float64, device=P.device)
# ... 301 lines not shown
```

Measured before the change: 2.952 million rays/s.

## Fuse backward kernels: bg adjoint into compose, paired segment sums, dense normal accumulation

Adds fused entry points to the backward step. The background adjoint is computed inside the ray-compose backward kernel. The two row segment sums (dV and d_fd) run in one launch. The heads backward writes normal gradients straight into the dense d_normals buffer, which removes a separate bounce_prep_bwd/heads_bwd pair and an add. The MLP side-stream join also moves later so more work overlaps. Each change is behind a flag that defaults to on; the cost is extra code paths and a risk of ordering mistakes in the dense accumulation.

```diff
diff --git a/include/nmf_hip.h b/include/nmf_hip.h
--- a/include/nmf_hip.h
+++ b/include/nmf_hip.h
@@ -375,6 +375,21 @@
                       int32_t part, int64_t row_base, float* sigma_m, float* dist_m, float* z_m, float* normal_m, int32_t* ray_id_m,
                       int32_t* part_m, int32_t* src_m, int32_t* inv_m, void* stream);
 
+int nmf_bounce_prep_heads_bwd_dense(const int32_t* bidx, int64_t Mb, const float* normals, const float* heads,
+                                    const int32_t* ray_id, const float* rays, const float* conv, float min_rough,
+                                    const float* dN, const float* dr1, const float* df0, const float* ddiffuse,
+                                    const int32_t row_strides[4], const float* dfeat, const float* app,
+                                    const float* head_W, const float* head_b, float diffuse_mul, float diffuse_bias,
+                                    float tint_bias, float f0_bias, float rough_bias, float* d_normals_acc, float* d_app,
+                                    float* g_head_W, float* g_head_b, void* stream);
+int nmf_segment_sum_pair(const float* vals3, float* out3, const float* vals_wide, int64_t row_stride, int32_t D,
+                         float* out_wide, const int64_t* offsets, int64_t n_seg, void* stream);
+int nmf_ray_compose_bwd_bg(const float* weight, const float* refl_rows, const int32_t* inv, const float* normals,
+                           const float* rays, const int32_t* ray_id, int64_t M, const float* bg,
+                           int32_t bg_per_ray, int32_t tonemap, int32_t noclip, const float* rgb_lin,
+                           const float* d_rgb_map, const float* d_acc, const float* d_ori, float* d_weight,
+                           float* d_refl, float* d_normals, const float* acc, int64_t B, float* d_bg, void* stream);
+
 #ifdef __cplusplus
 }
 #endif
diff --git a/nmf_amd/csrc/brdf.hip b/nmf_amd/csrc/brdf.hip
--- a/nmf_amd/csrc/brdf.hip
+++ b/nmf_amd/csrc/brdf.hip
@@ -1,4 +1,5 @@
 #include "common.hpp"
+#include "segsum_wide.hpp"
 
 namespace {
 
@@ -10,25 +11,7 @@
                                                           float* __restrict__ out) {
     const int64_t s = (int64_t)blockIdx.x * 4 + (threadIdx.x >> 6);
     if (s >= n_seg) return;
-    const int lane = lane_id();
-    const int ch = lane & (G - 1), slot = lane / G;
-    constexpr int SLOTS = 64 / G;
-    const int64_t b = offsets[s], e = offsets[s + 1];
-    float a = 0.f;
-    if (ch < D) {
-        float a1 = 0.f, a2 = 0.f, a3 = 0.f;
-        int64_t r = b + slot;
-        for (; r + 3 * SLOTS < e; r += 4 * SLOTS) {
-            const float v0 = vals[r * stride + ch], v1 = vals[(r + SLOTS) * stride + ch];
-            const float v2 = vals[(r + 2 * SLOTS) * stride + ch], v3 = vals[(r + 3 * SLOTS) * stride + ch];
-            a += v0; a1 += v1; a2 += v2; a3 += v3;
-        }
-        for (; r < e; r += SLOTS) a += vals[r * stride + ch];
-        a = (a + a1) + (a2 + a3);
-    }
-#pragma unroll
-    for (int sh = 32; sh >= G; sh >>= 1) a += __shfl_down(a, sh, 64);
-    if (lane < D) out[s * D + lane] = a;
+    nmf_segsum::wide_segment<G>(vals, stride, D, offsets, s, out);
 }
 
 }
diff --git a/nmf_amd/csrc/composite.hip b/nmf_amd/csrc/composite.hip
--- a/nmf_amd/csrc/composite.hip
+++ b/nmf_amd/csrc/composite.hip
@@ -1,4 +1,5 @@
 #include "common.hpp"
+#include "segsum_wide.hpp"
 
 namespace {
 
@@ -161,10 +162,10 @@
 }
 
 template <int D, int W>
-__global__ void __launch_bounds__(256) k_segment_sum_group(const float* __restrict__ vals, const float* __restrict__ scale,
-                                                           const int64_t* __restrict__ offsets, int64_t n_seg,
-                                                           float* __restrict__ out) {
-    const int64_t r = ((int64_t)blockIdx.x * 256 + threadIdx.x) / W;
+__device__ __forceinline__ void segment_sum_group_block(int64_t block, const float* __restrict__ vals, const float* __restrict__ scale,
+                                                        const int64_t* __restrict__ offsets, int64_t n_seg,
+                                                        float* __restrict__ out) {
+    const int64_t r = (block * 256 + threadIdx.x) / W;
     const int lane = threadIdx.x & (W - 1);
     const bool ok = r < n_seg;
     const int64_t s = ok ? offsets[r] : 0, e = ok ? offsets[r + 1] : 0;
@@ -199,6 +200,25 @@
 #pragma unroll
         for (int d = 0; d < D; ++d) out[r * D + d] = a[d];
     }
+}
+template <int D, int W>
+__global__ void __launch_bounds__(256) k_segment_sum_group(const float* __restrict__ vals, const float* __restrict__ scale,
+                                                           const int64_t* __restrict__ offsets, int64_t n_seg,
+                                                           float* __restrict__ out) {
+    segment_sum_group_block<D, W>((int64_t)blockIdx.x, vals, scale, offsets, n_seg, out);
+}
+
+__global__ void __launch_bounds__(256) k_segment_sum_pair(const float* __restrict__ vals_a, float* __restrict__ out_a, unsigned blocks_a,
+                                                          const float* __restrict__ vals_b, int64_t stride_b, int D_b,
+                                                          float* __restrict__ out_b, const int64_t* __restrict__ offsets,
+                                                          int64_t n_seg) {
+    if (blockIdx.x < blocks_a) {
+        segment_sum_group_block<3, 8>((int64_t)blockIdx.x, vals_a, nullptr, offsets, n_seg, out_a);
+        return;
+    }
+    const int64_t s = (int64_t)(blockIdx.x - blocks_a) * 4 + (threadIdx.x >> 6);
+    if (s >= n_seg) return;
+    nmf_segsum::wide_segment<8>(vals_b, stride_b, D_b, offsets, s, out_b);
 }
 
 }
@@ -273,3 +293,16 @@
     NMF_CHECK_LAUNCH("nmf_segment_sum");
     return NMF_OK;
 }
+
+extern "C" int nmf_segment_sum_pair(const float* vals3, float* out3, const float* vals_wide, int64_t row_stride, int32_t D,
+                                    float* out_wide, const int64_t* offsets, int64_t n_seg, void* stream) {
+    NMF_REQUIRE(n_seg >= 0, NMF_EINVAL, "nmf_segment_sum_pair: n_seg < 0");
+    if (n_seg == 0) return NMF_OK;
+    NMF_REQUIRE(vals3 && out3 && vals_wide && out_wide && offsets, NMF_EINVAL, "nmf_segment_sum_pair: null");
+    NMF_REQUIRE(D > 0 && D <= 8 && row_stride >= D, NMF_ERANGE, "nmf_segment_sum_pair: the wide source has 1..8 columns");
+    const unsigned blocks_a = (unsigned)cdiv(n_seg, 32), blocks_b = (unsigned)cdiv(n_seg, 4);
+    NMF_LAUNCH(k_segment_sum_pair, dim3(blocks_a + blocks_b), dim3(256), 0, (hipStream_t)stream, vals3, out3, blocks_a, vals_wide,
+                       row_stride, (int)D, out_wide, offsets, n_seg);
+    NMF_CHECK_LAUNCH("nmf_segment_sum_pair");
+    return NMF_OK;
+}
diff --git a/nmf_amd/csrc/heads.hip b/nmf_amd/csrc/heads.hip
--- a/nmf_amd/csrc/heads.hip
+++ b/nmf_amd/csrc/heads.hip
@@ -193,3 +193,26 @@
     NMF_CHECK_LAUNCH("nmf_bounce_prep_heads_bwd");
     return NMF_OK;
 }
+
+extern "C" int nmf_bounce_prep_heads_bwd_dense(const int32_t* bidx, int64_t Mb, const float* normals, const float* heads,
+                                               const int32_t* ray_id, const float* rays, const float* conv, float min_rough,
+                                               const float* dN, const float* dr1, const float* df0, const float* ddiffuse,
+                                               const int32_t row_strides[4], const float* dfeat, const float* app,
+                                               const float* head_W, const float* head_b, float diffuse_mul, float diffuse_bias,
+                                               float tint_bias, float f0_bias, float rough_bias, float* d_normals_acc, float* d_app,
+                                               float* g_head_W, float* g_head_b, void* stream) {
+    NMF_REQUIRE(Mb >= 0, NMF_EINVAL, "nmf_bounce_prep_heads_bwd_dense: Mb < 0");
+    if (Mb == 0) return NMF_OK;
+    NMF_REQUIRE(bidx && normals && heads && ray_id && rays && conv && app && head_W && head_b && d_normals_acc && d_app && g_head_W &&
+                    g_head_b, NMF_EINVAL, "nmf_bounce_prep_heads_bwd_dense: null");
+    HeadP hp{diffuse_mul, diffuse_bias, tint_bias, f0_bias, rough_bias};
+    nmf_rows::RowsBwdIn rin{bidx, normals, heads, ray_id, rays, nmf_rows::Conv{conv}, min_rough, 0, dN, dr1, df0, ddiffuse,
+                            row_strides ? row_strides[0] : 3, row_strides ? row_strides[1] : 1, row_strides ? row_strides[2] : 3,
+                            row_strides ? row_strides[3] : 3, dfeat, nullptr, d_normals_acc};
+    const int64_t n_it = cdiv(Mb, 256);
+    const unsigned grid = (unsigned)(n_it < 1024 ? n_it : 1024);
+    NMF_LAUNCH(k_heads_bwd, dim3(grid), dim3(256), 0, (hipStream_t)stream, app, Mb, head_W, head_b, hp, nullptr, nullptr, d_app,
+                       g_head_W, g_head_b, rin);
+    NMF_CHECK_LAUNCH("nmf_bounce_prep_heads_bwd_dense");
+    return NMF_OK;
+}
diff --git a/nmf_amd/csrc/host_ext.cpp b/nmf_amd/csrc/host_ext.cpp
--- a/nmf_amd/csrc/host_ext.cpp
+++ b/nmf_amd/csrc/host_ext.cpp
@@ -945,6 +945,77 @@
               "nmf_bounce_prep_heads_bwd");
     }
     return {d_normals, d_app};
+}
+
+Tensor bounce_prep_heads_bwd_dense(const Tensor& bidx, const Tensor& normals, const Tensor& heads, const Tensor& ray_id,
+                                   const Tensor& rays, const Tensor& conv, double min_rough, const OT& dN, const OT& dr1,
+                                   const OT& df0, const OT& ddiff, const OT& dfeat, const Tensor& app, const Tensor& W,
+                                   const Tensor& b, const std::vector<double>& hp, const Tensor& gW, const Tensor& gb,
+                                   Tensor d_normals_acc, int64_t stream) {
+    TimedScope _ts("heads_bwd", stream);
+    if (hp.size() != 5) fail("bounce_prep_heads_bwd_dense: hp = (diffuse_mul, diffuse_bias, tint_bias, f0_bias, rough_bias)");
+    const int64_t Mb = bidx.size(0), M = normals.size(0);
+    if (d_normals_acc.dim() != 2 || d_normals_acc.size(0) != M || d_normals_acc.size(1) != 3 || !d_normals_acc.is_contiguous() ||
+        ray_id.size(0) != M || Mb > M)
+        fail("bounce_prep_heads_bwd_dense: normals / d_normals_acc [M,3] (contiguous), ray_id [M], bidx [Mb <= M] expected");
+    Tensor d_app = fe(normals, {Mb, 24});
+    if (Mb) {
+        std::vector<Tensor> keep;
+        const auto a = rows_of(dN, 3, keep), b2 = rows_of(dr1, 1, keep), c = rows_of(df0, 3, keep), d = rows_of(ddiff, 3, keep);
+        const int32_t strides[4] = {a.second, b2.second, c.second, d.second};
+        OT df;
+        if (dfeat.has_value()) df = dfeat->contiguous();
+        check(nmf_bounce_prep_heads_bwd_dense(i32(bidx), Mb, f32(normals), f32(heads), i32(ray_id), f32(rays), f32(conv), (float)min_rough,
+                                              a.first, b2.first, c.first, d.first, strides, of32(df), f32(app), f32(W), f32(b),
+                                              (float)hp[0], (float)hp[1], (float)hp[2], (float)hp[3], (float)hp[4],
+                                              ptr<float>(d_normals_acc, at::kFloat), out(d_app), static_cast<float*>(vptr(gW)),
+                                              static_cast<float*>(vptr(gb)), st(stream)),
+              "nmf_bounce_prep_heads_bwd_dense");
+    }
+    return d_app;
+}
+
+std::tuple<Tensor, Tensor> segment_sum_pair(const Tensor& vals3, const Tensor& vals_wide, int64_t D, const Tensor& offsets,
+                                            int64_t n_seg, int64_t stream) {
+    TimedScope _ts(__func__, stream);
+    if (vals3.dim() != 2 || vals3.size(1) != 3 || vals_wide.dim() != 2 || vals_wide.size(0) != vals3.size(0) || D < 1 || D > 8 ||
+        vals_wide.size(1) < D || offsets.size(0) < n_seg + 1)
+        fail("segment_sum_pair: vals3 [n,3], vals_wide [n,>=D] with D in 1..8 and offsets [n_seg+1] expected");
+    Tensor o3 = fe(vals3, {n_seg, 3}), ow = fe(vals3, {n_seg, D});
+    if (vals3.size(0) == 0) {
+        o3.zero_();
+        ow.zero_();
+        return {o3, ow};
+    }
+    check(nmf_segment_sum_pair(f32(vals3), out(o3), f32(vals_wide), vals_wide.size(1), (int32_t)D, out(ow), i64(offsets), n_seg,
+                               st(stream)),
+          "nmf_segment_sum_pair");
+    return {o3, ow};
+}
+
+std::tuple<Tensor, OT, OT, Tensor> ray_compose_bwd_bg(const Tensor& weight, const OT& refl_rows, const OT& inv, const OT& normals,
+                                                      const Tensor& rays, const Tensor& ray_id, const Tensor& bg, bool bg_per_ray,
+                                                      bool tonemap, bool noclip, const OT& rgb_lin, const Tensor& d_rgb_map,
+                                                      const OT& d_acc, const OT& d_ori, bool want_d_normals, const Tensor& acc,
+                                                      int64_t stream) {
+    TimedScope _ts("ray_compose_bwd", stream);
+    const int64_t M = weight.size(0), B = acc.size(0);
+    if (d_rgb_map.dim() != 2 || d_rgb_map.size(0) != B || d_rgb_map.size(1) != 3 || !d_rgb_map.is_contiguous())
+        fail("ray_compose_bwd_bg: d_rgb_map [B,3] (contiguous) with B = acc.size(0) expected");
+    Tensor d_weight = fe(weight, {M}), d_bg = at::empty_like(d_rgb_map);
+    OT d_refl, d_normals;
+    if (refl_rows.has_value()) d_refl = at::empty_like(*refl_rows);
+    if (want_d_normals) d_normals = fe(weight, {M, 3});
+    if (M || B)
+        check(nmf_ray_compose_bwd_bg(M ? f32(weight) : nullptr, static_cast<const float*>(vptr(refl_rows)),
+                                     static_cast<const int32_t*>(vptr(inv)), static_cast<const float*>(vptr(normals)), f32(rays),
+                                     M ? i32(ray_id) : nullptr, M, f32(bg), bg_per_ray ? 1 : 0, tonemap ? 1 : 0, noclip ? 1 : 0,
+                                     static_cast<const float*>(vptr(rgb_lin)), f32(d_rgb_map), static_cast<const float*>(vptr(d_acc)),
+                                     static_cast<const float*>(vptr(d_ori)), M ? out(d_weight) : nullptr,
+                                     d_refl.has_value() ? out(*d_refl) : nullptr, d_normals.has_value() ? out(*d_normals) : nullptr,
+                                     f32(acc), B, out(d_bg), st(stream)),
+              "nmf_ray_compose_bwd_bg");
+    return {d_weight, d_refl, d_normals, d_bg};
 }
 
 void adam_step(int64_t slots_addr, int64_t n, const OT& guard, int64_t stream) {
@@ -1203,6 +1274,9 @@
     m.def("view_adjoint_to_rays", &view_adjoint_to_rays);
     m.def("select_total", &select_total);
     m.def("bounce_prep_bwd", &bounce_prep_bwd);
+    m.def("bounce_prep_heads_bwd_dense", &bounce_prep_heads_bwd_dense);
+    m.def("segment_sum_pair", &segment_sum_pair);
+    m.def("ray_compose_bwd_bg", &ray_compose_bwd_bg);
     py::class_<StepCore>(m, "StepCore")
         .def(py::init<>())
         .def("chunk", &StepCore::chunk)
@@ -1225,6 +1299,7 @@
         RW(max_samples) RW(alpha_bits) RW(alpha_coarse) RW(scale) RW(anoise) RW(min_rough) RW(rays_per_ray) RW(test_rays_per_ray)
         RW(detach_n) RW(max_brdf_rays) RW(max_retrace_rays) RW(white) RW(one) RW(select_ws) RW(g_dpk) RW(g_dlk) RW(g_apl) RW(g_ali)
         RW(g_mlp) RW(g_basis) RW(g_hW) RW(g_hb) RW(d_sat) RW(d_pole) RW(d_mip) RW(d_bg_out) RW(used_env) RW(sampler) RW(wait_tables) RW(wait_env)
+        RW(fold_rows0) RW(fold_row_sums) RW(fold_bg) RW(late_mlp_join)
 #undef RW
         ;
 }
diff --git a/nmf_amd/csrc/rows_bwd.hpp b/nmf_amd/csrc/rows_bwd.hpp
--- a/nmf_amd/csrc/rows_bwd.hpp
+++ b/nmf_amd/csrc/rows_bwd.hpp
@@ -53,11 +53,15 @@
     int sN, sr, sf, sd;
     const float* dfeat;
     float* d_normals;
+    float* d_normals_dense;
 };
 __device__ __forceinline__ void prep_bwd_row(const RowsBwdIn& q, int64_t t, float (&gh)[HEADS], float4 (&gf)[FEAT / 4]) {
     const bool want_n = !q.detach_n && q.dN;
     const int64_t m = q.bidx[t];
-    const float nx = q.normals[t * 3], ny = q.normals[t * 3 + 1], nz = q.normals[t * 3 + 2];
+    const int64_t in = q.d_normals_dense ? m : t;
+    const float nx = q.normals[in * 3], ny = q.normals[in * 3 + 1], nz = q.normals[in * 3 + 2];
+    float dm[3] = {0.f, 0.f, 0.f};
+    if (q.d_normals_dense) { dm[0] = q.d_normals_dense[m * 3]; dm[1] = q.d_normals_dense[m * 3 + 1]; dm[2] = q.d_normals_dense[m * 3 + 2]; }
     float dn[3] = {0.f, 0.f, 0.f}, dd[3] = {0.f, 0.f, 0.f}, d0[3] = {0.f, 0.f, 0.f}, dr = 0.f;
     if (want_n) { dn[0] = q.dN[t * q.sN]; dn[1] = q.dN[t * q.sN + 1]; dn[2] = q.dN[t * q.sN + 2]; }
     if (q.ddiff) { dd[0] = q.ddiff[t * q.sd]; dd[1] = q.ddiff[t * q.sd + 1]; dd[2] = q.ddiff[t * q.sd + 2]; }
@@ -73,7 +77,11 @@
         const float s = sgn(-(d[0] * nx + d[1] * ny + d[2] * nz));
         gn[0] = dn[0] * s; gn[1] = dn[1] * s; gn[2] = dn[2] * s;
     }
-    q.d_normals[t * 3] = gn[0]; q.d_normals[t * 3 + 1] = gn[1]; q.d_normals[t * 3 + 2] = gn[2];
+    if (q.d_normals_dense) {
+        q.d_normals_dense[m * 3] = dm[0] + gn[0]; q.d_normals_dense[m * 3 + 1] = dm[1] + gn[1]; q.d_normals_dense[m * 3 + 2] = dm[2] + gn[2];
+    } else {
+        q.d_normals[t * 3] = gn[0]; q.d_normals[t * 3 + 1] = gn[1]; q.d_normals[t * 3 + 2] = gn[2];
+    }
 #pragma unroll
     for (int j = 0; j < HEADS; ++j) gh[j] = 0.f;
     float E3[3];
diff --git a/nmf_amd/csrc/segsum_wide.hpp b/nmf_amd/csrc/segsum_wide.hpp
--- /dev/null
+++ b/nmf_amd/csrc/segsum_wide.hpp
@@ -0,0 +1,30 @@
+#pragma once
+#include "common.hpp"
+
+namespace nmf_segsum {
+
+template <int G>
+__device__ __forceinline__ void wide_segment(const float* __restrict__ vals, int64_t stride, int D,
+                                             const int64_t* __restrict__ offsets, int64_t s, float* __restrict__ out) {
+    const int lane = lane_id();
+    const int ch = lane & (G - 1), slot = lane / G;
+    constexpr int SLOTS = 64 / G;
+    const int64_t b = offsets[s], e = offsets[s + 1];
+    float a = 0.f;
+    if (ch < D) {
+        float a1 = 0.f, a2 = 0.f, a3 = 0.f;
+        int64_t r = b + slot;
+        for (; r + 3 * SLOTS < e; r += 4 * SLOTS) {
+            const float v0 = vals[r * stride + ch], v1 = vals[(r + SLOTS) * stride + ch];
+            const float v2 = vals[(r + 2 * SLOTS) * stride + ch], v3 = vals[(r + 3 * SLOTS) * stride + ch];
+            a += v0; a1 += v1; a2 += v2; a3 += v3;
+        }
+        for (; r < e; r += SLOTS) a += vals[r * stride + ch];
+        a = (a + a1) + (a2 + a3);
+    }
+#pragma unroll
+    for (int sh = 32; sh >= G; sh >>= 1) a += __shfl_down(a, sh, 64);
+    if (lane < D) out[s * D + lane] = a;
+}
+
+}
diff --git a/nmf_amd/csrc/shade.hip b/nmf_amd/csrc/shade.hip
--- a/nmf_amd/csrc/shade.hip
+++ b/nmf_amd/csrc/shade.hip
@@ -400,8 +400,14 @@
     const float* __restrict__ normals, const float* __restrict__ rays, const int32_t* __restrict__ ray_id, int64_t M,
     const float* __restrict__ bg, int bg_per_ray, int tonemap, int noclip, const float* __restrict__ rgb_lin,
     const float* __restrict__ d_rgb_map, const float* __restrict__ d_acc, const float* __restrict__ d_ori,
-    float* __restrict__ d_weight, float* __restrict__ d_refl, float* __restrict__ d_normals) {
+    float* __restrict__ d_weight, float* __restrict__ d_refl, float* __restrict__ d_normals,
+    const float* __restrict__ acc, int64_t B, float* __restrict__ d_bg) {
     const int64_t m = (int64_t)blockIdx.x * blockDim.x + threadIdx.x;
+    if (d_bg && m < B) {
+        const float ta = acc[m];
+#pragma unroll
+        for (int c = 0; c < 3; ++c) d_bg[m * 3 + c] = (1.f - ta) * d_rgb_map[m * 3 + c];
+    }
     if (m >= M) return;
     const int64_t r = ray_id[m];
     const float w = weight[m];
@@ -593,21 +599,43 @@
     return NMF_OK;
 }
 
+static int ray_compose_bwd_impl(const char* what, const float* weight, const float* refl_rows, const int32_t* inv, const float* normals,
+                                const float* rays, const int32_t* ray_id, int64_t M, const float* bg, int32_t bg_per_ray,
+                                int32_t tonemap, int32_t noclip, const float* rgb_lin, const float* d_rgb_map, const float* d_acc,
+                                const float* d_ori, float* d_weight, float* d_refl, float* d_normals, const float* acc, int64_t B,
+                                float* d_bg, void* stream) {
+    const int64_t n = d_bg && B > M ? B : M;
+    if (n == 0) return NMF_OK;
+    NMF_REQUIRE(M == 0 || (weight && rays && ray_id && bg && rgb_lin && d_weight), NMF_EINVAL, what);
+    NMF_REQUIRE(!(inv && refl_rows) || d_refl, NMF_EINVAL, what);
+    NMF_REQUIRE(M == 0 || !d_ori || normals, NMF_EINVAL, what);
+    NMF_LAUNCH(k_ray_compose_bwd, dim3((unsigned)cdiv(n, 256)), dim3(256), 0, (hipStream_t)stream, weight,
+                       refl_rows, inv, normals, rays, ray_id, M, bg, (int)bg_per_ray, (int)tonemap, (int)noclip, rgb_lin,
+                       d_rgb_map, d_acc, d_ori, d_weight, d_refl, d_normals, acc, B, d_bg);
+    NMF_CHECK_LAUNCH(what);
+    return NMF_OK;
+}
+
 extern "C" int nmf_ray_compose_bwd(const float* weight, const float* refl_rows, const int32_t* inv, const float* normals,
                                    const float* rays, const int32_t* ray_id, int64_t M, const float* bg,
                                    int32_t bg_per_ray, int32_t tonemap, int32_t noclip, const float* rgb_lin,
                                    const float* d_rgb_map, const float* d_acc, const float* d_ori, float* d_weight,
                                    float* d_refl, float* d_normals, void* stream) {
     NMF_REQUIRE(M >= 0, NMF_EINVAL, "nmf_ray_compose_bwd: M < 0");
-    if (M == 0) return NMF_OK;
-    NMF_REQUIRE(weight && rays && ray_id && bg && rgb_lin && d_weight, NMF_EINVAL, "nmf_ray_compose_bwd: null");
-    NMF_REQUIRE(!(inv && refl_rows) || d_refl, NMF_EINVAL, "nmf_ray_compose_bwd: d_refl missing");
-    NMF_REQUIRE(!d_ori || normals, NMF_EINVAL, "nmf_ray_compose_bwd: d_ori needs normals");
-    NMF_LAUNCH(k_ray_compose_bwd, dim3((unsigned)cdiv(M, 256)), dim3(256), 0, (hipStream_t)stream, weight,
-                       refl_rows, inv, normals, rays, ray_id, M, bg, (int)bg_per_ray, (int)tonemap, (int)noclip, rgb_lin,
-                       d_rgb_map, d_acc, d_ori, d_weight, d_refl, d_normals);
-    NMF_CHECK_LAUNCH("nmf_ray_compose_bwd");
-    return NMF_OK;
+    return ray_compose_bwd_impl("nmf_ray_compose_bwd: null", weight, refl_rows, inv, normals, rays, ray_id, M, bg, bg_per_ray, tonemap,
+                                noclip, rgb_lin, d_rgb_map, d_acc, d_ori, d_weight, d_refl, d_normals, nullptr, 0, nullptr, stream);
+}
+
+extern "C" int nmf_ray_compose_bwd_bg(const float* weight, const float* refl_rows, const int32_t* inv, const float* normals,
+                                      const float* rays, const int32_t* ray_id, int64_t M, const float* bg,
+                                      int32_t bg_per_ray, int32_t tonemap, int32_t noclip, const float* rgb_lin,
+                                      const float* d_rgb_map, const float* d_acc, const float* d_ori, float* d_weight,
+                                      float* d_refl, float* d_normals, const float* acc, int64_t B, float* d_bg, void* stream) {
+    NMF_REQUIRE(M >= 0 && B >= 0, NMF_EINVAL, "nmf_ray_compose_bwd_bg: M < 0 or B < 0");
+    NMF_REQUIRE(B == 0 || (acc && d_rgb_map && d_bg), NMF_EINVAL, "nmf_ray_compose_bwd_bg: acc / d_rgb_map / d_bg null");
+    return ray_compose_bwd_impl("nmf_ray_compose_bwd_bg: null", weight, refl_rows, inv, normals, rays, ray_id, M, bg, bg_per_ray,
+                                tonemap, noclip, rgb_lin, d_rgb_map, d_acc, d_ori, d_weight, d_refl, d_normals, acc, B,
+                                B ? d_bg : nullptr, stream);
 }
 
 extern "C" int nmf_bg_adjoint(const float* acc, const float* d_rgb_map, int64_t B, float* d_bg, void* stream) {
diff --git a/nmf_amd/csrc/step_core.inc b/nmf_amd/csrc/step_core.inc
--- a/nmf_amd/csrc/step_core.inc
+++ b/nmf_amd/csrc/step_core.inc
@@ -97,6 +97,7 @@
     bool used_env = false, early_env_done = false;
     bool env_split = true;
     int64_t env_split_min_lookups = 16384;
+    bool fold_rows0 = true, fold_row_sums = true, fold_bg = true, late_mlp_join = true;
     bool env_keep_sat = false;
     py::object early_cb = py::none();
     int64_t comm_stream = 0;
@@ -713,11 +714,17 @@
         CoreSamples& S = t.S;
         const int lvl = t.lvl;
         const bool view = lvl > 0;
-        Tensor d_w;
+        Tensor d_w, d_bg;
         OT d_refl, d_nrm;
-        std::tie(d_w, d_refl, d_nrm) =
-            ray_compose_bwd(t.w, t.refl, t.inv, d_ori.has_value() ? t.nr : OT(), S.rays, S.ray_id, t.bg, t.per_ray_bg, lvl == 0, false,
-                            t.rgb_lin, d_rgb, d_acc, d_ori, d_ori.has_value(), main_stream);
+        const bool bg_here = t.per_ray_bg && fold_bg && d_rgb.is_contiguous();
+        if (bg_here)
+            std::tie(d_w, d_refl, d_nrm, d_bg) =
+                ray_compose_bwd_bg(t.w, t.refl, t.inv, d_ori.has_value() ? t.nr : OT(), S.rays, S.ray_id, t.bg, t.per_ray_bg, lvl == 0,
+                                   false, t.rgb_lin, d_rgb, d_acc, d_ori, d_ori.has_value(), t.acc, main_stream);
+        else
+            std::tie(d_w, d_refl, d_nrm) =
+                ray_compose_bwd(t.w, t.refl, t.inv, d_ori.has_value() ? t.nr : OT(), S.rays, S.ray_id, t.bg, t.per_ray_bg, lvl == 0, false,
+                                t.rgb_lin, d_rgb, d_acc, d_ori, d_ori.has_value(), main_stream);
         Tensor d_sigma = composite_bwd(t.sg, S.dist, t.w, t.offsets, t.B, scale, d_w, main_stream);
         bool early_walk = false;
         if (t.sparse_n && t.M >= walk_side_min_samples) {
@@ -735,23 +742,24 @@
         Tensor d_rays;
         int64_t env_side = 0;
         if (t.per_ray_bg) {
-            Tensor d_bg = bg_adjoint(t.acc, d_rgb, main_stream);
+            if (!bg_here) d_bg = bg_adjoint(t.acc, d_rgb, main_stream);
             Tensor env_rows = t.B == S.rays.size(0) ? S.rays : S.rays.narrow(0, 0, t.B);
             env_side = t.B >= mlp_side_min_rays ? fork(2 + (lvl > 0 ? 1 : 0)) : 0;
             d_rays = env_bwd(env_rows, *t.rough, d_bg, env_side ? env_side : main_stream);
             if (env_side) end_side();
             keep_.push_back(d_bg);
         }
-        Tensor d_inc, d_brdf, dL, d_fd, dV, dV_rows;
+        Tensor d_inc, d_brdf, dL, d_fd, dV, dV_rows, rows6;
         if (view) {
             std::tie(d_inc, d_brdf, dL, d_fd, dV) =
                 shade_mix_bwd_view(t.V, t.f0, t.diff, t.cnt32, t.row_of_ray, t.L, t.incoming, *t.brdf, *d_refl, main_stream);
-            dV_rows = segment_sum(dV, OT(), t.row_off, t.Mb, 8, main_stream);
+            if (fold_row_sums) std::tie(dV_rows, rows6) = segment_sum_pair(dV, d_fd, 6, t.row_off, t.Mb, main_stream);
+            else dV_rows = segment_sum(dV, OT(), t.row_off, t.Mb, 8, main_stream);
         } else {
             std::tie(d_inc, d_brdf, dL, d_fd) =
                 shade_mix_bwd(t.V, t.f0, t.diff, t.cnt32, t.row_of_ray, t.L, t.incoming, *t.brdf, *d_refl, main_stream);
         }
-        Tensor rows6 = segment_sum_wide(d_fd, 6, t.row_off, t.Mb, main_stream);
+        if (!rows6.defined()) rows6 = segment_sum_wide(d_fd, 6, t.row_off, t.Mb, main_stream);
         const int64_t n_re = t.idx_re.has_value() ? t.idx_re->size(0) : (t.child ? t.R : 0);
         const int64_t n_env = t.R - n_re;
         const bool below = t.child && t.child->B >= mlp_side_min_rays;
@@ -792,7 +800,7 @@
                 early_env_done = true;
             }
         }
-        if (mlp_side) join(mlp_side, {d_feat});
+        if (mlp_side && !late_mlp_join) join(mlp_side, {d_feat});
         if (!have_feat)
             d_feat = brdf_mlp_bwd(mlp_ws, t.hl, t.dl, t.feat, t.r1, t.row_of_ray, *t.brdf, *t.brdf_mask, d_brdf, g_mlp, 0, main_stream, mlp_img());
         Tensor dN, dr1, dV_ggx;
@@ -806,10 +814,19 @@
             dN = rows4.slice(1, 0, 3); dr1 = rows4.select(1, 3);
         }
         Tensor d_normals, d_heads, d_app;
+        if (mlp_side && late_mlp_join) join(mlp_side, {d_feat});
+        OT d_normal;
+        bool normal_done = false;
         if (t.sparse_n) {
             std::tie(d_normals, d_app) =
                 bounce_prep_heads_bwd(t.bidx, *t.nr, t.heads, S.ray_id, S.rays, t.conv, min_rough, detach_n, dN, dr1, rows6.slice(1, 0, 3),
                                       rows6.slice(1, 3, 6), d_feat, t.app, head_W, head_b, head_p, g_hW, g_hb, main_stream);
+        } else if (fold_rows0 && !detach_n && d_nrm.has_value()) {
+            d_app = bounce_prep_heads_bwd_dense(t.bidx, *t.nr, t.heads, S.ray_id, S.rays, t.conv, min_rough, dN, dr1, rows6.slice(1, 0, 3),
+                                                rows6.slice(1, 3, 6), d_feat, t.app, head_W, head_b, head_p, g_hW, g_hb, *d_nrm,
+                                                main_stream);
+            d_normal = d_nrm;
+            normal_done = true;
         } else {
             std::tie(d_normals, d_heads, d_app) =
                 bounce_prep_bwd(OT(t.inv), *t.nr, t.heads, S.ray_id, S.rays, t.conv, min_rough, detach_n, dN, dr1,
@@ -817,8 +834,8 @@
             d_app = heads_bwd(t.app, head_W, head_b, head_p, d_heads, g_hW, g_hb, OT(d_app), main_stream);
         }
         app_segs_.push_back(Seg(t.xyz_rows, OT(), OT(), OT(), OT(), OT(), d_app));
-        OT d_normal;
-        if (detach_n) d_normal = d_nrm;
+        if (normal_done) {}
+        else if (detach_n) d_normal = d_nrm;
         else if (d_nrm.has_value()) d_normal = d_normals.add_(*d_nrm);
         else d_normal = d_normals;
         if (t.sparse_n) {
diff --git a/nmf_amd/hip.py b/nmf_amd/hip.py
--- a/nmf_amd/hip.py
+++ b/nmf_amd/hip.py
@@ -89,6 +89,7 @@
     "nmf_camera_rays", "nmf_frame_finish",
     "nmf_atlas_texels", "nmf_atlas_store",
     "nmf_rays_place", "nmf_merge_rank", "nmf_merge_scatter",
+    "nmf_bounce_prep_heads_bwd_dense", "nmf_segment_sum_pair", "nmf_ray_compose_bwd_bg",
 ]
 for _n in EXPORTS:
     if not hasattr(_lib, _n):
@@ -630,6 +631,22 @@
 
 def bg_adjoint(acc, d_rgb):
     return HOST_EXT.bg_adjoint(acc, d_rgb, _stream())
+
+
+def bounce_prep_heads_bwd_dense(bidx, normals, heads, ray_id, rays, conv, min_rough, dN, dr1, df0, ddiff, dfeat, app, head_W, head_b, hp,
+                                gW, gb, d_normals_acc):
+    return HOST_EXT.bounce_prep_heads_bwd_dense(bidx, normals, heads, ray_id, rays, conv, float(min_rough), dN, dr1, df0, ddiff, dfeat,
+                                                app, head_W, head_b, list(hp), gW, gb, d_normals_acc, _stream())
+
+
+def segment_sum_pair(vals3, vals_wide, D, offsets, n_seg):
+    return HOST_EXT.segment_sum_pair(vals3, vals_wide, int(D), offsets, int(n_seg), _stream())
+
+
+def ray_compose_bwd_bg(weight, refl_rows, inv, normals, rays, ray_id, bg, bg_per_ray, tonemap, noclip, rgb_lin, d_rgb_map,
+                       d_acc, d_ori, want_d_normals, acc):
+    return HOST_EXT.ray_compose_bwd_bg(weight, refl_rows, inv, normals, rays, ray_id, bg, bool(bg_per_ray), bool(tonemap),
+                                       bool(noclip), rgb_lin, d_rgb_map, d_acc, d_ori, bool(want_d_normals), acc, _stream())
 
 
 def sqerr_fwd(pred, gt):
```

Result: slower. 2.903 million rays/s (-1.7%).
